# Fro116/RecommenderSystem

Measured on AMD Instinct MI355X. Metric: interactions/sec, higher is better.
Workload: dtype bf16

## Files before the change

### include/rsys_debug.h

```cpp
#ifndef RSYS_DEBUG_H
#define RSYS_DEBUG_H
#include "rsys.h"

#ifdef __cplusplus
extern "C" {
#endif

int32_t rsys_debug_get(rsys_model* m, const char* key, void* out, int64_t bytes);

int32_t rsys_local_group_create(int32_t world, int32_t device, void** group);
int32_t rsys_local_group_destroy(void* group);
int32_t rsys_comm_init_local(void* group, int32_t rank, rsys_comm** out);
int32_t rsys_comm_debug_delay(rsys_comm* c, int32_t microseconds);

int32_t rsys_dev_alloc(void** p, size_t bytes);
int32_t rsys_dev_free(void* p);
int32_t rsys_dev_h2d(void* dst, const void* src, size_t bytes);
int32_t rsys_dev_d2h(void* dst, const void* src, size_t bytes);
int32_t rsys_dev_memset(void* dst, int value, size_t bytes);
int32_t rsys_op_gemm(int32_t dtype, const void* A, const void* B, void* C, int32_t M, int32_t N, int32_t K,
                     int64_t lda, int64_t ldb, int64_t ldc, int32_t a_km, int32_t b_km, int32_t a_f32, int32_t c_f32,
                     int32_t splitk);
int32_t rsys_op_gemm_rows(int32_t dtype, const void* A, const void* B, void* C, int32_t M, int32_t N, int32_t K,
                          int64_t lda, int64_t ldb, int64_t ldc, int32_t b_km, int32_t c_f32, const int32_t* rows_dev);
// ... 8 lines not shown
                              int32_t b_km, int32_t a_f32, int32_t c_f32, int32_t epi, int32_t splitk, int32_t flags, float alpha,
                              int32_t accum, int32_t set, int32_t m_expect, int32_t cus, char* tag, int32_t tag_bytes, int32_t* splits);
int32_t rsys_op_attention(int32_t dtype, int32_t B, int32_t T, int32_t H, int32_t KV, int32_t hd, const void* qkv,
                          const int32_t* uid, const int32_t* tm, void* O, float* lse, const void* dO, void* dqkv,
                          const float* rope_cos, const float* rope_sin);
int32_t rsys_op_attention_ex(int32_t dtype, int32_t B, int32_t T, int32_t H, int32_t KV, int32_t hd, const void* qkv,
                             const int32_t* uid, const int32_t* tm, void* O, float* lse, const void* dO, void* dqkv,
                             const float* rope_cos, const float* rope_sin, const int32_t* rope_pos, int32_t rope_rows,
                             const int32_t* q_active, float* amax_fwd, float* amax_bwd);
int32_t rsys_op_attention_cached(int32_t dtype, int32_t rows, int32_t T, int32_t H, int32_t KV, int32_t hd, const void* qkv, const void* cache,
                                 int32_t n_slots, const int32_t* slot, const int32_t* n_hist, const int32_t* n_cand, void* O);
int32_t rsys_op_attention_cached_tiles(int32_t dtype, int32_t rows, int32_t T, int32_t H, int32_t KV, int32_t hd, const void* qkv, const void* cache,
                                       int32_t n_slots, int32_t Tc, int32_t n_seg, const int32_t* seg, void* O);
int32_t rsys_op_rank_cache_copy_segments(int32_t dtype, int32_t rows, int32_t T, int32_t H, int32_t KV, int32_t hd, const void* qkv, void* cache,
                                         int32_t n_slots, int32_t Tc, int32_t n_seg, const int32_t* seg);
int32_t rsys_rank_cache_get(rsys_model* m, int32_t layer, int32_t slot, void* out, int64_t bytes);
int32_t rsys_op_topk(const float* scores, int64_t ld, int32_t rows, int32_t V, int32_t k,
                     int32_t* ids, float* vals, int32_t* counts);
int32_t rsys_op_target_rank(const float* scores, int64_t ld, int32_t rows, int32_t V, const int32_t* targets, int32_t* rank_out);
int32_t rsys_op_pair_ranks(const float* scores, int64_t ld, int32_t rows, int32_t V, const int32_t* self, const int64_t* tgt_offsets,
                           const int32_t* tgt_ids, int32_t* ranks_out);
int32_t rsys_sim_pair_scores(void* h, int32_t n_src, const int32_t* sources, float* out);
int32_t rsys_rank_gram_get(rsys_model* m, int32_t medium, int32_t n_groups, const int64_t* cand_offsets, const int32_t* cand_ids,
                           float* out, int64_t n_out);
int32_t rsys_op_rerank(int32_t n, int32_t partialk, const float* pen, const float* r, const float* gram, const int32_t* ss_bits,
                       const int32_t* related_bits, int32_t* picks);
int32_t rsys_render_debug_keep(rsys_model* m, int32_t on);
int32_t rsys_render_debug_get(rsys_model* m, const char* key, void* out, int64_t cap, int64_t* bytes);
int32_t rsys_sim_debug_get(void* h, const char* name, void* out, int64_t n);
int32_t rsys_search_debug_get(void* h, const char* name, float* out, int64_t n);
int32_t rsys_op_embedding_scatter(const float* gx0, int64_t ldx, const int32_t* matchedid, const int32_t* m_matchedid, int32_t N,
                                  int32_t V, int32_t D, float* gE, int32_t atomic);
int32_t rsys_op_f8_quantize(const void* src, int64_t ld_src, int32_t rows, int32_t cols, int32_t fmt, int32_t layout, int32_t seg_cols,
                            int32_t seg_rep, void* dst, int64_t ld_dst, float* amax_dev, float* desc_dev, const float* wamax_dev,
                            int32_t n_w, int32_t w_rep, int32_t desc_mode);
int32_t rsys_op_f8_weights(const float* src, int64_t ld, int32_t rows, int32_t cols, int32_t layout, int32_t seg_rows, int32_t seg_rep,
                           float* amax_dev, void* dst, void* dst_t, int64_t ld_t);
int32_t rsys_op_gemm_f8(const void* A8, const void* B8, void* C, int32_t M, int32_t N, int32_t K, int64_t lda, int64_t ldb, int64_t ldc,
                        int32_t a_fmt, int32_t c_f32, const float* desc_dev, int32_t seg_cols, int32_t alt, int32_t kb0, int32_t kb1,
                        int32_t kb2);
int32_t rsys_op_rmsnorm_fwd(int32_t dtype, const float* x, const float* scale, void* y, float* rstd, int64_t rows, int32_t D,
                            const int32_t* rows_dev, const int32_t* in_rows, float* amax);
int32_t rsys_op_rmsnorm_bwd(int32_t dtype, int32_t g_f32, const void* g, const float* x, const float* scale, const float* rstd,
                            const float* resid, const int32_t* resid_slot, const int32_t* io_rows, const int32_t* rows_dev,
                            float* dx, void* dx_t, float* dscale, int64_t rows, int32_t D, float* amax, int32_t deterministic);
int32_t rsys_op_ce(int32_t dtype, void* logits, int64_t ldl, int32_t n, int32_t V, const int32_t* idx, const float* label,
                   const float* weight, const int32_t* position, const float* stats, const int32_t* npos, float task_w, float* loss,
                   int32_t deterministic);
int32_t rsys_op_rating_tail(int32_t dtype, void* z, const void* hact, int32_t n, int32_t D, const float* w2, const float* b2,
                            const int32_t* idx, const float* label, const float* weight, const float* stats, float rating_mean,
                            float task_w, int32_t evaluate, float* loss, float* dw2, float* db2, float* db0, const int32_t* npos,
                            int32_t deterministic);
int32_t rsys_op_sumsq(const float* g, int64_t n, float* out);
int32_t rsys_op_clip_adamw(int32_t dtype, float* p, float* g, float* m, float* v, void* shadow, int64_t n_decay, int64_t n_total,
                           float lr, float b1, float b2, float eps, float wd, int32_t step, float max_norm, float grad_div,
                           int32_t zero_grad, int64_t sh_skip_lo, int64_t sh_skip_hi, int32_t fused, float* sumsq);
int32_t rsys_op_adapter_bank(int32_t dtype, int32_t stages, int32_t train, int32_t rows, int32_t Ttok, int32_t D, int32_t H, int32_t KV, int32_t hd,
                             int32_t L, int32_t layer, float p, uint64_t seed, int64_t stream, const int32_t* row_slot, const void* bankA,
                             const void* bankB, const void* xn, void* La, void* qkv, const void* dqkv, void* dLa, void* dxn, float* partA, float* partB,
                             float* gA, float* gB, const float* rope_cos, const float* rope_sin, const int32_t* rope_pos, int32_t rope_rows);
int32_t rsys_op_adapter_bank_tiles(int32_t dtype, int32_t stages, int32_t rows, int32_t Ttok, int32_t D, int32_t H, int32_t KV, int32_t hd, int32_t L,
                                   int32_t layer, const int32_t* tile_slot, const void* bankA, const void* bankB, const void* xn, void* La, void* qkv,
                                   const float* rope_cos, const float* rope_sin, const int32_t* rope_pos, int32_t rope_rows);
int32_t rsys_op_adapter_bank_segments(int32_t dtype, int32_t stages, int32_t train, int32_t rows, int32_t Ttok, int32_t D, int32_t H, int32_t KV, int32_t hd,
                                      int32_t L, int32_t layer, float p, uint64_t seed, int64_t stream, const int32_t* segs, int32_t n_seg, const void* bankA,
                                      const void* bankB, const void* xn, void* La, void* qkv, const void* dqkv, void* dLa, void* dxn, float* partA,
                                      float* partB, float* gA, float* gB, const float* rope_cos, const float* rope_sin, const int32_t* rope_pos,
                                      int32_t rope_rows);
int32_t rsys_op_adapter_bank_adamw(int32_t dtype, float* A32, float* B32, float* gA, float* gB, float* mA, float* vA, float* mB, float* vB, void* A,
                                   void* B, int64_t nA, int64_t nB, const float* per_slot, float b1, float b2, float eps, float wd, float* norms);
int32_t rsys_op_dropout(int32_t dtype, const void* src, void* dst, int64_t n, float p, uint64_t seed, int64_t stream, int32_t accumulate);
int32_t rsys_op_vp_ce(int32_t dtype, int32_t stages, int32_t deterministic, const int32_t* idx, const float* label, const float* weight,
                      const int32_t* position, const float* stats, const int32_t* npos, float task_w, int32_t KB, int32_t KBmax, float* own,
                      const void* EwAll, const float* metaAll, int32_t W, int32_t D, void* EwC, float* metaC, int32_t* nlive, int32_t* pre,
                      void* logits, int64_t ldl, int32_t Vloc, int32_t col0, float* lmax, const float* gmax, float* sums, int32_t cap,
                      int32_t rank, float* loss, int32_t rows, int32_t rows_finish);
int32_t rsys_op_ss(int32_t dtype, int32_t stages, int32_t deterministic, int32_t len, int32_t n_s, int32_t n_tot, int32_t col0, uint64_t seed,
                   int64_t stream, int32_t* cols, int32_t* bitmap, int32_t* tlist, int32_t* tcount, const float* metaC, const int32_t* nlive,
                   const int32_t* pre, int32_t rank, int32_t cap_rows, int32_t rows, int32_t rows_finish, const void* EwC, const void* Floc,
                   int32_t D, void* logits, int64_t ldl, float* lmax, float* lsum, float* tl, float* gmax, float* loss, float* dt,
                   float* gE_loc, float* dEwC, const int32_t* ridx, int32_t rbase, int64_t rld, int32_t rn, int32_t rtable_rows,
                   const void* gsrc, void* gdst, const float* asrc, float* adst);
int32_t rsys_op_shard_rows(int32_t stages, const int32_t* skey, const int32_t* sidx, int32_t N, int32_t V, int32_t* slot, int32_t* uniq,
                           int32_t* tok2u, int32_t* plan, const int32_t* bound, int32_t nb, int32_t* off, float* table, int64_t ld,
                           int32_t table_rows, const int32_t* ids, int32_t sub, float* packed, int32_t n, int32_t D, const int32_t* count,
                           const int32_t* m_matchedid, const int32_t* userid, const int32_t* m_tmid, int32_t Ntok, const float* Frem,
                           int32_t frem_rows, float* x0, int32_t* uid_t, int32_t* tm_t);

#ifdef __cplusplus
}
#endif
#endif
```

### recommendersystem_amd/_lib.py

```python
import ctypes as C
import os

os.environ.setdefault("HSA_ENABLE_IPC_MODE_LEGACY", "0")

HERE = os.path.dirname(os.path.abspath(__file__))
LIB_PATH = os.path.join(HERE, "librsys_hip.so")


class RsysError(RuntimeError):
    pass


class rsys_config(C.Structure):
    _fields_ = [
        ("num_layers", C.c_int32), ("num_heads", C.c_int32), ("num_kv_heads", C.c_int32),
        ("embed_dim", C.c_int32), ("intermediate_dim", C.c_int32), ("max_sequence_length", C.c_int32),
        ("vocab_0", C.c_int32), ("vocab_1", C.c_int32),
        ("vocab_status", C.c_int32), ("vocab_gender", C.c_int32), ("vocab_source", C.c_int32),
        ("metadata_dim", C.c_int32),
        ("min_ts", C.c_double), ("max_ts", C.c_double),
        ("rating_mean", C.c_float), ("rating_std", C.c_float), ("mask_rate", C.c_float),
        ("mask_topk", C.c_int32), ("finetune", C.c_int32), ("finetune_metric", C.c_int32),
        ("dtype", C.c_int32), ("max_rows", C.c_int32), ("lora_dropout", C.c_float),
        ("table_shard_rank", C.c_int32), ("table_shard_world", C.c_int32), ("sampled_negatives", C.c_int32),
# ... 149 lines not shown
    ("rsys_comm_destroy", C.c_int32, [_P]),
    ("rsys_comm_debug_delay", C.c_int32, [_P, C.c_int32]),
    ("rsys_set_grad_sync", C.c_int32, [_P, _P]),
    ("rsys_model_set_split_table_reduce", C.c_int32, [_P, C.c_int32]),
    ("rsys_model_set_shard_comm", C.c_int32, [_P, _P]),
    ("rsys_table_rows", C.c_int32, [_P, C.POINTER(C.c_int64), C.POINTER(C.c_int64)]),
    ("rsys_local_group_create", C.c_int32, [C.c_int32, C.c_int32, C.POINTER(_P)]),
    ("rsys_local_group_destroy", C.c_int32, [_P]),
    ("rsys_comm_init_local", C.c_int32, [_P, C.c_int32, C.POINTER(_P)]),
    ("rsys_allreduce_grads", C.c_int32, [_P, _P]),
    ("rsys_grad_sync_early", C.c_int32, [_P, C.POINTER(C.c_int64)]),
    ("rsys_grad_sync_schedule", C.c_int32, [_P, C.POINTER(C.c_int64), C.c_int32, C.POINTER(C.c_int32)]),
    ("rsys_comm_info", C.c_int32, [_P, C.POINTER(C.c_int32)]),
    ("rsys_allreduce_f64", C.c_int32, [_P, C.POINTER(C.c_double), C.c_int32]),
    ("rsys_self_test", C.c_int32, [_P]),
    ("rsys_param_checksum", C.c_int32, [_P, C.POINTER(C.c_double * 4)]),
    ("rsys_grad_buffer", C.c_int32, [_P, C.POINTER(_P), C.POINTER(C.c_int64)]),
    ("rsys_param_buffer", C.c_int32, [_P, C.POINTER(_P), C.POINTER(C.c_int64)]),
    ("rsys_refresh_shadow", C.c_int32, [_P]),
    ("rsys_dev_alloc", C.c_int32, [C.POINTER(_P), C.c_size_t]),
    ("rsys_dev_free", C.c_int32, [_P]),
    ("rsys_dev_h2d", C.c_int32, [_P, _P, C.c_size_t]),
    ("rsys_dev_d2h", C.c_int32, [_P, _P, C.c_size_t]),
    ("rsys_dev_memset", C.c_int32, [_P, C.c_int, C.c_size_t]),
    ("rsys_op_gemm", C.c_int32, [C.c_int32, _P, _P, _P, C.c_int32, C.c_int32, C.c_int32, C.c_int64, C.c_int64, C.c_int64,
                                 C.c_int32, C.c_int32, C.c_int32, C.c_int32, C.c_int32]),
    ("rsys_op_f8_quantize", C.c_int32, [_P, C.c_int64, C.c_int32, C.c_int32, C.c_int32, C.c_int32, C.c_int32, C.c_int32, _P, C.c_int64, _P, _P, _P,
                                          C.c_int32, C.c_int32, C.c_int32]),
    ("rsys_op_f8_weights", C.c_int32, [_P, C.c_int64, C.c_int32, C.c_int32, C.c_int32, C.c_int32, C.c_int32, _P, _P, _P, C.c_int64]),
    ("rsys_op_gemm_f8", C.c_int32, [_P, _P, _P, C.c_int32, C.c_int32, C.c_int32, C.c_int64, C.c_int64, C.c_int64, C.c_int32, C.c_int32, _P,
                                      C.c_int32, C.c_int32, C.c_int32, C.c_int32, C.c_int32]),
    ("rsys_op_gemm_rows", C.c_int32, [C.c_int32, _P, _P, _P, C.c_int32, C.c_int32, C.c_int32, C.c_int64, C.c_int64, C.c_int64,
                                      C.c_int32, C.c_int32, _P]),
    ("rsys_op_gemm_klimit", C.c_int32, [C.c_int32, _P, _P, _P, C.c_int32, C.c_int32, C.c_int32, C.c_int64, C.c_int64, C.c_int64, C.c_int32, _P]),
    ("rsys_op_gemm_epi", C.c_int32, [C.c_int32, _P, _P, _P, C.c_int32, C.c_int32, C.c_int32, C.c_int64, C.c_int64, C.c_int64, C.c_int32, C.c_int32,
                                     C.c_int32, C.c_float, C.c_int32, _P, _P, C.c_int64, _P, C.c_int64, _P, _P, _P, _P, _P,
                                     C.c_int32, C.c_int32, C.c_int32, C.c_int32, _P, C.c_char_p, C.c_int32, C.POINTER(C.c_int32)]),
    ("rsys_debug_gemm_route", C.c_int32, [C.c_int32] * 4 + [C.c_int64] * 3 + [C.c_int32] * 7 + [C.c_float] + [C.c_int32] * 4
                                          + [C.c_char_p, C.c_int32, C.POINTER(C.c_int32)]),
    ("rsys_op_attention", C.c_int32, [C.c_int32] + [C.c_int32] * 5 + [_P] * 9),
    ("rsys_op_attention_ex", C.c_int32, [C.c_int32] + [C.c_int32] * 5 + [_P] * 10 + [C.c_int32, _P, _P, _P]),
    ("rsys_op_topk", C.c_int32, [_P, C.c_int64, C.c_int32, C.c_int32, C.c_int32, _P, _P, _P]),
    ("rsys_op_target_rank", C.c_int32, [_P, C.c_int64, C.c_int32, C.c_int32, _P, _P]),
    ("rsys_op_pair_ranks", C.c_int32, [_P, C.c_int64, C.c_int32, C.c_int32, _P, _P, _P, _P]),
    ("rsys_rank_gram_get", C.c_int32, [_P, C.c_int32, C.c_int32, _P, _P, _P, C.c_int64]),
    ("rsys_op_rerank", C.c_int32, [C.c_int32, C.c_int32, _P, _P, _P, _P, _P, _P]),
    ("rsys_op_embedding_scatter", C.c_int32, [_P, C.c_int64, _P, _P, C.c_int32, C.c_int32, C.c_int32, _P, C.c_int32]),
    ("rsys_op_rmsnorm_fwd", C.c_int32, [C.c_int32, _P, _P, _P, _P, C.c_int64, C.c_int32, _P, _P, _P]),
    ("rsys_op_rmsnorm_bwd", C.c_int32, [C.c_int32, C.c_int32] + [_P] * 11 + [C.c_int64, C.c_int32, _P, C.c_int32]),
    ("rsys_op_ce", C.c_int32, [C.c_int32, _P, C.c_int64, C.c_int32, C.c_int32] + [_P] * 6 + [C.c_float, _P, C.c_int32]),
    ("rsys_op_rating_tail", C.c_int32, [C.c_int32, _P, _P, C.c_int32, C.c_int32] + [_P] * 6 + [C.c_float, C.c_float, C.c_int32]
                                        + [_P] * 5 + [C.c_int32]),
    ("rsys_op_sumsq", C.c_int32, [_P, C.c_int64, _P]),
    ("rsys_op_clip_adamw", C.c_int32, [C.c_int32] + [_P] * 5 + [C.c_int64, C.c_int64] + [C.c_float] * 5
                                       + [C.c_int32, C.c_float, C.c_float, C.c_int32, C.c_int64, C.c_int64, C.c_int32, _P]),
    ("rsys_op_adapter_bank", C.c_int32, [C.c_int32] * 11 + [C.c_float, C.c_uint64, C.c_int64] + [_P] * 16 + [C.c_int32]),
    ("rsys_op_adapter_bank_tiles", C.c_int32, [C.c_int32] * 10 + [_P] * 9 + [C.c_int32]),
    ("rsys_op_adapter_bank_segments", C.c_int32, [C.c_int32] * 11 + [C.c_float, C.c_uint64, C.c_int64, _P, C.c_int32] + [_P] * 15 + [C.c_int32]),
    ("rsys_op_adapter_bank_adamw", C.c_int32, [C.c_int32] + [_P] * 10 + [C.c_int64, C.c_int64, _P] + [C.c_float] * 4 + [_P]),
    ("rsys_op_dropout", C.c_int32, [C.c_int32, _P, _P, C.c_int64, C.c_float, C.c_uint64, C.c_int64, C.c_int32]),
    ("rsys_op_vp_ce", C.c_int32, [C.c_int32] * 3 + [_P] * 6 + [C.c_float, C.c_int32, C.c_int32, _P, _P, _P, C.c_int32, C.c_int32]
                                  + [_P] * 5 + [C.c_int64, C.c_int32, C.c_int32, _P, _P, _P, C.c_int32, C.c_int32, _P, C.c_int32, C.c_int32]),
    ("rsys_op_ss", C.c_int32, [C.c_int32] * 7 + [C.c_uint64, C.c_int64] + [_P] * 7 + [C.c_int32] * 4 + [_P, _P, C.c_int32, _P, C.c_int64]
                               + [_P] * 9 + [C.c_int32, C.c_int64, C.c_int32, C.c_int32] + [_P] * 4),
    ("rsys_op_shard_rows", C.c_int32, [C.c_int32, _P, _P, C.c_int32, C.c_int32] + [_P] * 5 + [C.c_int32, _P, _P, C.c_int64, C.c_int32, _P,
                                       C.c_int32, _P, C.c_int32, C.c_int32] + [_P] * 4 + [C.c_int32, _P, C.c_int32, _P, _P, _P]),
    ("rsys_step_mark", C.c_int32, [_P]),
    ("rsys_step_marks_get", C.c_int32, [_P, _P, C.c_int32, C.POINTER(C.c_int32)]),
    ("rsys_op_timing", C.c_int32, [_P, C.c_int32]),
    ("rsys_timing_get", C.c_int32, [_P, C.c_char_p, C.c_size_t]),
    ("rsys_op_timing_filter", C.c_int32, [_P, C.c_char_p]),
    ("rsys_switches_reload", C.c_int32, []),
    ("rsys_switches_describe", C.c_int32, [C.c_char_p, C.c_int32]),
]
EXPORTED = [s[0] for s in _SIGS]

_lib = None


def lib():
    global _lib
    if _lib is None:
        if not os.path.exists(LIB_PATH):
            raise RsysError(f"{LIB_PATH} is missing: build it with `make -C recommendersystem_amd/csrc` "
                            "(there is no CPU fallback for the HIP path)")
        L = C.CDLL(LIB_PATH, mode=C.RTLD_GLOBAL)
        for name, res, args in _SIGS:
            fn = getattr(L, name)
            fn.restype = res
            fn.argtypes = args
        _lib = L
    return _lib


def last_error():
    buf = C.create_string_buffer(2048)
    lib().rsys_last_error(buf, 2048)
    return buf.value.decode(errors="replace")


def check(rc):
    if rc != 0:
        raise RsysError(f"rsys error {rc}: {last_error()}")


def device_count():
# ... 16 lines not shown
```

### recommendersystem_amd/csrc/capi.hip

```cpp
#include <algorithm>
#include <dlfcn.h>
#include <math.h>
#include <stdlib.h>
#include <string.h>

#include <sstream>

#include "comm.hpp"
#include "encoder_handle.hpp"
#include "model_internal.hpp"

namespace rsys {
static thread_local std::string g_err;
void set_error(const std::string& msg) { g_err = msg; }
}

using namespace rsys;

struct rsys_model { Model* m; };
struct rsys_optimizer { Optimizer o; };

#define CHECK_HANDLE(h) do { if ((h) == nullptr) { set_error("null handle"); return RSYS_ERR_ARG; } } while (0)

extern "C" {

const char* rsys_version(void) { return "recommendersystem_amd 0.1 (gfx950)"; }

size_t rsys_last_error(char* buf, size_t n) {
  if (buf && n) { strncpy(buf, g_err.c_str(), n - 1); buf[n - 1] = 0; }
  return g_err.size();
}

int32_t rsys_device_count(int32_t* n) {
  int c = 0;
  hipError_t e = hipGetDeviceCount(&c);
  if (e != hipSuccess) c = 0;
  if (n) *n = c;
  return RSYS_OK;
}
int32_t rsys_device_synchronize(void) { HIP_CHECK(hipDeviceSynchronize()); return RSYS_OK; }

int32_t rsys_model_create(const rsys_config* cfg, int32_t device, rsys_model** out) {
  switches_parse();
  Model* m = nullptr;
  int rc = model_create(cfg, device, &m);
  if (rc) return rc;
  *out = new rsys_model{m};
  return RSYS_OK;
}
int32_t rsys_model_destroy(rsys_model* h) { if (!h) return RSYS_OK; model_destroy(h->m); delete h; return RSYS_OK; }
int32_t rsys_model_init_random(rsys_model* h, uint64_t seed) { CHECK_HANDLE(h); return model_init_random(h->m, seed); }
int32_t rsys_model_load_metadata(rsys_model* h, const float* t, int64_t V, int64_t M) { CHECK_HANDLE(h); ARG_CHECK(t, "null table"); return model_load_metadata(h->m, t, V, M); }
int32_t rsys_model_random_metadata(rsys_model* h, uint64_t seed) { CHECK_HANDLE(h); return model_random_metadata(h->m, seed); }
int32_t rsys_model_set_rope(rsys_model* h, const float* c, const float* s, int64_t n) { CHECK_HANDLE(h); ARG_CHECK(c && s, "null table"); return model_set_rope(h->m, c, s, n); }

int32_t rsys_param_count(rsys_model* h, int32_t* n) { CHECK_HANDLE(h); *n = (int32_t)h->m->tensors.size(); return RSYS_OK; }
int32_t rsys_param_info(rsys_model* h, int32_t i, char* name, size_t cap, int64_t shape[2], int32_t* ndim, int32_t* trainable) {
  CHECK_HANDLE(h);
  ARG_CHECK(i >= 0 && i < (int)h->m->tensors.size(), "parameter index");
  const TensorInfo& t = h->m->tensors[i];
  if (name && cap) { strncpy(name, t.name.c_str(), cap - 1); name[cap - 1] = 0; }
  if (shape) { if (t.ndim == 1) { shape[0] = t.cols; shape[1] = 0; } else { shape[0] = t.rows; shape[1] = t.cols; } }
  if (ndim) *ndim = t.ndim;
  if (trainable) *trainable = t.trainable ? 1 : 0;
  return RSYS_OK;
}
int32_t rsys_param_get(rsys_model* h, const char* name, float* out, int64_t n) { CHECK_HANDLE(h); ARG_CHECK(name && out, "null"); return model_param_io(h->m, name, out, nullptr, n, 0); }
int32_t rsys_param_set(rsys_model* h, const char* name, const float* in, int64_t n) { CHECK_HANDLE(h); ARG_CHECK(name && in, "null"); return model_param_io(h->m, name, nullptr, in, n, 0); }
int32_t rsys_grad_get(rsys_model* h, const char* name, float* out, int64_t n) { CHECK_HANDLE(h); ARG_CHECK(name && out, "null"); return model_param_io(h->m, name, out, nullptr, n, 1); }
int32_t rsys_zero_grad(rsys_model* h) {
  CHECK_HANDLE(h);
  HIP_CHECK(hipSetDevice(h->m->device));
  HIP_CHECK(hipMemsetAsync(h->m->G, 0, h->m->n_total * 4, h->m->stream));
  h->m->table_grads_pending = false;
  h->m->gE_clean[0] = h->m->gE_clean[1] = true;
  return RSYS_OK;
}

int32_t rsys_batch_upload(rsys_model* h, const rsys_batch* b) { CHECK_HANDLE(h); return model_batch_upload(h->m, b); }
int32_t rsys_batch_rows(rsys_model* h, int32_t* rows_out) { CHECK_HANDLE(h); ARG_CHECK(rows_out, "null"); *rows_out = h->m->cur_rows; return RSYS_OK; }
int32_t rsys_batch_upload_trimmed(rsys_model* h, const rsys_batch* b, int32_t row_len) { CHECK_HANDLE(h); return model_batch_upload_trimmed(h->m, b, row_len); }
int32_t rsys_batch_row_length(rsys_model* h, int32_t* row_len_out) {
  CHECK_HANDLE(h); ARG_CHECK(row_len_out, "null");
  *row_len_out = h->m->cur_rows > 0 ? h->m->S : 0;
  return RSYS_OK;
}
int32_t rsys_serving_pack_set(rsys_model* h, int32_t on) { CHECK_HANDLE(h); h->m->serving_pack = on != 0; return RSYS_OK; }
int32_t rsys_serving_pack_get(rsys_model* h, int32_t* on_out) { CHECK_HANDLE(h); ARG_CHECK(on_out, "null"); *on_out = h->m->serving_pack ? 1 : 0; return RSYS_OK; }
int32_t rsys_serving_pack_ranking_set(rsys_model* h, int32_t on) { CHECK_HANDLE(h); h->m->serving_pack_ranking = on != 0; return RSYS_OK; }
int32_t rsys_serving_pack_ranking_get(rsys_model* h, int32_t* on_out) { CHECK_HANDLE(h); ARG_CHECK(on_out, "null"); *on_out = h->m->serving_pack_ranking ? 1 : 0; return RSYS_OK; }
int32_t rsys_serving_trim_set(rsys_model* h, int32_t on) { CHECK_HANDLE(h); h->m->serving_trim = on != 0; return RSYS_OK; }
int32_t rsys_serving_trim_get(rsys_model* h, int32_t* on_out) { CHECK_HANDLE(h); ARG_CHECK(on_out, "null"); *on_out = h->m->serving_trim ? 1 : 0; return RSYS_OK; }
int32_t rsys_batch_prefetch(rsys_model* h, const rsys_batch* b) { CHECK_HANDLE(h); return model_batch_prefetch(h->m, b); }
int32_t rsys_batch_swap(rsys_model* h) { CHECK_HANDLE(h); return model_batch_swap(h->m); }

int32_t rsys_forward_backward(rsys_model* h, int32_t evaluate, const float task_w[4], float grad_scale, uint64_t seed, uint64_t step) {
  CHECK_HANDLE(h);
  return model_forward_backward(h->m, evaluate, task_w, grad_scale, seed, step);
}

int32_t rsys_losses_get(rsys_model* h, float losses_out[12], float wsum_out[4]) {
  CHECK_HANDLE(h);
  Model* m = h->m;
  HIP_CHECK(hipSetDevice(m->device));
  float acc[16], st[8];
  HIP_CHECK(hipMemcpyAsync(acc, m->loss_acc, 16 * 4, hipMemcpyDeviceToHost, m->stream));
  HIP_CHECK(hipMemcpyAsync(st, m->stats, 8 * 4, hipMemcpyDeviceToHost, m->stream));
  HIP_CHECK(hipStreamSynchronize(m->stream));
  for (int ti = 0; ti < 4; ++ti) {
    float ws = fmaxf(st[2 * ti], 1e-8f);
    for (int k = 0; k < 3; ++k) losses_out[3 * ti + k] = acc[3 * ti + k] / ws;
    if (wsum_out) wsum_out[ti] = st[2 * ti + 1];
  }
  return RSYS_OK;
}

int32_t rsys_losses_push(rsys_model* h) {
  CHECK_HANDLE(h);
  Model* m = h->m;
  HIP_CHECK(hipSetDevice(m->device));
  if (m->loss_ring == nullptr) HIP_CHECK(hipMalloc((void**)&m->loss_ring, (size_t)Model::loss_ring_cap * 24 * 4));
  if (m->loss_ring_n >= Model::loss_ring_cap) { set_error("rsys_losses_push: ring full (rsys_losses_drain first)"); return RSYS_ERR_STATE; }
  float* slot = m->loss_ring + (size_t)m->loss_ring_n * 24;
  HIP_CHECK(hipMemcpyAsync(slot, m->loss_acc, 16 * 4, hipMemcpyDeviceToDevice, m->stream));
  HIP_CHECK(hipMemcpyAsync(slot + 16, m->stats, 8 * 4, hipMemcpyDeviceToDevice, m->stream));
  m->loss_ring_n += 1;
  return RSYS_OK;
}
// ... 561 lines not shown
  std::vector<std::pair<int64_t, int64_t>> done = m->reduced, rem;
  m->reduced.clear();
  if (m->sharded) done.emplace_back(m->o_E, m->o_E + (int64_t)m->TR * m->D);
  if (split) {
    done.emplace_back(m->o_E, m->o_E + (int64_t)m->TR * m->D);
    m->early_reduced += (int64_t)m->TR * m->D;
  }
  std::sort(done.begin(), done.end());
  int64_t at = 0;
  for (auto& r : done) { if (r.first > at) rem.emplace_back(at, r.first); at = std::max(at, r.second); }
  if (at < m->n_opt) rem.emplace_back(at, m->n_opt);
  auto reduce_rest = [&](int64_t lo, int64_t hi) -> int {
    for (auto& r : rem) {
      const int64_t a = std::max(r.first, lo), b = std::min(r.second, hi);
      if (a < b) { int rc = reduce_range(m, c, a, b); if (rc) return rc; }
    }
    return RSYS_OK;
  };
  if (model_finalize_splittable(m)) {
    int64_t wo = 0, wn = 0;
    int rc = model_finalize_stage(m, 1, &wo, &wn);
    if (rc) return rc;
    HIP_CHECK(hipEventRecord(c->ev_ready, m->stream));
    HIP_CHECK(hipStreamWaitEvent(c->stream, c->ev_ready, 0));
    m->bucket_phase = 1;
    if (split) {
      int64_t tail_rows = 0;
      rc = model_split_table_tail(m, c, c->stream, &tail_rows);
      if (rc) return rc;
      m->bucket_log.push_back({0, (int64_t)c->world * tail_rows * (m->D + 1), 4});
    }
    rc = reduce_rest(0, std::min(wo, m->n_opt));
    if (rc) return rc;
    rc = reduce_rest(std::min(wo + wn, m->n_opt), m->n_opt);
    if (rc) return rc;
    rc = model_finalize_stage(m, 2, nullptr, nullptr);
    if (rc) return rc;
    HIP_CHECK(hipEventRecord(c->ev_ready, m->stream));
    HIP_CHECK(hipStreamWaitEvent(c->stream, c->ev_ready, 0));
    m->bucket_phase = 2;
    rc = reduce_rest(wo, std::min(wo + wn, m->n_opt));
    if (rc) return rc;
  } else {
    m->bucket_phase = 1;
    int rc = model_finalize_grads(m);
    if (rc) return rc;
    HIP_CHECK(hipEventRecord(c->ev_ready, m->stream));
    HIP_CHECK(hipStreamWaitEvent(c->stream, c->ev_ready, 0));
    rc = reduce_rest(0, m->n_opt);
    if (rc) return rc;
  }
  HIP_CHECK(hipEventRecord(c->ev_done, c->stream));
  HIP_CHECK(hipStreamWaitEvent(m->stream, c->ev_done, 0));
  return RSYS_OK;
}
int32_t rsys_grad_sync_early(rsys_model* h, int64_t* n) { CHECK_HANDLE(h); ARG_CHECK(n, "null"); *n = h->m->early_reduced; return RSYS_OK; }
int32_t rsys_grad_sync_schedule(rsys_model* h, int64_t* out, int32_t cap, int32_t* n_out) {
  CHECK_HANDLE(h); ARG_CHECK(out && n_out && cap >= 0, "null");
  const auto& log = h->m->bucket_log;
  const int n = (int)std::min<size_t>(log.size(), (size_t)cap);
  for (int i = 0; i < n; ++i) { out[3 * i] = log[i].lo; out[3 * i + 1] = log[i].hi; out[3 * i + 2] = log[i].phase; }
  *n_out = (int32_t)log.size();
  return RSYS_OK;
}
int32_t rsys_comm_info(rsys_comm* c, int32_t out[4]) {
  CHECK_HANDLE(c); ARG_CHECK(out, "null");
  out[0] = c->rank; out[1] = c->world;
  out[2] = c->lg ? 2 : (c->comm ? 1 : 0);
  out[3] = c->comm ? comm_rccl_version() : 0;
  return RSYS_OK;
}
int32_t rsys_allreduce_f64(rsys_comm* c, double* x, int32_t n) {
  CHECK_HANDLE(c);
  ARG_CHECK(n >= 1 && n <= 64 && x, "n in [1,64]");
  if (!comm_active(c)) return RSYS_OK;
  HIP_CHECK(hipSetDevice(c->device));
  HIP_CHECK(hipMemcpyAsync(c->scratch, x, n * 8, hipMemcpyHostToDevice, c->stream));
  RC(comm_all_reduce_f64(c, c->scratch, (size_t)n, c->stream));
  HIP_CHECK(hipMemcpyAsync(x, c->scratch, n * 8, hipMemcpyDeviceToHost, c->stream));
  HIP_CHECK(hipStreamSynchronize(c->stream));
  return RSYS_OK;
}
int32_t rsys_self_test(rsys_comm* c) {
  CHECK_HANDLE(c);
  double one = 1.0;
  int rc = rsys_allreduce_f64(c, &one, 1);
  if (rc) return rc;
  if (one != (double)c->world) { set_error("all-reduce self test: sum of ones != world size"); return RSYS_ERR_COMM; }
  return RSYS_OK;
}

int32_t rsys_grad_buffer(rsys_model* h, void** p, int64_t* n) {
  CHECK_HANDLE(h);
  int rc = model_finalize_grads(h->m);
  if (rc) return rc;
  *p = h->m->G; *n = h->m->n_opt;
  return RSYS_OK;
}
int32_t rsys_param_buffer(rsys_model* h, void** p, int64_t* n) { CHECK_HANDLE(h); *p = h->m->P; *n = h->m->n_total; return RSYS_OK; }
int32_t rsys_refresh_shadow(rsys_model* h) { CHECK_HANDLE(h); return model_refresh_shadow(h->m); }

int32_t rsys_dev_alloc(void** p, size_t bytes) { HIP_CHECK(hipMalloc(p, bytes ? bytes : 16)); HIP_CHECK(hipMemset(*p, 0, bytes ? bytes : 16)); return RSYS_OK; }
int32_t rsys_dev_free(void* p) { HIP_CHECK(hipFree(p)); return RSYS_OK; }
int32_t rsys_dev_h2d(void* d, const void* s, size_t n) { HIP_CHECK(hipMemcpy(d, s, n, hipMemcpyHostToDevice)); return RSYS_OK; }
int32_t rsys_dev_d2h(void* d, const void* s, size_t n) { HIP_CHECK(hipDeviceSynchronize()); HIP_CHECK(hipMemcpy(d, s, n, hipMemcpyDeviceToHost)); return RSYS_OK; }
int32_t rsys_dev_memset(void* d, int v, size_t n) { HIP_CHECK(hipMemset(d, v, n)); return RSYS_OK; }

int32_t rsys_op_gemm(int32_t dtype, const void* A, const void* B, void* C, int32_t M, int32_t N, int32_t K, int64_t lda,
                     int64_t ldb, int64_t ldc, int32_t a_km, int32_t b_km, int32_t a_f32, int32_t c_f32, int32_t splitk) {
  switches_parse();
  GemmParams p{};
  p.A = A; p.B = B; p.C = C; p.M = M; p.N = N; p.K = K; p.lda = lda; p.ldb = ldb; p.ldc = ldc;
  p.c_f32 = c_f32; p.splitk = splitk < 1 ? 1 : splitk; p.alpha = 1.f;
  p.epi = p.splitk > 1 ? EPI_ATOMIC : EPI_STORE;
  if (sw().debug_epi >= 0) p.epi = sw().debug_epi;
  int rc = dtype == RSYS_DTYPE_BF16 ? launch_gemm<bf16>(p, a_f32 != 0, false, a_km != 0, b_km != 0, nullptr)
                                    : launch_gemm<float>(p, false, false, a_km != 0, b_km != 0, nullptr);
  if (rc) return rc;
  HIP_CHECK(hipDeviceSynchronize());
  return RSYS_OK;
}

int32_t rsys_op_gemm_rows(int32_t dtype, const void* A, const void* B, void* C, int32_t M, int32_t N, int32_t K, int64_t lda,
                          int64_t ldb, int64_t ldc, int32_t b_km, int32_t c_f32, const int32_t* rows_dev) {
  switches_parse();
  ARG_CHECK(rows_dev != nullptr, "rsys_op_gemm_rows: rows_dev is null");
  GemmParams p{};
  p.A = A; p.B = B; p.C = C; p.M = M; p.N = N; p.K = K; p.lda = lda; p.ldb = ldb; p.ldc = ldc;
  p.c_f32 = c_f32 != 0; p.splitk = 1; p.alpha = 1.f; p.epi = EPI_STORE; p.m_dev = rows_dev;
  if (c_f32 == 3) { p.epi = EPI_ATOMIC; p.splitk = 8; }
  int rc = dtype == RSYS_DTYPE_BF16 ? launch_gemm<bf16>(p, false, false, false, b_km != 0, nullptr)
                                    : launch_gemm<float>(p, false, false, false, b_km != 0, nullptr);
  if (rc) return rc;
  HIP_CHECK(hipDeviceSynchronize());
  return RSYS_OK;
}

int32_t rsys_op_gemm_klimit(int32_t dtype, const void* A, const void* B, void* C, int32_t M, int32_t N, int32_t K, int64_t lda,
                            int64_t ldb, int64_t ldc, int32_t accumulate, const int32_t* k_dev) {
  switches_parse();
  ARG_CHECK(k_dev != nullptr, "rsys_op_gemm_klimit: k_dev is null");
  GemmParams p{};
  p.A = A; p.B = B; p.C = C; p.M = M; p.N = N; p.K = K; p.lda = lda; p.ldb = ldb; p.ldc = ldc;
  p.c_f32 = 1; p.splitk = 1; p.alpha = 1.f; p.epi = accumulate ? EPI_ACCUM : EPI_STORE; p.k_dev = k_dev;
  int rc = dtype == RSYS_DTYPE_BF16 ? launch_gemm<bf16>(p, false, false, true, true, nullptr)
                                    : launch_gemm<float>(p, false, false, true, true, nullptr);
  if (rc) return rc;
  HIP_CHECK(hipDeviceSynchronize());
// ... 335 lines not shown
                     : launch_rmsnorm_bwd_f32<float>((const float*)g, x, scale, rstd, resid, dx, (float*)dx_t, dscale, rows, D, nullptr, rows_dev, amax);
  else rc = bf ? launch_rmsnorm_bwd<bf16>((const bf16*)g, x, scale, rstd, resid, dx, (bf16*)dx_t, dscale, rows, D, nullptr, rows_dev, resid_slot, io_rows, amax)
               : launch_rmsnorm_bwd<float>((const float*)g, x, scale, rstd, resid, dx, (float*)dx_t, dscale, rows, D, nullptr, rows_dev, resid_slot, io_rows, amax);
  if (rc) return rc;
  HIP_CHECK(hipDeviceSynchronize());
  return det.check("rsys_op_rmsnorm_bwd");
}

int32_t rsys_op_ce(int32_t dtype, void* logits, int64_t ldl, int32_t n, int32_t V, const int32_t* idx, const float* label,
                   const float* weight, const int32_t* position, const float* stats, const int32_t* npos, float task_w, float* loss,
                   int32_t deterministic) {
  switches_parse();
  ARG_CHECK(logits && idx && label && weight && position && stats && loss && n >= 0 && V >= 1, "rsys_op_ce: arguments");
  HookDet det(deterministic != 0 && n > 0);
  RC(det.alloc(n, ceil32(n)));
  int rc = dtype == RSYS_DTYPE_BF16 ? launch_ce_fwd_bwd<bf16>((bf16*)logits, ldl, n, V, idx, label, weight, position, stats, npos, task_w, loss, nullptr)
                                    : launch_ce_fwd_bwd<float>((float*)logits, ldl, n, V, idx, label, weight, position, stats, npos, task_w, loss, nullptr);
  if (rc) return rc;
  HIP_CHECK(hipDeviceSynchronize());
  return det.check("rsys_op_ce");
}

int32_t rsys_op_rating_tail(int32_t dtype, void* z, const void* hact, int32_t n, int32_t D, const float* w2, const float* b2,
                            const int32_t* idx, const float* label, const float* weight, const float* stats, float rating_mean,
                            float task_w, int32_t evaluate, float* loss, float* dw2, float* db2, float* db0, const int32_t* npos,
                            int32_t deterministic) {
  switches_parse();
  ARG_CHECK(z && hact && w2 && b2 && idx && label && weight && stats && loss && dw2 && db2 && db0 && n >= 0, "rsys_op_rating_tail: arguments");
  HookDet det(deterministic != 0 && n > 0);
  const long long grid = std::min<long long>((n + 3) / 4, 512);
  RC(det.alloc(grid * (2LL * D + 4), ceil32(grid) * D));
  int rc = dtype == RSYS_DTYPE_BF16
               ? launch_rating_tail<bf16>((bf16*)z, (const bf16*)hact, n, D, w2, b2, idx, label, weight, stats, rating_mean, task_w, evaluate, loss,
                                          dw2, db2, db0, nullptr, npos)
               : launch_rating_tail<float>((float*)z, (const float*)hact, n, D, w2, b2, idx, label, weight, stats, rating_mean, task_w, evaluate, loss,
                                           dw2, db2, db0, nullptr, npos);
  if (rc) return rc;
  HIP_CHECK(hipDeviceSynchronize());
  return det.check("rsys_op_rating_tail");
}

int32_t rsys_op_sumsq(const float* g, int64_t n, float* out) {
  ARG_CHECK(g && out, "rsys_op_sumsq: arguments");
  float* part = nullptr;
  HIP_CHECK(hipMalloc((void**)&part, (size_t)sumsq_parts() * 4));
  int rc = launch_sumsq(g, n, out, part, nullptr, true);
  hipError_t e = hipDeviceSynchronize();
  hipFree(part);
  if (rc) return rc;
  HIP_CHECK(e);
  return RSYS_OK;
}

int32_t rsys_op_clip_adamw(int32_t dtype, float* p, float* g, float* m, float* v, void* shadow, int64_t n_decay, int64_t n_total,
                           float lr, float b1, float b2, float eps, float wd, int32_t step, float max_norm, float grad_div,
                           int32_t zero_grad, int64_t sh_skip_lo, int64_t sh_skip_hi, int32_t fused, float* sumsq) {
  switches_parse();
  ARG_CHECK(p && g && m && v && sumsq && n_total >= 4 && step >= 1, "rsys_op_clip_adamw: arguments");
  float* part = nullptr;
  HIP_CHECK(hipMalloc((void**)&part, (size_t)sumsq_parts() * 4));
  const bool bf = dtype == RSYS_DTYPE_BF16;
  int rc = launch_sumsq(g, n_total, sumsq, part, nullptr, true);
  if (fused) {
    const float* ss = max_norm > 0.f ? sumsq : nullptr;
    if (!rc) rc = bf ? launch_adamw<bf16>(p, g, m, v, (bf16*)shadow, n_decay, n_total, lr, b1, b2, eps, wd, step, ss, grad_div, max_norm, zero_grad, nullptr,
                                          sh_skip_lo, sh_skip_hi)
                     : launch_adamw<float>(p, g, m, v, nullptr, n_decay, n_total, lr, b1, b2, eps, wd, step, ss, grad_div, max_norm, zero_grad, nullptr);
  } else {
    if (!rc) rc = launch_scale(g, n_total, sumsq, grad_div, max_norm, nullptr);
    if (!rc) rc = bf ? launch_adamw<bf16>(p, g, m, v, (bf16*)shadow, n_decay, n_total, lr, b1, b2, eps, wd, step, nullptr, 1.f, 0.f, zero_grad, nullptr,
                                          sh_skip_lo, sh_skip_hi)
                     : launch_adamw<float>(p, g, m, v, nullptr, n_decay, n_total, lr, b1, b2, eps, wd, step, nullptr, 1.f, 0.f, zero_grad, nullptr);
  }
  hipError_t e = hipDeviceSynchronize();
  hipFree(part);
  if (rc) return rc;
  HIP_CHECK(e);
  return RSYS_OK;
}

int32_t rsys_op_adapter_bank(int32_t dtype, int32_t stages, int32_t train, int32_t rows, int32_t Ttok, int32_t D, int32_t H, int32_t KV, int32_t hd,
                             int32_t L, int32_t layer, float p, uint64_t seed, int64_t stream, const int32_t* row_slot, const void* bankA,
                             const void* bankB, const void* xn, void* La, void* qkv, const void* dqkv, void* dLa, void* dxn, float* partA, float* partB,
                             float* gA, float* gB, const float* rope_cos, const float* rope_sin, const int32_t* rope_pos, int32_t rope_rows) {
  switches_parse();
  return adapter_bank_op(dtype, stages, train, rows, Ttok, D, H, KV, hd, L, layer, p, seed, stream, row_slot, bankA, bankB, xn, La, qkv, dqkv, dLa, dxn,
                         partA, partB, gA, gB, rope_cos, rope_sin, rope_pos, rope_rows);
}

int32_t rsys_op_adapter_bank_tiles(int32_t dtype, int32_t stages, int32_t rows, int32_t Ttok, int32_t D, int32_t H, int32_t KV, int32_t hd, int32_t L,
                                   int32_t layer, const int32_t* tile_slot, const void* bankA, const void* bankB, const void* xn, void* La, void* qkv,
                                   const float* rope_cos, const float* rope_sin, const int32_t* rope_pos, int32_t rope_rows) {
  switches_parse();
  return adapter_bank_op(dtype, stages, 0, rows, Ttok, D, H, KV, hd, L, layer, 0.f, 0, 0, tile_slot, bankA, bankB, xn, La, qkv, nullptr, nullptr, nullptr,
                         nullptr, nullptr, nullptr, nullptr, rope_cos, rope_sin, rope_pos, rope_rows, 1);
}

int32_t rsys_op_adapter_bank_segments(int32_t dtype, int32_t stages, int32_t train, int32_t rows, int32_t Ttok, int32_t D, int32_t H, int32_t KV, int32_t hd,
                                      int32_t L, int32_t layer, float p, uint64_t seed, int64_t stream, const int32_t* segs, int32_t n_seg, const void* bankA,
                                      const void* bankB, const void* xn, void* La, void* qkv, const void* dqkv, void* dLa, void* dxn, float* partA,
                                      float* partB, float* gA, float* gB, const float* rope_cos, const float* rope_sin, const int32_t* rope_pos,
                                      int32_t rope_rows) {
  switches_parse();
  return adapter_bank_op(dtype, stages, train, rows, Ttok, D, H, KV, hd, L, layer, p, seed, stream, segs, bankA, bankB, xn, La, qkv, dqkv, dLa, dxn, partA,
                         partB, gA, gB, rope_cos, rope_sin, rope_pos, rope_rows, 2, n_seg);
}
// ... 275 lines not shown
```

### recommendersystem_amd/csrc/elementwise.hip

```cpp
#include "kernels.hpp"

namespace rsys {

thread_local DetScratch g_det;

__global__ void reduce_parts_kernel(const float* __restrict__ part, int nparts, long long stride, int n, float* dst) {
  const int c = blockIdx.x * blockDim.x + threadIdx.x;
  if (c >= n) return;
  float acc = 0.f;
  for (int b = 0; b < nparts; ++b) acc += part[(long long)b * stride + c];
  dst[c] += acc;
}
__global__ void reduce_parts_stage_kernel(const float* __restrict__ part, int nparts, long long stride, int n, float* out) {
  const int c = blockIdx.x * blockDim.x + threadIdx.x, chunk = blockIdx.y;
  if (c >= n) return;
  const int b0 = chunk * 32, b1 = min(nparts, b0 + 32);
  float acc = 0.f;
  for (int b = b0; b < b1; ++b) acc += part[(long long)b * stride + c];
  out[(long long)chunk * n + c] = acc;
}
int launch_reduce_parts(const float* part, int nparts, long long stride, int n, float* dst, hipStream_t s) {
  if (nparts <= 0 || n <= 0) return RSYS_OK;
  if (nparts > 64 && g_det.tmp != nullptr) {
    const int chunks = (nparts + 31) / 32;
// ... 796 lines not shown
__global__ __launch_bounds__(1024) void cast_colsum_kernel(const float* __restrict__ src, bf16* __restrict__ dst, long long rows, int D,
                                                           float* colsum, int rows_per_block, float* part) {
  __shared__ float red[2048];
  const int cg = D >> 2;
  const int c = (threadIdx.x % cg) * 4, lane_r = threadIdx.x / cg, nr = 1024 / cg;
  const long long r0 = (long long)blockIdx.x * rows_per_block, r1 = min(rows, r0 + rows_per_block);
  float4 acc = make_float4(0, 0, 0, 0);
  long long r = r0 + lane_r;
  for (; r + 3 * nr < r1; r += 4 * nr) {
    float4 v[4];
#pragma unroll
    for (int u = 0; u < 4; ++u) v[u] = *(const float4*)(src + (r + u * nr) * D + c);
#pragma unroll
    for (int u = 0; u < 4; ++u) {
      bf16x4 o; o[0] = (bf16)v[u].x; o[1] = (bf16)v[u].y; o[2] = (bf16)v[u].z; o[3] = (bf16)v[u].w;
      *(bf16x4*)(dst + (r + u * nr) * D + c) = o;
      acc.x += v[u].x; acc.y += v[u].y; acc.z += v[u].z; acc.w += v[u].w;
    }
  }
  for (; r < r1; r += nr) {
    const float4 v = *(const float4*)(src + r * D + c);
    bf16x4 o; o[0] = (bf16)v.x; o[1] = (bf16)v.y; o[2] = (bf16)v.z; o[3] = (bf16)v.w;
    *(bf16x4*)(dst + r * D + c) = o;
    acc.x += v.x; acc.y += v.y; acc.z += v.z; acc.w += v.w;
  }
  if (lane_r < 2) *(float4*)&red[lane_r * D + c] = acc;
  __syncthreads();
  for (int base = 2; base < nr; base += 2) {
    if (lane_r >= base && lane_r < base + 2) {
      float4 o = *(float4*)&red[(lane_r - base) * D + c];
      o.x += acc.x; o.y += acc.y; o.z += acc.z; o.w += acc.w;
      *(float4*)&red[(lane_r - base) * D + c] = o;
    }
    __syncthreads();
  }
  for (int cc = threadIdx.x; cc < D; cc += 1024) {
    const float v = red[cc] + (nr > 1 ? red[D + cc] : 0.f);
    if (part != nullptr) part[(long long)blockIdx.x * D + cc] = v;
    else if (v != 0.f) atomicAdd(&colsum[cc], v);
  }
}
int launch_cast_colsum(const float* src, bf16* dst, long long rows, int D, float* colsum, hipStream_t s) {
  ARG_CHECK(D % 4 == 0 && D <= 1024 && 1024 % (D >> 2) == 0, "cast_colsum: D/4 must divide 1024, D <= 1024");
  const int rpb = (int)std::max<long long>(32, (rows + 511) / 512);
  const int grid = div_up(rows, rpb);
  float* part = det_part((long long)grid * D);
  hipLaunchKernelGGL(cast_colsum_kernel, dim3(grid), dim3(1024), 0, s, src, dst, rows, D, colsum, rpb, part);
  HIP_CHECK(hipGetLastError());
  if (part != nullptr) return launch_reduce_parts(part, grid, D, D, colsum, s);
  return RSYS_OK;
}

__global__ __launch_bounds__(256) void cast_transpose_colsum_kernel(const float* __restrict__ src, bf16* __restrict__ dstT, long long rows, int D,
                                                                    long long ldt, float* colsum, int rows_per_block, float* part) {
  __shared__ unsigned short tile[64][72];
  __shared__ float red[16][64];
  const int t = threadIdx.x;
  const int lr = t >> 4, c4 = (t & 15) * 4;
  const int oc = t >> 2, or8 = (t & 3) * 16;
  const long long r0 = (long long)blockIdx.x * rows_per_block;
  const long long rend = min((rows + 63) & ~63LL, r0 + rows_per_block);
  for (int ct = 0; ct < D / 64; ++ct) {
    float4 acc = make_float4(0, 0, 0, 0);
    for (long long rb = r0; rb < rend; rb += 64) {
      float4 v[4];
#pragma unroll
      for (int i = 0; i < 4; ++i) {
        const long long r = rb + 4 * lr + i;
        v[i] = r < rows ? *(const float4*)(src + r * D + ct * 64 + c4) : make_float4(0, 0, 0, 0);
        acc.x += v[i].x; acc.y += v[i].y; acc.z += v[i].z; acc.w += v[i].w;
      }
      {
        bf16x4 o;
        o[0] = (bf16)v[0].x; o[1] = (bf16)v[1].x; o[2] = (bf16)v[2].x; o[3] = (bf16)v[3].x; *(bf16x4*)&tile[c4 + 0][4 * lr] = o;
        o[0] = (bf16)v[0].y; o[1] = (bf16)v[1].y; o[2] = (bf16)v[2].y; o[3] = (bf16)v[3].y; *(bf16x4*)&tile[c4 + 1][4 * lr] = o;
        o[0] = (bf16)v[0].z; o[1] = (bf16)v[1].z; o[2] = (bf16)v[2].z; o[3] = (bf16)v[3].z; *(bf16x4*)&tile[c4 + 2][4 * lr] = o;
        o[0] = (bf16)v[0].w; o[1] = (bf16)v[1].w; o[2] = (bf16)v[2].w; o[3] = (bf16)v[3].w; *(bf16x4*)&tile[c4 + 3][4 * lr] = o;
      }
      __syncthreads();
      {
        const uint4 q0 = *(const uint4*)&tile[oc][or8], q1 = *(const uint4*)&tile[oc][or8 + 8];
        uint4* d = (uint4*)(dstT + (long long)(ct * 64 + oc) * ldt + rb + or8);
        d[0] = q0; d[1] = q1;
      }
      __syncthreads();
    }
    *(float4*)&red[lr][c4] = acc;
    __syncthreads();
    if (t < 64) {
      float v = 0.f;
#pragma unroll
      for (int k = 0; k < 16; ++k) v += red[k][t];
      if (part != nullptr) part[(long long)blockIdx.x * D + ct * 64 + t] = v;
      else if (v != 0.f) atomicAdd(&colsum[ct * 64 + t], v);
    }
    __syncthreads();
  }
}
int launch_cast_transpose_colsum(const float* src, bf16* dstT, long long rows, int D, long long ldt, float* colsum, hipStream_t s) {
  ARG_CHECK(D % 64 == 0 && ldt % 8 == 0 && ldt >= ((rows + 63) & ~63LL), "cast_transpose_colsum: D % 64, ldt % 8, ldt >= rows rounded up to 64");
  const long long chunks = (rows + 63) / 64;
  const int cpb = (int)std::max<long long>(1, (chunks + 2047) / 2048);
  const int grid = (int)((chunks + cpb - 1) / cpb);
  float* part = det_part((long long)grid * D);
  hipLaunchKernelGGL(cast_transpose_colsum_kernel, dim3(grid), dim3(256), 0, s, src, dstT, rows, D, ldt, colsum, cpb * 64, part);
  HIP_CHECK(hipGetLastError());
  if (part != nullptr) return launch_reduce_parts(part, grid, D, D, colsum, s);
  return RSYS_OK;
}

__global__ void embedding_scatter_kernel(const float* __restrict__ gx0, BatchDev b, int V, int D, float* gE) {
  const int n = (blockIdx.x * blockDim.x + threadIdx.x) >> 6, l = threadIdx.x & 63;
  if (n >= b.N) return;
  int id = b.m_matchedid[n];
  id = id == -1 ? V : id;
  const float* src = gx0 + (long long)(2 * n) * D;
  float* dst = gE + (long long)id * D;
  for (int c = l; c < D; c += 64) atomicAdd(&dst[c], src[c]);
}
int launch_embedding_scatter_add(const float* gx0, const BatchDev& b, int V, int D, float* gE, hipStream_t s) {
  hipLaunchKernelGGL(embedding_scatter_kernel, dim3(div_up(b.N, 4)), dim3(256), 0, s, gx0, b, V, D, gE);
  HIP_CHECK(hipGetLastError());
  return RSYS_OK;
}

__global__ __launch_bounds__(256) void action_small_bwd_kernel(const float* __restrict__ gf, BatchDev b, SmallParams sp,
                                                               float* g_cos, float* g_sin, float* g_status, float* g_gender,
                                                               float* g_source) {
  __shared__ float acc[4 + 16 * 4 + 16 * 4 + 16 * 16];
  const int NG = (sp.n_gender + 1) * 4, NS = (sp.n_source + 1) * 4, NST = (sp.n_status + 1) * 16;
  float* a_g = acc + 4; float* a_s = a_g + 64; float* a_st = a_s + 64;
  for (int c = threadIdx.x; c < 4 + 64 + 64 + 256; c += 256) acc[c] = 0.f;
  __syncthreads();
  for (int i = blockIdx.x * blockDim.x + threadIdx.x; i < b.N; i += gridDim.x * blockDim.x) {
    const float* g = gf + (long long)i * 32;
    float p0, p1; double ts;
    periodic_args(b.time[i], sp.min_ts, p0, p1, ts);
    atomicAdd(&acc[0], -sinf(p0 + sp.per_cos[0]) * g[1]);
    atomicAdd(&acc[1], -sinf(p1 + sp.per_cos[1]) * g[2]);
    atomicAdd(&acc[2], cosf(p0 + sp.per_sin[0]) * g[3]);
    atomicAdd(&acc[3], cosf(p1 + sp.per_sin[1]) * g[4]);
    int gi = b.gender[i]; gi = gi == -1 ? sp.n_gender : gi;
    int si = b.source[i]; si = si == -1 ? sp.n_source : si;
    int st = b.m_status[i]; st = st == -1 ? sp.n_status : st;
#pragma unroll
    for (int k = 0; k < 4; ++k) atomicAdd(&a_g[gi * 4 + k], g[5 + k]);
#pragma unroll
    for (int k = 0; k < 4; ++k) atomicAdd(&a_s[si * 4 + k], g[9 + k]);
#pragma unroll
    for (int k = 0; k < 16; ++k) atomicAdd(&a_st[st * 16 + k], g[15 + k]);
  }
  __syncthreads();
  const int t = threadIdx.x;
  if (t < 2) atomicAdd(&g_cos[t], acc[t]);
  else if (t < 4) atomicAdd(&g_sin[t - 2], acc[t]);
  for (int c = t; c < NG; c += 256) atomicAdd(&g_gender[c], a_g[c]);
  for (int c = t; c < NS; c += 256) atomicAdd(&g_source[c], a_s[c]);
  for (int c = t; c < NST; c += 256) atomicAdd(&g_status[c], a_st[c]);
// ... 51 lines not shown
```

### recommendersystem_amd/csrc/kernels.hpp

```cpp
#pragma once
#include "common.hpp"

namespace rsys {

struct BatchDev {
  int N, rows, S;
  const int *userid, *tmid, *gender, *source, *matchedid, *status;
  const double* time;
  const float *rating, *progress;
  const float* label[6]; const float* weight[6]; const int* position[6];
  const unsigned char *watch_mask, *rating_mask;
  const int* rope_pos;
  int *m_tmid, *m_matchedid, *m_status;
  float *m_rating, *m_progress;
  float* m_label[4]; float* m_weight[4]; int* m_position[4];
};

struct DetScratch {
  float* part = nullptr; long long cap = 0; float* tmp = nullptr; long long tmp_cap = 0;
  int part_used = 0, part_short = 0;
};
extern thread_local DetScratch g_det;
int launch_reduce_parts(const float* part, int nparts, long long stride, int n, float* dst, hipStream_t s);

// ... 10 lines not shown

int launch_mask_tokens_rows(BatchDev b, const int* row_task, hipStream_t s);
int launch_mask_tokens_tiles(BatchDev b, const int* tile_task, hipStream_t s);

template <typename T>
int launch_action_features(const BatchDev& b, const SmallParams& sp, T* feat , hipStream_t s);

int launch_gather_items(const BatchDev& b, const float* F32, int V, int D, float* x0, int* uid_t, int* tm_t, hipStream_t s);

template <typename T>
int launch_rmsnorm_fwd(const float* x, const float* scale, T* y, float* rstd, long long rows, int D, hipStream_t s, const int* rows_dev = nullptr,
                       const int* in_rows = nullptr ,
                       float* f8_amax = nullptr );

template <typename T>
int launch_rmsnorm_bwd(const T* g, const float* x, const float* scale, const float* rstd, const float* resid_grad,
                       float* dx_out, T* dx_out_t, float* dscale, long long rows, int D, hipStream_t s, const int* rows_dev = nullptr,
                       const int* resid_slot = nullptr ,
                       const int* io_rows = nullptr ,
                       float* f8_amax = nullptr );
template <typename T>
int launch_rmsnorm_bwd_f32(const float* g, const float* x, const float* scale, const float* rstd, const float* resid_grad,
                           float* dx_out, T* dx_out_t, float* dscale, long long rows, int D, hipStream_t s, const int* rows_dev = nullptr,
                           float* f8_amax = nullptr);

template <typename T>
int launch_dropout(const T* src, T* dst, long long n, float p, unsigned long long seed, unsigned int stream, int accumulate, hipStream_t s);

int launch_select_positions(const float* w, int N, int topk, int* idx, float* stats ,
                            int* npos_out , hipStream_t s);
int launch_select_positions_chunked(int ntask, const float* const* w, int N, int topk, int* const* idx, float* const* stats, int* const* npos_out,
                                    void* scratch, hipStream_t s);
int launch_select_positions_batch(int ntask, const float* const* w, int N, int topk, int* const* idx, float* const* stats,
                                  int* const* npos_out, hipStream_t s);

template <typename T>
int launch_gather_rows(const T* src, long long ld, const int* idx, int parity, T* dst, int n, int D, hipStream_t s);

int launch_scatter_rows_add(const float* src, const int* idx, int parity, float* dst, long long ld, int n, int D, hipStream_t s,
                            const int* npos = nullptr );

template <typename T>
int launch_ce_fwd_bwd(T* logits, long long ldl, int n, int V, const int* idx, const float* label, const float* weight,
                      const int* position, const float* stats, const int* npos, float task_w, float* loss_out, hipStream_t s);

template <typename T>
int launch_rating_tail(T* z, const T* hact, int n, int D, const float* w2, const float* b2, const int* idx,
                       const float* label, const float* weight, const float* stats, float rating_mean, float task_w,
                       int evaluate, float* loss_out , float* dw2, float* db2, float* db0, hipStream_t s,
                       const int* npos = nullptr );

int launch_colsum_add(const float* src, long long ld, long long rows, int cols, float* dst, hipStream_t s);
int launch_cast_colsum(const float* src, bf16* dst, long long rows, int D, float* colsum, hipStream_t s);
int launch_cast_transpose_colsum(const float* src, bf16* dstT, long long rows, int D, long long ldt, float* colsum, hipStream_t s);

int launch_embedding_scatter_add(const float* gx0, const BatchDev& b, int V, int D, float* gE, hipStream_t s);

int token_index_capacity(int N);
int launch_token_index_build(const int* matchedid, int N, int V, unsigned long long* keys, int* skey, int* sidx, hipStream_t s);
size_t seg_scatter_slab_floats(int N, int D);
int launch_embedding_scatter_segmented(const float* gx0, long long ldx, const int* m_matchedid, const int* skey, const int* sidx,
                                       int N, int V, int D, float* gE, float* slab, hipStream_t s);

int launch_token_union(const int* const* idx, const int* const* npos, int ntask, int NT, unsigned int* bits, int* pre, int* nsel, hipStream_t s);
int launch_selected_first(const unsigned int* bits, const int* pre, int* slot, int* sel, const int* uid, const int* tm, const int* rope_pos, int B, int T,
                          int* perm, int* uid_p, int* tm_p, int* pos_p, int* slot_p, int* sel_p, int* q_active, hipStream_t s);
template <typename T> int launch_gather_rows_sel(const T* src, long long ld, const int* sel, const int* n_dev, int cap, T* dst, int D, hipStream_t s);
template <typename T> int launch_scatter_rows_fill(const T* src, const int* slot_p, const int* q_active, int B, int Tseq, T* dst, long long ld, int D, hipStream_t s);
template <typename T> int launch_scatter_rows_sel(const T* src, const int* sel, const int* n_dev, int cap, T* dst, long long ld, int D, hipStream_t s);
template <typename T> int launch_scatter_rows_map(const T* src, const int* map, int n, T* dst, long long ld, int D, hipStream_t s);
template <typename T> int launch_gather_rows_slot(const T* compact, const int* slot, const int* idx, int parity, T* dst, int n, int D, hipStream_t s);
int launch_scatter_rows_add_slot(const float* src, const int* slot, const int* idx, int parity, const int* npos, float* compact, int n, int D, hipStream_t s);

int launch_plan_unique(const int* skey, const int* sidx, int N, int V, int* slot, int* uniq, int* tok2u, int* plan , hipStream_t s);
int launch_plan_offsets(const int* uniq, const int* plan, const int* bound_dev, int nb, int* off, hipStream_t s);
int launch_gather_rows_by_id(const float* src, long long ld, const int* ids, int sub, float* dst, int n, int D, hipStream_t s);
int launch_add_rows_by_id(const float* src, const int* ids, int sub, float* dst, long long ld, int n, int D, hipStream_t s);
int launch_add_rows_by_id_counted(const float* src, const int* ids, const int* count_dev, float* dst, long long ld, int cap, int D, hipStream_t s);
int launch_gather_items_remote(const BatchDev& b, const float* Frem, const int* tok2u, const int* plan, int D, float* x0,
                               int* uid_t, int* tm_t, hipStream_t s);
int launch_vp_meta(const int* idx, const float* label, const float* weight, const int* position, const float* stats,
                   const int* npos, float task_w, int KB, int KBmax, float* own , hipStream_t s);
int launch_add_scalar(float* dst, const float* src, hipStream_t s);
template <typename T>
int launch_vp_compact(const T* EwAll, const float* metaAll, int W, int KB, int D, T* EwC, float* metaC, int* nlive, int* pre , hipStream_t s);
template <typename T>
int launch_vp_stats(const T* logits, long long ldl, int Vloc, int col0, const float* metaC, const int* nlive, float* lmax,
                    float* sums , int cap, int grid_rows, hipStream_t s);
int launch_vp_rebase(const float* lmax, const float* gmax, float* sums, int n, hipStream_t s);
template <typename T>
int launch_vp_finish(T* logits, long long ldl, int Vloc, int col0, const float* metaC, const float* gmax, const float* sums, int cap,
                     const int* nlive, const int* pre, int rank, float* loss_out, int grid_rows, hipStream_t s);

int launch_ss_sample(int len, int n_s, unsigned long long seed, unsigned int stream, int* cols, hipStream_t s);
template <typename T> int launch_gather_rows_plain(const T* src, long long ld, const int* idx, int base, T* dst, int n, int D, hipStream_t s);
int launch_add_rows_plain(const float* src, const int* idx, int base, float* dst, long long ld, int n, int D, hipStream_t s);
template <typename T>
int launch_ss_target_logit(const T* EwC, const T* Floc, int D, int len, int col0, const float* metaC, const int* nlive, float* tl, int grid_rows, hipStream_t s);
template <typename T>
int launch_ss_stats(const T* logits, long long ldl, int n_s, int n_tot, int len, int col0, const int* cols, const float* metaC, const int* nlive,
                    float* lmax, float* lsum, int grid_rows, hipStream_t s);
int launch_ss_targets(const float* metaC, const int* nlive, int cap_rows, int len, int col0, unsigned int* bitmap, int* out, int* count, hipStream_t s);
int launch_ss_drop_hits(int* cols, int n_s, const unsigned int* bitmap, hipStream_t s);
int launch_ss_max_with_target(const float* lmax, const float* tl, float* out, int n, hipStream_t s);
int launch_ss_rebase(const float* lmax, const float* gmax, float* lsum, int n, hipStream_t s);
template <typename T>
int launch_ss_finish(T* logits, long long ldl, int n_s, int n_tot, int len, int col0, const int* cols, const float* metaC, const float* gmax,
                     const float* sneg, const float* tl, const int* nlive, const int* pre, int rank, float* loss_out,
                     float* dt, int grid_rows, hipStream_t s);
template <typename T>
int launch_ss_target_grad(const T* EwC, const T* Floc, int D, int len, int col0, const float* metaC, const float* dt, const int* nlive,
                          float* gE_loc, float* dEwC, int grid_rows, hipStream_t s);

int launch_action_small_bwd(const float* gf , const BatchDev& b, const SmallParams& sp,
                            float* g_per_cos, float* g_per_sin, float* g_status, float* g_gender, float* g_source,
                            hipStream_t s);

struct AttnParams {
  int B, T, H, KV, hd;
  int is_bf16;
  const void *q, *k, *v;
  long long ld;
  void* o; long long ldo;
  float* lse;
  const int *uid, *tm;
  unsigned int *qmap, *kmap, *qmap_full, *kmap_full;
  unsigned int *qmap16, *kmap16;
  const int* q_active;
  void* maps_zero_base; size_t maps_zero_bytes;
  const void* dO; float* delta;
  void *dq, *dk, *dv; long long ldg;
  const float *rope_cos, *rope_sin; const int* rope_pos;
  float* f8_amax;
  int *order_q, *order_k;
  unsigned long long *qbits, *kbits;
};
inline int attn_map_words(int T) { return (T + 63) / 64 > 32 ? 2 : 1; }
int launch_attn_tilemap(const AttnParams& p, hipStream_t s);
struct CandAttnParams {
  int rows, T, H, KV, hd;
  const void* qkv; long long ld;
  const void* cache; int n_slots;
  int Tc;
  const int *slot, *n_hist, *n_cand;
  void* o; long long ldo;
  const int *tile_seg, *seg; int n_seg;
};
template <typename T> int launch_attn_cand(const CandAttnParams& p, hipStream_t s);
template <typename T> int launch_rank_cache_copy(const T* qkv, long long ld, int kv_off, int kvw, int T_len, int T_slot, int rows, const int* slot, const int* n_hist,
                                                 int n_slots, T* cache, hipStream_t s);
template <typename T> int launch_rank_cache_copy_segments(const T* qkv, long long ld, int kv_off, int kvw, int T_len, int T_slot, int rows, const int* seg, int n_seg,
                                                          int n_slots, T* cache, hipStream_t s);
template <typename T> int launch_attn_fwd(const AttnParams& p, hipStream_t s);
template <typename T> int launch_attn_bwd(const AttnParams& p, hipStream_t s);

int launch_sumsq(const float* g, long long n, float* out , float* part, hipStream_t s, bool overwrite = false);
int sumsq_parts();
int launch_checksum(const float* p, const long long* ranges, int n_ranges, double* part, double* out, hipStream_t s);
int checksum_scratch_doubles();
template <typename T>
int launch_adamw(float* p, float* g, float* m, float* v, T* shadow, long long n_decay, long long n_total,
                 float lr, float b1, float b2, float eps, float wd, int step, const float* sumsq, float grad_div,
                 float max_norm, int zero_grad, hipStream_t s, long long sh_skip_lo = 0, long long sh_skip_hi = 0 );
template <typename T> int launch_cast(const float* src, T* dst, long long n, hipStream_t s);
int launch_add_bias_rows(const float* a, const float* bias, float* dst, long long rows, int D, hipStream_t s);
template <typename T> int launch_widen(const T* src, float* dst, long long n, hipStream_t s);
template <typename T> int launch_rowdot(const T* h, const float* w, const float* b, float* out, int n, int D, hipStream_t s);
struct TransposeJob { const void* src; void* dst; int rows, cols; long long ld_src, ld_dst; };
struct TransposeBatch { TransposeJob job[64]; int n; };
int launch_transpose_bf16(const TransposeBatch& b, hipStream_t s);
int launch_scale(float* g, long long n, const float* sumsq, float grad_div, float max_norm, hipStream_t s);
int launch_fill_normal(float* dst, long long n, float std, unsigned long long seed, unsigned int stream, hipStream_t s, long long first = 0);
template <typename T>
int launch_fill_normal_t(T* dst, long long rows, int cols, long long ld, float std, unsigned long long seed, hipStream_t s, long long row0 = 0);


enum { F8_E4M3 = 0, F8_E5M2 = 1 };
enum { F8_LAYOUT_PLAIN = 0, F8_LAYOUT_SEGS = 1, F8_LAYOUT_SWIGLU = 2 };
struct F8Cast {
  const void* src; long long ld_src; int src_f32;
  int rows, cols;
  const int* rows_dev;
  int fmt, layout, seg_cols, seg_rep;
  float* amax;
  unsigned char* dst; long long ld_dst;
  float* desc; const float* wamax; int n_w; int w_rep; int desc_mode;
  unsigned char* dst_t; long long ld_dst_t;
  float* desc_dw; const float* xamax; int dw_units;
};
int launch_f8_amax(const F8Cast& c, hipStream_t s);
int launch_round_bf16_accum(float* stage, float* dst, long long n, hipStream_t s);
int launch_f8_cast(const F8Cast& c, hipStream_t s);
struct F8WeightJob {
  const float* src; long long ld; int rows, cols;
  int layout, seg_rows, seg_rep;
  float* amax;
  unsigned char* dst;
  unsigned char* dst_t; long long ld_t;
};
int launch_f8_weights(const F8WeightJob* jobs_dev, const int* tile_job_dev, const int* tile_first_dev, int ntiles, hipStream_t s);
int launch_scatter_nan(float* sc, const long long* pos, long long n, hipStream_t s);

}
```

### recommendersystem_amd/csrc/model.hip

```cpp
#include "model_internal.hpp"

namespace rsys {

static void add_tensor(Model* m, const std::string& name, int64_t rows, int64_t cols, int ndim, int64_t off, int64_t ld,
                       int map, bool trainable = true, bool frozen = false) {
  TensorInfo t{name, rows, cols, ndim, off, ld, map, trainable, frozen};
  m->by_name[name] = (int)m->tensors.size();
  m->tensors.push_back(t);
}

static void build_layout(Model* m) {
  const int D = m->D, Ip = m->Ip, I = m->I, L = m->L, hd = m->hd, H = m->H, KV = m->KV;
  const bool ft = m->cfg.finetune != 0;
  int64_t off = 0;
  auto take = [&](int64_t n) { int64_t o = off; off += pad8(n); return o; };
  m->lo.resize(L);
  if (ft) {
    for (int l = 0; l < L; ++l) { m->lo[l].la = take((int64_t)16 * D); m->lo[l].lb = take((int64_t)m->Nqkv * 16); }
  }
  const int64_t n_lora = off;
  m->o_status = take((m->cfg.vocab_status + 1) * 16);
  m->o_gender = take((m->cfg.vocab_gender + 1) * 4);
  m->o_source = take((m->cfg.vocab_source + 1) * 4);
  m->o_lin_w = take((int64_t)D * 32);
// ... 179 lines not shown
  for (int l = 0; l < m->L; ++l) {
    Model::LayerAct& a = m->la[l];
    if (l == 0) a.x = m->x0; else DALLOC(a.x, NT * D * 4);
    DALLOC(a.xn, NT * D * e); DALLOC(a.qkv, NT * m->Nqkv * e);
    a.xnd = a.xn; a.La = nullptr;
    if (cfg->finetune) { DALLOC(a.La, NT * 16 * e); if (cfg->lora_dropout > 0.f) DALLOC(a.xnd, NT * D * e); }
    DALLOC(a.O, NT * D * e); DALLOC(a.lse, (int64_t)m->rows_max * m->H * m->Ta * 4);
    DALLOC(a.rstd1, NT * 4); DALLOC(a.h, NT * D * 4); DALLOC(a.hn, NT * D * e); DALLOC(a.rstd2, NT * 4);
    DALLOC(a.ab, NT * 2 * m->Ip * e); DALLOC(a.g, NT * m->Ip * e);
  }
  DALLOC(m->xL, NT * D * 4); DALLOC(m->rstdf, NT * 4); DALLOC(m->out, NT * D * e);
  for (int k = 0; k < 4; ++k) DALLOC(m->idx[k], KB * 4);
  DALLOC(m->stats, 8 * 4); DALLOC(m->npos, 4 * 4); DALLOC(m->Ew, KB * D * e);
  m->ldl = pad8(std::max(m->V0, m->V1));
  if (m->sharded) {
    const int W = m->sh_world;
    int len_max = 0;
    for (int med = 0; med < 2; ++med) { int len, col0, row; shard_medium_range(m, med, &len, &col0, &row); len_max = std::max(len_max, len); }
    m->ldl_loc = pad8(std::max(len_max, 8));
    const int64_t cap = (int64_t)W * KB;
    const int64_t ss_ns = std::min<int64_t>(cfg->sampled_negatives, std::max(len_max, 1)), ss_tmax = std::min<int64_t>(cap, len_max);
    if (cfg->sampled_negatives > 0) m->ldl_loc = pad8(std::max<int64_t>(m->ldl_loc, ss_ns + ss_tmax));
    DALLOC(m->logits, cap * m->ldl_loc * e); DALLOC(m->dEwC, cap * D * 4); m->dE = m->dEwC;
    DALLOC(m->EwAll, cap * D * e); DALLOC(m->EwC, cap * D * e);
    DALLOC(m->metaOwn, (KB * 4 + 4) * 4); DALLOC(m->metaAll, (int64_t)W * (KB * 4 + 4) * 4); DALLOC(m->metaC, cap * 4 * 4 + 4096);
    DALLOC(m->metaAllT[0], (int64_t)W * (KB * 4 + 4) * 4); DALLOC(m->metaAllT[1], (int64_t)W * (KB * 4 + 4) * 4);
    HIP_CHECK(hipHostMalloc((void**)&m->h_counts, 2 * 64 * sizeof(int), hipHostMallocDefault));
    HIP_CHECK(hipEventCreateWithFlags(&m->ev_counts, hipEventDisableTiming));
    DALLOC(m->vp_max, cap * 4); DALLOC(m->vp_lmax, cap * 4); DALLOC(m->vp_sums, 2 * cap * 4); DALLOC(m->vp_nlive, 64); DALLOC(m->vp_pre, 64 * 4);
    DALLOC(m->u_slot, N * 4); DALLOC(m->u_ids, (N + 1) * 4); DALLOC(m->u_tok, N * 4); DALLOC(m->u_plan, 64);
    DALLOC(m->u_bound, (W + 1) * 4); DALLOC(m->u_off, ((W + 1) + W + (int64_t)W * W) * 4 + 64);
    DALLOC(m->Frem, (N + 1) * D * 4); DALLOC(m->sumsq_E, 64);
    if (cfg->sampled_negatives > 0) {
      const int64_t ns = ss_ns + ss_tmax;
      DALLOC(m->ss_cols, ns * 4 + 64); DALLOC(m->ss_F, ns * D * e); DALLOC(m->ss_dF, ns * D * 4);
      DALLOC(m->ss_tl, cap * 4); DALLOC(m->ss_dt, cap * 4);
      DALLOC(m->ss_bitmap, (len_max / 32 + 2) * 4); DALLOC(m->ss_tcount, 64);
    }
    std::vector<int> bound(W + 1);
    for (int r = 0; r <= W; ++r) bound[r] = (int)((int64_t)r * (m->V + 1) / W);
    HIP_CHECK(hipMemcpy(m->u_bound, bound.data(), (W + 1) * 4, hipMemcpyHostToDevice));
    m->need_off.assign(W + 1, 0); m->serve_off.assign(W + 1, 0); m->need_offD.assign(W + 1, 0); m->serve_offD.assign(W + 1, 0);
  } else {
    DALLOC(m->logits, KB * m->ldl * e); DALLOC(m->dE, KB * D * 4);
  }
  DALLOC(m->z, KB * D * e); DALLOC(m->hact, KB * D * e); DALLOC(m->loss_acc, 16 * 4);
  DALLOC(m->gy, NT * D * 4); DALLOC(m->gxa, NT * D * 4); DALLOC(m->gxb, NT * D * 4); DALLOC(m->dh, NT * D * 4);
  if (m->bf16_mode) { DALLOC(m->gxa_t, NT * D * 2); DALLOC(m->gxb_t, NT * D * 2); DALLOC(m->dh_t, NT * D * 2); }
  else { m->gxa_t = m->gxa; m->gxb_t = m->gxb; m->dh_t = m->dh; }
  DALLOC(m->dab, NT * 2 * m->Ip * e); DALLOC(m->dhn, NT * D * e);
  DALLOC(m->dO, NT * D * e); DALLOC(m->dqkv, NT * m->Nqkv * e);
  DALLOC(m->delta, (int64_t)m->rows_max * m->H * m->Ta * 4); DALLOC(m->gf, N * 32 * 4);
  DALLOC(m->sumsq, 64); DALLOC(m->sumsq_part, (size_t)sumsq_parts() * 4);
  DALLOC(m->sel_scratch, 12 * 32 * 4);
  m->dLa = nullptr; m->dxl = nullptr;
  if (cfg->finetune) { DALLOC(m->dLa, NT * 16 * e); DALLOC(m->dxl, NT * D * e); }
  {
    const int grp = sw().dw_group;
    const long long t13 = (long long)((2 * m->Ip + 255) / 256) * ((m->D + 255) / 256);
    m->defer_dw = grp != 0 && m->bf16_mode && !cfg->finetune && t13 < 32 && m->D % 8 == 0 && m->Ip % 8 == 0 && m->Nqkv % 8 == 0 && m->L <= 30;
    const int sp = sw().sparse_top;
    m->sparse_top = sp != 0 && NT <= (1 << 19) && !m->fp8;
    if (m->defer_dw) {
      m->dwb.resize(m->L);
      for (int l = 0; l < m->L; ++l) {
        m->dwb[l] = Model::DwOperands{nullptr, nullptr, nullptr, nullptr};
        DALLOC(m->dwb[l].dqkv, NT * m->Nqkv * 2);
        if (l == m->L - 1 && m->sparse_top) continue;
        DALLOC(m->dwb[l].gxt, NT * D * 2); DALLOC(m->dwb[l].dab, NT * 2 * m->Ip * 2); DALLOC(m->dwb[l].dht, NT * D * 2);
      }
    }
    if (m->sparse_top) {
      const int64_t cap = (std::min<int64_t>(NT, 4 * KB) + 255) / 256 * 256;
      m->ctop_cap = (int)cap;
      DALLOC(m->c_sel, cap * 4); DALLOC(m->c_slot, NT * 4); DALLOC(m->c_n, 64);
      DALLOC(m->c_bits, (NT / 32 + 2) * 4); DALLOC(m->c_pre, (NT / 32 + 2) * 4);
      DALLOC(m->c_x, cap * D * 4); DALLOC(m->c_h, cap * D * 4); DALLOC(m->c_xL, cap * D * 4); DALLOC(m->c_rstd2, cap * 4); DALLOC(m->c_rstdf, cap * 4);
      DALLOC(m->c_O, cap * D * e); DALLOC(m->c_hn, cap * D * e); DALLOC(m->c_ab, cap * 2 * m->Ip * e); DALLOC(m->c_g, cap * m->Ip * e); DALLOC(m->c_out, cap * D * e);
      { float* blk = nullptr; DALLOC(blk, 256 + cap * D * 4); m->loss_acc = blk; m->c_gy = blk + 64; m->loss_acc_with_c_gy = true; }
      DALLOC(m->c_gx, cap * D * 4); DALLOC(m->c_dh, cap * D * 4);
      DALLOC(m->c_dab, cap * 2 * m->Ip * e); DALLOC(m->c_dhn, cap * D * e); DALLOC(m->c_dO, cap * D * e);
      if (m->bf16_mode) { DALLOC(m->c_gx_t, cap * D * 2); DALLOC(m->c_dh_t, cap * D * 2); } else { m->c_gx_t = m->c_gx; m->c_dh_t = m->c_dh; }
      DALLOC(m->c_perm, NT * 4); DALLOC(m->uid_p, NT * 4); DALLOC(m->tm_p, NT * 4); DALLOC(m->pos_p, NT * 4); DALLOC(m->c_slot_p, NT * 4);
      DALLOC(m->c_sel_p, cap * 4); DALLOC(m->c_qact, (int64_t)m->rows_max * 4 + 64);
      const int64_t mb = ((int64_t)m->rows_max * ((m->Ta + 63) / 64) * 4 * attn_map_words(m->Ta) + 255) / 256 * 256;
      unsigned char* base = nullptr;
      DALLOC(base, mb * 12);
      m->kmap_p = (unsigned int*)base; m->kmap_full_p = (unsigned int*)(base + mb); m->qmap_full_p = (unsigned int*)(base + 2 * mb); m->kmap16_p = (unsigned int*)(base + 3 * mb);
      m->qmap_p = (unsigned int*)(base + 7 * mb); m->qmap16_p = (unsigned int*)(base + 8 * mb);
      const int64_t nt = (m->Ta + 63) / 64;
      DALLOC(m->attn_order_q_p, (int64_t)m->rows_max * m->H * nt * 4); DALLOC(m->attn_order_k_p, (int64_t)m->rows_max * m->KV * nt * 4);
      DALLOC(m->attn_qbits_p, (int64_t)m->rows_max * nt * nt * 64 * 8); DALLOC(m->attn_kbits_p, (int64_t)m->rows_max * nt * nt * 64 * 8);
    }
  }
  if (m->fp8) {
    const int L = m->L, Ip = m->Ip;
    const int64_t base = m->lo[0].wqkv, end = m->lo[L - 1].w2 + (int64_t)D * Ip;
    m->w8_base = base;
    DALLOC(m->W8, end - base); DALLOC(m->W8T, end - base);
    DALLOC(m->f8_wamax, L * 8 * 4); DALLOC(m->f8_aamax, (int64_t)L * F8_AMAX_SHARDS * F8_AMAX_SHARD * 4); DALLOC(m->f8_desc, L * 8 * 32 * 4);
    DALLOC(m->a8, NT * std::max<int64_t>(2 * Ip, m->Nqkv));
    std::vector<F8WeightJob> jobs; std::vector<int> tile_job, tile_first;
    bool aligned = true;
    auto add = [&](int l, int64_t off, int rows, int cols, int layout, int seg_rows, int slot) {
      F8WeightJob j{};
      j.src = m->P + off; j.ld = cols; j.rows = rows; j.cols = cols; j.layout = layout; j.seg_rows = seg_rows; j.seg_rep = m->H / m->KV;
// ... 183 lines not shown
  ARG_CHECK(V == m->V && Mdim == m->M, "metadata table shape must be (V, metadata_dim)");
  const int64_t nrows = std::max<int64_t>(0, std::min<int64_t>(m->row_lo + m->TR, m->V) - m->row_lo);
  return meta_write_rows(m, table + (int64_t)m->row_lo * Mdim, nrows);
}

int model_random_metadata(Model* m, uint64_t seed) {
  HIP_CHECK(hipSetDevice(m->device));
  HIP_CHECK(hipMemsetAsync(m->Meta, 0, (size_t)m->TR * m->Mp * m->esz, m->stream));
  const float std_ = 1.0f / sqrtf((float)m->M);
  const long long nrows = std::max<long long>(0, std::min<long long>(m->row_lo + m->TR, m->V) - m->row_lo);
  if (m->bf16_mode) RC(launch_fill_normal_t<bf16>((bf16*)m->Meta, nrows, m->M, m->Mp, std_, seed, m->stream, m->row_lo));
  else RC(launch_fill_normal_t<float>((float*)m->Meta, nrows, m->M, m->Mp, std_, seed, m->stream, m->row_lo));
  HIP_CHECK(hipStreamSynchronize(m->stream));
  return build_meta_t(m);
}

int model_set_rope(Model* m, const float* c, const float* s, int64_t n_pos) {
  ARG_CHECK(n_pos == m->Ta, "rope tables must have 2*max_sequence_length positions");
  HIP_CHECK(hipSetDevice(m->device));
  size_t bytes = (size_t)n_pos * (m->hd / 2) * 4;
  HIP_CHECK(hipMemcpy(m->rope_cos, c, bytes, hipMemcpyHostToDevice));
  HIP_CHECK(hipMemcpy(m->rope_sin, s, bytes, hipMemcpyHostToDevice));
  {
    const size_t n = bytes / 4;
    std::vector<float> cs(n * 2);
    for (size_t i = 0; i < n; ++i) { cs[2 * i] = c[i]; cs[2 * i + 1] = s[i]; }
    HIP_CHECK(hipMemcpy(m->rope_cs, cs.data(), cs.size() * 4, hipMemcpyHostToDevice));
  }
  return RSYS_OK;
}

int model_param_io(Model* m, const char* name, float* out, const float* in, int64_t n, int which) {
  auto it = m->by_name.find(name);
  if (it == m->by_name.end()) { set_error(std::string("unknown parameter: ") + name); return RSYS_ERR_ARG; }
  const TensorInfo& t = m->tensors[it->second];
  ARG_CHECK(n == t.rows * t.cols, "element count does not match the parameter's shape");
  HIP_CHECK(hipSetDevice(m->device));
  HIP_CHECK(hipStreamSynchronize(m->stream));
  if (t.frozen_table) {
    ARG_CHECK(which == 0, "the metadata table is frozen (model.py:113-114)");
    if (in) {
      return meta_write_rows(m, in, std::max<int64_t>(0, std::min<int64_t>(m->row_lo + m->TR, m->V) - m->row_lo));
    }
    std::vector<unsigned char> host((size_t)t.rows * m->Mp * m->esz);
    HIP_CHECK(hipMemcpy(host.data(), m->Meta, host.size(), hipMemcpyDeviceToHost));
    for (int64_t r = 0; r < t.rows; ++r)
      for (int64_t c = 0; c < t.cols; ++c) {
        if (m->bf16_mode) { uint32_t u = (uint32_t)((unsigned short*)host.data())[r * m->Mp + c] << 16; memcpy(&out[r * t.cols + c], &u, 4); }
        else out[r * t.cols + c] = ((float*)host.data())[r * m->Mp + c];
      }
    return RSYS_OK;
  }
  if (which == 1) RC(model_finalize_grads(m));
  float* base = (which == 0 ? m->P : m->G) + t.off;
  const int64_t int_rows = (t.map == MAP_DIRECT) ? t.rows : 2 * m->Ip;
  std::vector<float> host((size_t)int_rows * t.ld);
  HIP_CHECK(hipStreamSynchronize(m->stream));
  HIP_CHECK(hipMemcpy(host.data(), base, host.size() * 4, hipMemcpyDeviceToHost));
  if (out) {
    for (int64_t r = 0; r < t.rows; ++r) memcpy(out + r * t.cols, host.data() + internal_row(t, r) * t.ld, t.cols * 4);
    return RSYS_OK;
  }
  for (int64_t r = 0; r < t.rows; ++r) memcpy(host.data() + internal_row(t, r) * t.ld, in + r * t.cols, t.cols * 4);
  HIP_CHECK(hipMemcpy(base, host.data(), host.size() * 4, hipMemcpyHostToDevice));
  if (which == 0) { m->wt_dirty = true; m->table_dirty = true; m->w8_dirty = true; }
  if (which == 0 && m->bf16_mode)
    RC(launch_cast<bf16>(base, (bf16*)m->Sh + t.off, (int64_t)host.size(), m->stream));
  HIP_CHECK(hipStreamSynchronize(m->stream));
  return RSYS_OK;
}

static int build_exchange_plan(Model* m, int N) {
  const int W = m->sh_world;
  hipStream_t s = m->stream;
  ARG_CHECK(W == 1 || m->shard_comm != nullptr, "row-sharded table: call rsys_model_set_shard_comm before the first batch");
  RC(launch_plan_unique(m->tok_skey, m->tok_sidx, N, m->V, m->u_slot, m->u_ids, m->u_tok, m->u_plan, s));
  int* d_off = m->u_off; int* d_cnt = m->u_off + (W + 1); int* d_all = d_cnt + W;
  RC(launch_plan_offsets(m->u_ids, m->u_plan, m->u_bound, W + 1, d_off, s));
  int plan[2]; std::vector<int> off(W + 1), cnt(W), all((size_t)W * W);
  HIP_CHECK(hipMemcpyAsync(plan, m->u_plan, 8, hipMemcpyDeviceToHost, s));
  HIP_CHECK(hipMemcpyAsync(off.data(), d_off, (W + 1) * 4, hipMemcpyDeviceToHost, s));
  HIP_CHECK(hipStreamSynchronize(s));
  m->U = plan[0]; m->uV = plan[1];
  ARG_CHECK(off[W] == m->U && m->U >= 1 && m->U <= N + 1, "exchange plan: inconsistent unique-id list");
  for (int q = 0; q <= W; ++q) { m->need_off[q] = off[q]; m->need_offD[q] = (long long)off[q] * m->D; }
  for (int q = 0; q < W; ++q) cnt[q] = off[q + 1] - off[q];
  HIP_CHECK(hipMemcpyAsync(d_cnt, cnt.data(), W * 4, hipMemcpyHostToDevice, s));
  RC(comm_all_gather(m->shard_comm, d_cnt, d_all, (size_t)W * 4, s));
  HIP_CHECK(hipMemcpyAsync(all.data(), d_all, (size_t)W * W * 4, hipMemcpyDeviceToHost, s));
  HIP_CHECK(hipStreamSynchronize(s));
  long long acc = 0;
  for (int q = 0; q < W; ++q) { m->serve_off[q] = acc; m->serve_offD[q] = acc * m->D; acc += all[(size_t)q * W + m->sh_rank]; }
  m->serve_off[W] = acc; m->serve_offD[W] = acc * m->D; m->R = acc;
  if (acc > m->req_cap) {
    if (m->req_ids) HIP_CHECK(hipFree(m->req_ids));
    if (m->rows_xchg) HIP_CHECK(hipFree(m->rows_xchg));
    m->req_cap = acc + acc / 4 + 1024;
    HIP_CHECK(hipMalloc((void**)&m->req_ids, (size_t)m->req_cap * 4));
    HIP_CHECK(hipMalloc((void**)&m->rows_xchg, (size_t)m->req_cap * m->D * 4));
  }
  RC(comm_exchange(m->shard_comm, m->u_ids, m->need_off.data(), m->req_ids, m->serve_off.data(), 4, s));
  HIP_CHECK(hipStreamSynchronize(s));
  return RSYS_OK;
}

struct BlobLayout {
// ... 231 lines not shown
  m->has_masks = m->pending.has_masks; m->d_wm = m->pending.d_wm; m->d_rm = m->pending.d_rm;
  m->has_rope_pos = m->pending.has_rope_pos; m->d_rope_pos = m->pending.d_rope_pos;
  m->cur_rows = m->pending.rows;
  set_row_len(m, m->Sa);
  m->u_bound_host = m->pending.distinct_ids;
  m->tok_index_valid = false;
  m->split_plan_valid = false;
  m->pending.valid = false;
  return RSYS_OK;
}

int model_ensure_det_scratch(Model* m) {
  HIP_CHECK(hipSetDevice(m->device));
  if (m->det_part == nullptr) {
    const long long KB = (long long)m->K * m->rows_max;
    m->det_part_floats = std::max<long long>(std::max<long long>(2048LL * m->D, 512LL * (2 * m->D + 4)), std::max<long long>(KB * m->sh_world, 4096)) + 1024;
    HIP_CHECK(hipMalloc((void**)&m->det_part, (size_t)m->det_part_floats * 4));
    m->det_tmp_floats = m->det_part_floats / 32 + 4096;
    HIP_CHECK(hipMalloc((void**)&m->det_tmp, (size_t)m->det_tmp_floats * 4));
  }
  return RSYS_OK;
}

int model_set_deterministic(Model* m, int on) {
  if (on) RC(model_ensure_det_scratch(m));
  m->deterministic = on != 0;
  return RSYS_OK;
}

template <typename T>
static int forward_backward_t(Model* m, int evaluate, const float task_w[4], float grad_scale, uint64_t seed, uint64_t step,
                              const int* d_row_task = nullptr ) {
  const int rows = m->cur_rows, N = rows * m->S;
  BatchDev b = m->bd; b.N = N; b.rows = rows; b.S = m->S;
  if (m->has_masks) { b.watch_mask = m->d_wm; b.rating_mask = m->d_rm; }
  m->cur_seed = seed; m->cur_step = step;
  if (d_row_task && m->bank_packed) RC(launch_mask_tokens_tiles(b, d_row_task, m->stream));
  else if (d_row_task) RC(launch_mask_tokens_rows(b, d_row_task, m->stream));
  else RC(launch_mask_tokens(b, m->cfg.finetune, m->cfg.finetune_metric, m->cfg.mask_rate, seed, step, m->stream));
  m->drop_active = m->cfg.finetune && !evaluate && m->cfg.lora_dropout > 0.f;
  m->drop_seed = seed ^ 0xD409ull; m->drop_step = step;
  m->top_is_sparse = m->sparse_top && !evaluate && !m->bank_packed;
  m->f8_tcopies = !evaluate;
  m->host_stream_syncs = 0; m->host_event_waits = 0;
  float tw[4];
  for (int i = 0; i < 4; ++i) tw[i] = task_w ? task_w[i] * grad_scale : 0.f;
  RC(select_positions_all(m));
  if (m->sharded) RC(sharded_counts_early<T>(m, !evaluate, tw));
  RC(forward_trunk<T>(m));
  RC(heads<T>(m, evaluate, tw));
  if (!evaluate) {
    m->split_head_reduced = false;
    m->split_head_event = nullptr;
    if (m->table_head_hook) RC(m->table_head_hook());
    RC(backward_trunk<T>(m));
  }
  return RSYS_OK;
}

int model_forward_backward(Model* m, int evaluate, const float task_w[4], float grad_scale, uint64_t seed, uint64_t step) {
  ARG_CHECK(m->cur_rows > 0, "no batch uploaded");
  RC(check_not_trimmed(m));
  ARG_CHECK(evaluate || task_w != nullptr, "task weights are required for training");
  HIP_CHECK(hipSetDevice(m->device));
  DetScope det(m);
  m->last_evaluate = evaluate != 0;
  return m->bf16_mode ? forward_backward_t<bf16>(m, evaluate, task_w, grad_scale, seed, step)
                      : forward_backward_t<float>(m, evaluate, task_w, grad_scale, seed, step);
}

int model_forward_backward_rows(Model* m, int evaluate, const int* d_row_task, float grad_scale, uint64_t seed, uint64_t step) {
  const float tw[4] = {1.f, 1.f, 1.f, 1.f};
  RC(check_not_trimmed(m));
  m->last_evaluate = evaluate != 0;
  return m->bf16_mode ? forward_backward_t<bf16>(m, evaluate, tw, grad_scale, seed, step, d_row_task)
                      : forward_backward_t<float>(m, evaluate, tw, grad_scale, seed, step, d_row_task);
}

template <typename T>
static int infer_rows_t(Model* m, int task, const int* d_sel, int64_t ntok, float* dst, const float** rows_f32);

template <typename T>
static int infer_t(Model* m, int task, const int32_t* sel, int64_t n_sel, float* out, int64_t n) {
  const int rows = m->cur_rows, N = rows * m->S, NT = 2 * N, D = m->D;
  hipStream_t s = m->stream;
  std::vector<int32_t> moved;
  if (sel != nullptr) {
    ARG_CHECK(n_sel <= NT, "selection: more tokens than the batch holds");
    if (batch_trimmed(m)) {
      moved.resize((size_t)n_sel);
      for (int64_t i = 0; i < n_sel; ++i) {
        ARG_CHECK(sel[i] >= 0 && sel[i] < rows * m->Ta, "selection: token index out of range");
        const int r = sel[i] / m->Ta, t = sel[i] % m->Ta;
        ARG_CHECK(t < m->T, "selection: a token at or behind 2 row_len of a trimmed row");
        moved[(size_t)i] = r * m->T + t;
      }
      sel = moved.data();
    }
    for (int64_t i = 0; i < n_sel; ++i) ARG_CHECK(sel[i] >= 0 && sel[i] < NT, "selection: token index out of range");
  }
  const int64_t ntok = sel != nullptr ? n_sel : NT;
  ARG_CHECK(n == (task == 0 ? ntok * D : ntok), task == 0 ? "retrieval output has tokens*D floats" : "ranking output has one float per token");
  int* d_sel = nullptr;
  if (sel != nullptr) {
    d_sel = (int*)m->gf;
    HIP_CHECK(hipMemcpyAsync(d_sel, sel, (size_t)n_sel * 4, hipMemcpyHostToDevice, s));
  }
// ... 136 lines not shown
```

### recommendersystem_amd/csrc/model.hpp

```cpp
#pragma once
#include <functional>
#include <map>
#include <string>
#include <vector>

#include "../../include/rsys.h"
#include "../../include/rsys_debug.h"
#include "comm.hpp"
#include "gemm.hpp"
#include "kernels.hpp"
#include "workspace.hpp"

namespace rsys {

enum RowMap { MAP_DIRECT = 0, MAP_W1 = 1, MAP_W3 = 2 };

struct TensorInfo {
  std::string name;
  int64_t rows, cols;
  int ndim;
  int64_t off;
  int64_t ld;
  int map;
  bool trainable;
// ... 112 lines not shown
  std::vector<void*> allocs;
  BatchDev bd;
  void* batch_blob = nullptr;
  unsigned char* raw_blob = nullptr; unsigned char* h_stage = nullptr; size_t raw_bytes = 0;
  unsigned char* slot_blob[2] = {nullptr, nullptr}; unsigned char* slot_stage[2] = {nullptr, nullptr};
  int cur_slot = 0;
  hipStream_t copy_stream = nullptr;
  hipEvent_t ev_copy_done = nullptr;
  hipEvent_t ev_blob_free[2] = {nullptr, nullptr};
  bool blob_free_valid[2] = {false, false};
  struct PendingBatch { bool valid = false; BatchDev bd; int rows = 0; bool has_masks = false, has_rope_pos = false; int distinct_ids = 0;
                        unsigned char *d_wm = nullptr, *d_rm = nullptr; int* d_rope_pos = nullptr; } pending;
  bool tok_index_valid = false;
  bool deterministic = false;
  float* det_slab = nullptr; long long det_slab_floats = 0;
  float* det_part = nullptr; long long det_part_floats = 0;
  float* det_tmp = nullptr; long long det_tmp_floats = 0;
  bool has_masks = false, has_rope_pos = false;
  int cur_rows = 0;
  unsigned long long* tok_keys = nullptr; int *tok_skey = nullptr, *tok_sidx = nullptr; float* scatter_slab = nullptr;
  unsigned char *d_wm = nullptr, *d_rm = nullptr;
  int* d_rope_pos = nullptr;
  size_t maps_zero_bytes = 0;
  void* feat; float* x0; int *uid_t, *tm_t; unsigned int *qmap, *kmap, *qmap_full, *kmap_full, *qmap16, *kmap16;
  struct LayerAct { float* x; void* xn; void* xnd; void* La; void* qkv; void* O; float* lse; float* rstd1; float* h; void* hn; float* rstd2; void* ab; void* g; };
  std::vector<LayerAct> la;
  float* xL; float* rstdf; void* out;
  float* loss_ring = nullptr; int loss_ring_n = 0; static constexpr int loss_ring_cap = 1024;
  int* idx[4]; int* npos; float* stats; void* Ew; void* logits; int64_t ldl; float* dE; void* z; void* hact; float* loss_acc;
  float *gy, *gxa, *gxb, *dh; void *gxa_t, *gxb_t, *dh_t;
  void *dab, *dhn, *dO, *dqkv; float* delta; float* gf;
  void *dLa, *dxl;
  float* sumsq; float* sumsq_part;
  bool defer_dw = false;
  struct DwOperands { void *gxt, *dab, *dht, *dqkv; };
  std::vector<DwOperands> dwb;
  std::map<long long, GemmGroupPlan*> dw_plans;
  bool sparse_top = false;
  bool top_is_sparse = false;
  int ctop_cap = 0;
  int *c_sel = nullptr, *c_slot = nullptr, *c_n = nullptr;
  unsigned int* c_bits = nullptr; int* c_pre = nullptr;
  float *c_x = nullptr, *c_h = nullptr, *c_xL = nullptr, *c_rstd2 = nullptr, *c_rstdf = nullptr;
  void *c_O = nullptr, *c_hn = nullptr, *c_ab = nullptr, *c_g = nullptr, *c_out = nullptr;
  float *c_gy = nullptr, *c_gx = nullptr, *c_dh = nullptr;
  bool loss_acc_with_c_gy = false;
  void *c_gx_t = nullptr, *c_dab = nullptr, *c_dhn = nullptr, *c_dh_t = nullptr, *c_dO = nullptr;
  int *c_perm = nullptr, *uid_p = nullptr, *tm_p = nullptr, *pos_p = nullptr, *c_slot_p = nullptr, *c_sel_p = nullptr, *c_qact = nullptr;
  unsigned int *qmap_p = nullptr, *kmap_p = nullptr, *qmap_full_p = nullptr, *kmap_full_p = nullptr, *qmap16_p = nullptr, *kmap16_p = nullptr;
  unsigned long long *attn_qbits = nullptr, *attn_kbits = nullptr, *attn_qbits_p = nullptr, *attn_kbits_p = nullptr;
  int *attn_order_q = nullptr, *attn_order_k = nullptr, *attn_order_q_p = nullptr, *attn_order_k_p = nullptr;
  bool table_grads_pending = false;
  bool gE_clean[2] = {false, false};
  bool drop_active = false; unsigned long long drop_seed = 0, drop_step = 0;
  bool last_evaluate = false;
  PhaseTimer timer;
  std::vector<hipEvent_t> step_marks;
  DevScratch rws;
  RetrievalTables* rtab = nullptr;
  RankTables* rank = nullptr;
  DevScratch ews;
  AdapterBank* bank = nullptr;
  const int* bank_rows = nullptr;
  const int* bank_tiles = nullptr;
  bool bank_train = false;
  bool bank_packed = false;
  float* bank_sink = nullptr;
  RenderState* render = nullptr;
  void* rcache = nullptr; int rc_slots = 0; std::vector<int> rc_nhist;
  int* rc_rows = nullptr;
  int rc_mode = 0;
  int* rc_seg = nullptr;
  int rc_nseg = 0;
};

struct Optimizer {
  Model* m;
  int device = 0;
  float lr, b1, b2, eps, wd;
  int step = 0;
  float *mom = nullptr, *var = nullptr;
  bool zero1 = false;
  int z_rank = 0, z_world = 1;
  long long z_chunk = 0, z_tail = 0;
  float* z_tailbuf = nullptr;
};
int optimizer_set_zero1(Optimizer* o, int rank, int world);
int optimizer_step_zero1(Optimizer* o, struct rsys_comm* c, float lr_factor, float clip, float grad_div);

int model_create(const rsys_config* cfg, int device, Model** out);
int model_destroy(Model* m);
int model_init_random(Model* m, uint64_t seed);
int model_load_metadata(Model* m, const float* table, int64_t V, int64_t Mdim);
int model_random_metadata(Model* m, uint64_t seed);
int model_set_rope(Model* m, const float* c, const float* s, int64_t n_pos);
int model_param_io(Model* m, const char* name, float* out, const float* in, int64_t n, int which );
int model_refresh_shadow(Model* m);
int model_batch_upload(Model* m, const rsys_batch* b);
int model_batch_upload_trimmed(Model* m, const rsys_batch* b, int row_len);
int check_not_trimmed(const Model* m);
int model_forward_backward(Model* m, int evaluate, const float task_w[4], float grad_scale, uint64_t seed, uint64_t step);
int model_infer(Model* m, int task, const int32_t* token_index, int64_t n_tokens, float* out, int64_t n);
int adapter_io(Model* m, int slot, const char* name, float* out, const float* in, int64_t n);
int adapter_clear(Model* m, int slot);
int adapter_slots(Model* m, int32_t* mask_out);
int adapter_bind_rows(Model* m, const int32_t* row_adapter);
int adapter_bind_tiles(Model* m, const int32_t* tile_adapter);
void adapter_unbind_rows(Model* m);
void adapter_bank_free(Model* m);
template <typename T> int adapter_bank_stage_a(Model* m, int l, const T* xn);
template <typename T> int adapter_bank_stage_b(Model* m, int l, T* qkv, const int* rope_pos);
inline void set_row_len(Model* m, int row_len) { m->S = row_len; m->T = 2 * row_len; }
inline bool batch_trimmed(const Model* m) { return m->S != m->Sa; }
inline bool trunk_frozen(const Model* m) { return m->cfg.finetune != 0 || m->bank_train; }
inline float* small_grad(Model* m, int64_t off) { return m->bank_train ? m->bank_sink : m->G + off; }
int adapter_train_enable(Model* m, float dropout);
int adapter_forward_backward(Model* m, int evaluate, const int32_t* row_slot, const int32_t* row_task, float grad_scale, uint64_t seed, uint64_t step);
int adapter_forward_backward_packed(Model* m, int evaluate, const int32_t* seg, int n_seg, float grad_scale, uint64_t seed, uint64_t step);
int adapter_grad_get(Model* m, int slot, const char* name, float* out, int64_t n);
int adapter_zero_grad(Model* m);
int adapter_adamw_step(Model* m, float lr0, float b1, float b2, float eps, float wd, const float* per_slot, int n_slots, float* norms_out);
int adapter_adamw_state_io(Model* m, int slot, const char* name, float* m_out, float* v_out, const float* m_in, const float* v_in, int64_t n, int32_t* step_out, int32_t step_in);
template <typename T> int adapter_bank_backward(Model* m, int l, const T* xn, const T* dqkv, T* dxn);
int adapter_bank_op(int dtype, int stages, int train, int rows, int Ttok, int D, int H, int KV, int hd, int L, int layer, float p, uint64_t seed,
                    int64_t stream, const int32_t* row_slot, const void* bankA, const void* bankB, const void* xn, void* La, void* qkv, const void* dqkv,
                    void* dLa, void* dxn, float* partA, float* partB, float* gA, float* gB, const float* rope_cos, const float* rope_sin,
                    const int32_t* rope_pos, int rope_rows, int tiles = 0 ,
                    int n_seg = 0 );
int adapter_bank_adamw_op(int dtype, float* A32, float* B32, float* gA, float* gB, float* mA, float* vA, float* mB, float* vB, void* A, void* B,
                          int64_t nA, int64_t nB, const float* per_slot, float b1, float b2, float eps, float wd, float* norms);
int model_forward_backward_rows(Model* m, int evaluate, const int* d_row_task, float grad_scale, uint64_t seed, uint64_t step);
int model_infer_adapters(Model* m, int task, const int32_t* row_adapter, const int32_t* token_index, int64_t n_tokens, float* out, int64_t n);
int model_infer_tiles(Model* m, int task, const int32_t* tile_adapter, const int32_t* token_index, int64_t n_tokens, float* out, int64_t n);
struct BatchDevRows { double* time; int *userid, *tmid, *gender, *source, *matchedid, *status; float *rating, *progress; int* rope_pos; };
int model_batch_device_begin(Model* m, int rows, BatchDevRows* out, int row_len = 0 );
int model_infer_device(Model* m, int task, const int32_t* row_adapter, const int* d_sel, int n_sel, float* d_out, const int32_t* tile_adapter = nullptr);
int model_rank_cache_reserve(Model* m, int n_slots);
int model_rank_cache_store(Model* m, const int32_t* row_adapter, const int32_t* n_hist, const int32_t* slot);
int model_rank_cache_candidates(Model* m, const int32_t* row_adapter, const int32_t* slot, const int32_t* n_cand, float* out);
int model_rank_cache_store_packed(Model* m, const int32_t* seg_adapter, int n_seg, const int32_t* seg);
int model_rank_cache_candidates_packed(Model* m, const int32_t* seg_adapter, int n_seg, const int32_t* seg, float* out);
int model_rank_cache_get(Model* m, int layer, int slot, void* out, int64_t bytes);
void rank_cache_free(Model* m);
int rank_cache_store_rows(Model* m, const int32_t* row_adapter, const int32_t* n_hist, const int32_t* slot, int* tab);
int rank_cache_candidates_rows(Model* m, const int32_t* row_adapter, const int32_t* slot, const int32_t* n_cand, int* tab, int* d_pos,
                               const int* d_sel, int64_t ntok, float* d_out);
int rank_cache_store_packed_rows(Model* m, const int32_t* seg_adapter, int n_seg, const int32_t* seg, int* d_pos);
template <typename T> int rank_cache_store_layer(Model* m, int l, const T* qkv);
template <typename T> int rank_cache_attention(Model* m, int l, const T* qkv, T* O);
template <typename T> int infer_rows_device(Model* m, int task, const int* d_sel, int64_t ntok, float* dst, const float** rows_f32);
template <typename T> int infer_trunk(Model* m);
int model_item_table(Model* m, float* out, int64_t n);
int model_item_table_device(Model* m, int medium, const float** rows, int64_t* Vm, int* D);
int model_materialise_trunk_output(Model* m);
int model_finalize_grads(Model* m);
bool model_finalize_splittable(const Model* m);
int model_batch_prefetch(Model* m, const rsys_batch* b);
int model_batch_swap(Model* m);
int model_split_table_enable(Model* m, int on);
int model_split_table_arm(Model* m, struct rsys_comm* c);
int model_split_table_tail(Model* m, struct rsys_comm* c, hipStream_t cs, int64_t* rows_out);
int model_finalize_stage(Model* m, int stage , int64_t* wp_off, int64_t* wp_n);
int model_clip(Model* m, float max_norm, float* norm_out);
int model_set_deterministic(Model* m, int on);
int model_ensure_det_scratch(Model* m);
int model_retrieve_topk(Model* m, int medium, const float* queries, int64_t nq, const int32_t* group, int32_t ng, const float* prior,
                        const int64_t* excl_off, const int32_t* excl_ids, int32_t k, int32_t* ids_out, float* scores_out, int32_t* counts_out);
using RetrieveInit = std::function<int(float* sc, hipStream_t s)>;
struct RetrieveDev;
struct RetrieveWin { const int64_t* start; const int32_t* len; int32_t* total_out; };
int model_retrieve_run(Model* m, int medium, const float* queries, int64_t nq, const int32_t* group, int32_t ng, const RetrieveInit& init,
                       int32_t k, int32_t* ids_out, float* scores_out, int32_t* counts_out, RetrieveDev* dev = nullptr,
                       const RetrieveWin* win = nullptr);
constexpr int RETRIEVE_CHUNK = 256, RETRIEVE_LSE_SPLIT = 64;
template <typename T>
int retrieve_chunk_scores(Model* m, const T* qt, int nc, int q0, const T* Fm, int Vm, float* z, long long ldz, float2* part, float* lse);
int model_retrieve_relations_set(Model* m, int medium, int kind, int64_t n_rows, int64_t n_cols, const int64_t* colptr, const int32_t* rowval,
                                 const float* nzval);
int model_retrieve_similarity_set(Model* m, int medium, int64_t dim, const float* emb, const float* crossproject);
int model_retrieve_released_set(Model* m, int medium, const uint8_t* mask);
int model_retrieve_request(Model* m, int medium, const float* queries, int64_t nq, const int32_t* group, int32_t ng, const int64_t* hist_off,
                           const int32_t* hist_medium, const int32_t* hist_ids, const int32_t* hist_status, const int64_t* sel_off,
                           const int32_t* sel_medium, const int32_t* sel_ids, int32_t k, int32_t* ids_out, float* scores_out,
                           int32_t* counts_out);
void retrieve_tables_free(Model* m);
struct RetrieveDev { const float* d_queries = nullptr; int32_t* d_ids = nullptr; float* d_vals = nullptr; };
int model_retrieve_request_dev(Model* m, int medium, RetrieveDev* dev, int64_t nq, const int32_t* group, int32_t ng, const int64_t* hist_off,
                               const int32_t* hist_medium, const int32_t* hist_ids, const int32_t* hist_status, const int64_t* sel_off,
                               const int32_t* sel_medium, const int32_t* sel_ids, int32_t k, int32_t* counts_out);
int model_retrieve_window(Model* m, int medium, const float* queries, int64_t nq, const int32_t* group, int32_t ng, const int64_t* hist_off,
                          const int32_t* hist_medium, const int32_t* hist_ids, const int32_t* hist_status, const int64_t* sel_off,
                          const int32_t* sel_medium, const int32_t* sel_ids, const RetrieveWin* win, RetrieveDev* dev, int32_t* ids_out,
                          float* scores_out, int32_t* counts_out);
const float* retrieve_similarity_table(Model* m, int medium, int64_t* dim);
int model_rank_related_set(Model* m, int medium, int64_t n, const int64_t* colptr, const int32_t* rowval, const float* nzval);
int model_rank_request(Model* m, int medium, int32_t ng, const int64_t* cand_off, const int32_t* cand_ids, const int32_t* partialk,
                       const float* penalties, const float* queries, int64_t nu, const int32_t* group, const float* r_masked, int64_t n_rm,
                       const int64_t* hist_off, const int32_t* hist_medium, const int32_t* hist_ids, const int32_t* hist_status,
                       const float* retrieval_coef, const float* rating_coefs, float rating_mean, const float* r_in, int32_t* ids_out,
                       float* r_out);
int model_rank_gram(Model* m, int medium, int32_t ng, const int64_t* cand_off, const int32_t* cand_ids, float* out, int64_t n_out);
struct RankDev { const int32_t* d_cand; const float* d_queries; const float* d_rm; const int32_t *page_lo, *page_hi; const int64_t* page_off;
                 int32_t* page_out; float* keep_r; int32_t* keep_picks; };
int model_rank_request_dev(Model* m, int medium, int32_t ng, const int64_t* cand_off, const RankDev* dev, const int32_t* partialk,
                           const float* penalties, int64_t nu, const int32_t* group, int64_t n_rm, const int64_t* hist_off,
                           const int32_t* hist_medium, const int32_t* hist_ids, const int32_t* hist_status, const float* retrieval_coef,
                           const float* rating_coefs, float rating_mean);
int model_rank_items_dev(Model* m, int medium, int32_t ng, const int64_t* cand_off, const RankDev* dev, const int32_t* partialk,
// ... 37 lines not shown
```

### recommendersystem_amd/csrc/model_backward.hip

```cpp
#include "model_internal.hpp"

namespace rsys {

static int ensure_transposes(Model* m) {
  if (!m->bf16_mode || !m->wt_dirty) return RSYS_OK;
  const int D = m->D, Ip = m->Ip;
  TransposeBatch b; b.n = 0;
  auto add = [&](int64_t off, int rows, int cols, long long ld) -> int {
    TransposeJob& j = b.job[b.n++];
    j.src = (const bf16*)m->Sh + off; j.dst = (bf16*)m->ShT + off; j.rows = rows; j.cols = cols; j.ld_src = ld; j.ld_dst = rows;
    if (b.n == 64) { int rc = launch_transpose_bf16(b, m->stream); b.n = 0; return rc; }
    return RSYS_OK;
  };
  for (int l = 0; l < m->L; ++l) {
    RC(add(m->lo[l].wqkv, m->Nqkv, D, D));
    RC(add(m->lo[l].wo, D, D, D));
    RC(add(m->lo[l].w13, 2 * Ip, D, D));
    RC(add(m->lo[l].w2, D, Ip, Ip));
  }
  RC(launch_transpose_bf16(b, m->stream));
  m->wt_dirty = false;
  return RSYS_OK;
}

// ... 248 lines not shown
        p.C = m->G + m->lo[l].lb + (int64_t)nv0 * 16 + 8; p.ldc = 16; p.c_f32 = 1;
        p.M = nkv; p.N = 8; p.K = NT; p.epi = EPI_ATOMIC; p.alpha = 2.f;
        RC(gemm<T>(m, "gemm_lora_db", p, false, true, true));
      }
      {
        GemmParams p{};
        p.A = m->dLa; p.lda = 16; p.B = xnd; p.ldb = D; p.C = m->G + m->lo[l].la; p.ldc = D; p.c_f32 = 1;
        p.M = 16; p.N = D; p.K = NT; p.epi = EPI_ATOMIC;
        RC(gemm<T>(m, "gemm_lora_da", p, false, true, true));
      }
      {
        GemmParams p{};
        p.A = m->dLa; p.lda = 16; p.B = W<T>(m, m->lo[l].la); p.ldb = D; p.ldc = D;
        p.M = NT; p.N = D; p.K = 16; p.epi = EPI_STORE;
        if (m->drop_active) {
          p.C = m->dxl;
          RC(gemm<T>(m, "gemm_lora_dx", p, false, false, true));
          RC(launch_dropout<T>(AT<T>(m->dxl), AT<T>(m->dhn), (long long)NT * D, m->cfg.lora_dropout, m->drop_seed,
                               (unsigned int)(m->drop_step * 64 + l), 1, s));
        } else {
          p.C = m->dhn; p.accum = 1;
          RC(gemm<T>(m, "gemm_lora_dx", p, false, false, true));
        }
      }
    }
    tic(m, "hbm_rmsnorm_bwd", nb_bytes);
    if (top)
      RC(launch_rmsnorm_bwd<T>(AT<T>(m->dhn), a.x, m->P + m->lo[l].sa, a.rstd1, m->c_dh, gx_other, cp ? gxt_other : nullptr, small_grad(m, m->lo[l].sa), NT, D, s,
                               nullptr, m->c_slot_p, m->c_perm));
    else {
      RC(launch_rmsnorm_bwd<T>(AT<T>(m->dhn), a.x, m->P + m->lo[l].sa, a.rstd1, m->dh, gx_other, cp ? gxt_other : nullptr, small_grad(m, m->lo[l].sa), NT, D, s, nullptr, nullptr, nullptr,
                               (m->fp8 && l > 0) ? f8_slot(m, l - 1, F8S_DY2) : nullptr));
    }
    toc(m);
    std::swap(gx, gx_other);
    std::swap(gxt, gxt_other);
    if (f8dw && !defer && !ft) RC(f8_dw_round_accum(m, l, l));
    if (defer && !m->grad_bucket_hook && l == 0) RC(grouped_weight_grads<T>(m, 0, m->L - 1));
    if (m->grad_bucket_hook && !ft) {
      const int64_t lo = m->lo[l].wqkv, hi = m->lo[bucket_top].w2 + pad8((int64_t)D * Ip);
      const bool boundary = defer ? (l == m->L / 2 && (hi - lo) * 4 >= (25ll << 20)) : (hi - lo) * 4 >= (25ll << 20);
      if (l == 0 || boundary) {
        if (defer) RC(grouped_weight_grads<T>(m, l, bucket_top));
        RC(m->grad_bucket_hook(lo, hi));
        bucket_top = l - 1;
        m->gemm_flags |= GEMM_ONE_WG_PER_TILE;
      }
    }
  }
  toc(m);
  if (trunk_frozen(m)) return RSYS_OK;
  tic(m, "phase_embed_bwd");
  BatchDev b = m->bd; b.N = N; b.rows = rows; b.S = m->S;
  tic(m, "hbm_scatter", 12.0 * D * N);
  {
    const bool atomic_ab = sw().scatter_atomic != 0;
    if (m->sharded) {
      HIP_CHECK(hipMemsetAsync(m->Frem, 0, (size_t)m->U * D * 4, s));
      RC(launch_embedding_scatter_segmented(gx, 2LL * D, b.m_matchedid, m->u_slot, m->tok_sidx, N, m->uV, D, m->Frem, m->scatter_slab, s));
      RC(comm_exchange(m->shard_comm, m->Frem, m->need_offD.data(), m->rows_xchg, m->serve_offD.data(), 4, s));
      for (int q = 0; q < m->sh_world; ++q) {
        const long long o = m->serve_off[q], n = m->serve_off[q + 1] - o;
        RC(launch_add_rows_by_id(m->rows_xchg + o * D, m->req_ids + o, m->row_lo, m->G + m->o_E, D, (int)n, D, s));
      }
    } else if (atomic_ab) RC(launch_embedding_scatter_add(gx, b, m->V, D, m->G + m->o_E, s));
    else {
      if (!m->tok_index_valid) {
        RC(launch_token_index_build(b.matchedid, N, m->V, m->tok_keys, m->tok_skey, m->tok_sidx, s));
        m->tok_index_valid = true;
      }
      if (m->split_head_reduced) {
        if (!m->split_plan_valid) {
          RC(launch_plan_unique(m->tok_skey, m->tok_sidx, N, m->V, m->u_slot, m->u_ids, m->u_tok, m->u_plan, s));
          int plan[2];
          HIP_CHECK(hipMemcpyAsync(plan, m->u_plan, 8, hipMemcpyDeviceToHost, s));
          HIP_CHECK(hipStreamSynchronize(s));
          ARG_CHECK(plan[0] >= 1 && plan[0] <= N + 1 && plan[0] <= m->tok_cap && plan[1] >= 0 && plan[1] < plan[0], "split table reduce: inconsistent list of distinct ids");
          m->U = plan[0]; m->uV = plan[1];
          m->split_plan_valid = true;
        }
        HIP_CHECK(hipMemsetAsync(m->tok_T, 0, (size_t)m->U * D * 4, s));
        RC(launch_embedding_scatter_segmented(gx, 2LL * D, b.m_matchedid, m->u_slot, m->tok_sidx, N, m->uV, D, m->tok_T, m->scatter_slab, s));
        if (m->split_head_event) HIP_CHECK(hipStreamWaitEvent(s, m->split_head_event, 0));
        RC(launch_add_rows_by_id(m->tok_T, m->u_ids, 0, m->G + m->o_E, D, m->U, D, s));
      } else
      RC(launch_embedding_scatter_segmented(gx, 2LL * D, b.m_matchedid, m->tok_skey, m->tok_sidx, N, m->V, D, m->G + m->o_E, m->scatter_slab, s));
    }
  }
  toc(m);
  m->table_grads_pending = true;
  m->gE_clean[0] = m->gE_clean[1] = false;
  {
    GemmParams p{};
    p.A = gxt + D; p.lda = 2 * D; p.B = m->feat; p.ldb = 32; p.C = m->G + m->o_lin_w; p.ldc = 32; p.c_f32 = 1;
    p.M = D; p.N = 32; p.K = N; p.epi = EPI_ATOMIC;
    RC(gemm<T>(m, "gemm_action_dw", p, false, true, true));
  }
  RC(launch_colsum_add(gx + D, 2 * D, N, D, m->G + m->o_lin_b, s));
  {
    GemmParams p{};
    p.A = gxt + D; p.lda = 2 * D; p.B = W<T>(m, m->o_lin_w); p.ldb = 32; p.C = m->gf; p.ldc = 32; p.c_f32 = 1;
    p.M = N; p.N = 32; p.K = D; p.epi = EPI_STORE;
    RC(gemm<T>(m, "gemm_action_dx", p, false, false, true));
  }
  SmallParams sp = small_params(m);
  RC(launch_action_small_bwd(m->gf, b, sp, m->G + m->o_pcos, m->G + m->o_psin, m->G + m->o_status, m->G + m->o_gender,
                             m->G + m->o_source, s));
  toc(m);
  return RSYS_OK;
}

template <typename T>
static int finalize_grads_t(Model* m, int stage) {
  tic(m, stage == 2 ? "phase_table_bwd_gemm" : "phase_table_bwd");
  const bool direct = m->bf16_mode && m->D % 64 == 0;
  if (stage != 2 && direct) {
    RC(launch_cast_transpose_colsum(m->G + m->o_E, (bf16*)m->dFT, m->TR, m->D, m->Vp, m->G + m->o_bp, m->stream));
  } else if (stage != 2) {
    m->table_dirty = true;
    const bool fused = m->bf16_mode && m->D <= 1024 && 1024 % (m->D >> 2) == 0;
    if (fused) {
      RC(launch_cast_colsum(m->G + m->o_E, (bf16*)m->FT, m->TR, m->D, m->G + m->o_bp, m->stream));
    } else {
      if (m->bf16_mode) RC(launch_cast<bf16>(m->G + m->o_E, (bf16*)m->FT, (long long)m->TR * m->D, m->stream));
      RC(launch_colsum_add(m->G + m->o_E, m->D, m->TR, m->D, m->G + m->o_bp, m->stream));
    }
    if (m->bf16_mode) {
      TransposeBatch b; b.n = 1;
      b.job[0].src = (const bf16*)m->FT; b.job[0].dst = (bf16*)m->dFT; b.job[0].rows = m->TR; b.job[0].cols = m->D;
      b.job[0].ld_src = m->D; b.job[0].ld_dst = m->Vp;
      RC(launch_transpose_bf16(b, m->stream));
    }
  }
  if (stage != 1) {
    GemmParams p{};
    p.C = m->G + m->o_Wp; p.ldc = m->Mp; p.c_f32 = 1; p.M = m->D; p.N = m->Mp; p.epi = EPI_ATOMIC;
    if (m->bf16_mode) {
      p.A = m->dFT; p.lda = m->Vp; p.B = m->MetaT; p.ldb = m->Vp; p.K = (int)m->Vp;
      RC(gemm<T>(m, "gemm_table_dw", p, false, false, false));
    } else {
      p.A = m->G + m->o_E; p.lda = m->D; p.B = m->Meta; p.ldb = m->Mp; p.K = m->TR;
      RC(gemm<T>(m, "gemm_table_dw", p, false, true, true));
    }
  }
  toc(m);
  return RSYS_OK;
}

int model_finalize_grads(Model* m) {
  if (!m->table_grads_pending || m->cfg.finetune) return RSYS_OK;
  DetScope det(m);
  m->table_grads_pending = false;
  return m->bf16_mode ? finalize_grads_t<bf16>(m, 0) : finalize_grads_t<float>(m, 0);
}

bool model_finalize_splittable(const Model* m) { return m->table_grads_pending && !m->cfg.finetune && m->bf16_mode; }

int model_split_table_enable(Model* m, int on) {
  if (!on) { m->split_table = false; m->table_head_hook = nullptr; return RSYS_OK; }
  ARG_CHECK(!m->sharded, "split table reduce: the item table is row-sharded (its rows are reduced by their owners already)");
  ARG_CHECK(m->bf16_mode && !m->cfg.finetune, "split table reduce: bf16 training of the full model only (the fp32 mode's metadata-projection gradient reads G[E] itself)");
  HIP_CHECK(hipSetDevice(m->device));
  if (!m->tbl_R) {
    const int64_t N = (int64_t)m->rows_max * m->Sa;
    m->tok_cap = N + 1;
    DALLOC(m->tbl_R, (int64_t)m->TR * m->D * 4);
    DALLOC(m->tok_T, m->tok_cap * m->D * 4);
    if (!m->u_slot) { DALLOC(m->u_slot, N * 4); DALLOC(m->u_ids, (N + 1) * 4); DALLOC(m->u_tok, N * 4); DALLOC(m->u_plan, 64); }
  }
  m->split_table = true;
  return RSYS_OK;
}

int model_split_table_rows(Model* m, int64_t* rows) {
  int64_t n = m->tok_cap;
  if (m->umax_pending) {
    HIP_CHECK(hipEventSynchronize(m->ev_umax));
    m->umax_pending = false;
    const int64_t got = (int64_t)m->h_umax[1];
    ARG_CHECK(got >= m->U && got <= m->tok_cap, "split table reduce: the ranks' maximum of distinct ids is smaller than this rank's own list");
    n = (got + 63) / 64 * 64;
    if (n > m->tok_cap) n = m->tok_cap;
  }
  *rows = n;
  return RSYS_OK;
}
int model_split_table_arm(Model* m, rsys_comm* c) {
  if (m->h_umax == nullptr) {
    HIP_CHECK(hipHostMalloc((void**)&m->h_umax, 64, hipHostMallocDefault));
    HIP_CHECK(hipMalloc((void**)&m->d_umax, 64));
    HIP_CHECK(hipEventCreateWithFlags(&m->ev_umax, hipEventDisableTiming));
  }
  const int64_t bound = (m->u_bound_host >= 1 && m->u_bound_host <= m->tok_cap) ? m->u_bound_host : m->tok_cap;
  if (m->umax_pending) HIP_CHECK(hipEventSynchronize(m->ev_umax));
  m->h_umax[0] = (float)bound;
  HIP_CHECK(hipMemcpyAsync(m->d_umax, m->h_umax, 4, hipMemcpyHostToDevice, c->stream));
  RC(comm_all_reduce_f32(c, m->d_umax, 1, COMM_MAX, c->stream));
  HIP_CHECK(hipMemcpyAsync(m->h_umax + 1, m->d_umax, 4, hipMemcpyDeviceToHost, c->stream));
  HIP_CHECK(hipEventRecord(m->ev_umax, c->stream));
  m->umax_pending = true;
  return RSYS_OK;
}

int model_split_table_tail(Model* m, rsys_comm* c, hipStream_t cs, int64_t* rows_out) {
  const int W = comm_active(c) ? c->world : 1, D = m->D;
  int64_t cap = 0;
  RC(model_split_table_rows(m, &cap));
  if (rows_out) *rows_out = cap;
  if (m->tok_all_world < W || m->tok_all_rows < cap) {
    for (void* p : {(void*)m->tok_Tall, (void*)m->tok_Uall, (void*)m->tok_Pall}) if (p) HIP_CHECK(hipFree(p));
    m->tok_Tall = nullptr; m->tok_Uall = nullptr; m->tok_Pall = nullptr;
    const int64_t rows = std::min<int64_t>(m->tok_cap, cap + cap / 8);
    HIP_CHECK(hipMalloc((void**)&m->tok_Tall, (size_t)W * rows * D * 4));
    HIP_CHECK(hipMalloc((void**)&m->tok_Uall, (size_t)W * rows * 4));
    HIP_CHECK(hipMalloc((void**)&m->tok_Pall, (size_t)W * 64));
    m->tok_all_world = W; m->tok_all_rows = rows;
  }
  RC(comm_all_gather(c, m->tok_T, m->tok_Tall, (size_t)cap * D * 4, cs));
  RC(comm_all_gather(c, m->u_ids, m->tok_Uall, (size_t)cap * 4, cs));
  RC(comm_all_gather(c, m->u_plan, m->tok_Pall, 64, cs));
  HIP_CHECK(hipMemcpyAsync(m->G + m->o_E, m->tbl_R, (size_t)m->TR * D * 4, hipMemcpyDeviceToDevice, cs));
  for (int q = 0; q < W; ++q)
    RC(launch_add_rows_by_id_counted(m->tok_Tall + (size_t)q * cap * D, m->tok_Uall + (size_t)q * cap, m->tok_Pall + (size_t)q * 16,
                                     m->G + m->o_E, D, (int)cap, D, cs));
  return RSYS_OK;
}
int model_finalize_stage(Model* m, int stage, int64_t* wp_off, int64_t* wp_n) {
  if (wp_off) *wp_off = m->o_Wp;
  if (wp_n) *wp_n = (int64_t)m->D * m->Mp;
  if (stage == 2) m->table_grads_pending = false;
  DetScope det(m);
  return finalize_grads_t<bf16>(m, stage);
}

template int backward_trunk<float>(Model*);
template int backward_trunk<bf16>(Model*);

}
```

### recommendersystem_amd/csrc/model_forward.hip

```cpp
#include "model_internal.hpp"

namespace rsys {

template <typename T>
int table_forward(Model* m) {
  GemmParams p{};
  p.A = m->Meta; p.lda = m->Mp; p.B = W<T>(m, m->o_Wp); p.ldb = m->Mp; p.C = m->F32; p.ldc = m->D; p.c_f32 = 1;
  p.M = m->TR; p.N = m->D; p.K = m->Mp; p.epi = EPI_TABLE; p.E = m->P + m->o_E; p.bias = m->P + m->o_bp;
  p.C2 = m->FT; p.ldc2 = m->D;
  int rows_main = m->TR;
  if constexpr (is_bf16<T>::value) {
    const int cus = cu_count();
    const int tiles_n = (m->D + 255) / 256, tiles = ((m->TR + 255) / 256) * tiles_n;
    const int rounds = tiles / cus, rem = tiles % cus;
    if (sw().table_tail != 0 && !m->deterministic && rounds >= 3 && rem > 0 && rem * 4 <= cus && (rounds * cus) % tiles_n == 0 && m->D % 256 == 0 &&
        m->Mp % 64 == 0 && m->Mp >= 1024)
      rows_main = (rounds * cus / tiles_n) * 256;
  }
  p.M = rows_main;
  RC(gemm<T>(m, "gemm_table_fwd", p, false, false, false));
  if (rows_main < m->TR) {
    const int64_t r0 = rows_main, nr = m->TR - rows_main;
    float* Ft = (float*)m->F32 + r0 * m->D;
    tic(m, "table_tail_rows");
// ... 387 lines not shown
  return RSYS_OK;
}

template <typename T>
int heads(Model* m, int evaluate, const float tw[4]) {
  const int D = m->D, rows = m->cur_rows, N = rows * m->S, NT = 2 * N, KB = m->K * rows;
  hipStream_t s = m->stream;
  const bool train = !evaluate;
  tic(m, "phase_heads");
  const bool ctop = m->top_is_sparse;
  if (train && ctop && m->loss_acc_with_c_gy) HIP_CHECK(hipMemsetAsync(m->loss_acc, 0, 256 + (size_t)m->ctop_cap * D * 4, s));
  else {
    HIP_CHECK(hipMemsetAsync(m->loss_acc, 0, 16 * 4, s));
    if (train && !ctop) HIP_CHECK(hipMemsetAsync(m->gy, 0, (size_t)NT * D * 4, s));
    if (train && ctop) HIP_CHECK(hipMemsetAsync(m->c_gy, 0, (size_t)m->ctop_cap * D * 4, s));
  }
  auto add_rows = [&](const float* src, int ti, int parity) -> int { return head_add_rows(m, src, ti, parity, KB); };
  for (int ti = 0; ti < 4; ++ti) {
    const int medium = ti >> 1, metric = ti & 1;
    float* st = m->stats + 2 * ti;
    int* np = m->npos + ti;
    if (ctop) RC(launch_gather_rows_slot<T>(AT<T>(m->c_out), m->c_slot, m->idx[ti], metric, AT<T>(m->Ew), KB, D, s));
    else RC(launch_gather_rows<T>(AT<T>(m->out), D, m->idx[ti], metric, AT<T>(m->Ew), KB, D, s));
    const bool bwd = train && tw[ti] != 0.f;
    if (metric == 0 && m->sharded) {
      RC(watch_head_sharded<T>(m, ti, medium, train, bwd, tw[ti]));
    } else if (metric == 0) {
      const int vs = medium == 0 ? 0 : m->V0, Vm = medium == 0 ? m->V0 : m->V1;
      T* Fm = AT<T>(m->FT) + (int64_t)vs * D;
      {
        GemmParams p{};
        p.A = m->Ew; p.lda = D; p.B = Fm; p.ldb = D; p.C = m->logits; p.ldc = m->ldl;
        p.M = KB; p.N = Vm; p.K = D; p.epi = EPI_STORE; p.m_dev = np;
        RC(gemm<T>(m, "gemm_logits", p, false, false, false));
      }
      tic(m, "ce");
      RC(launch_ce_fwd_bwd<T>(AT<T>(m->logits), m->ldl, KB, Vm, m->idx[ti], m->bd.m_label[ti], m->bd.m_weight[ti],
                              m->bd.m_position[ti], st, np, train ? tw[ti] : 0.f, m->loss_acc + 3 * ti, s));
      toc(m);
      if (bwd) {
        {
          GemmParams p{};
          HIP_CHECK(hipMemsetAsync(m->dE, 0, (size_t)KB * D * 4, s));
          p.A = m->logits; p.lda = m->ldl; p.B = Fm; p.ldb = D; p.C = m->dE; p.ldc = D; p.c_f32 = 1;
          p.M = KB; p.N = D; p.K = Vm; p.epi = EPI_ATOMIC; p.m_dev = np;
          RC(gemm<T>(m, "gemm_head_dx", p, false, false, true));
        }
        RC(add_rows(m->dE, ti, 0));
        if (!trunk_frozen(m)) {
          GemmParams p{};
          p.A = m->logits; p.lda = m->ldl; p.B = m->Ew; p.ldb = D; p.C = m->G + m->o_E + (int64_t)vs * D; p.ldc = D; p.c_f32 = 1;
          p.M = Vm; p.N = D; p.K = KB; p.epi = m->gE_clean[medium] ? EPI_STORE : EPI_ACCUM; p.k_dev = np;
          m->gE_clean[medium] = false;
          RC(gemm<T>(m, "gemm_head_dw", p, false, true, true));
        }
        if (!trunk_frozen(m)) m->table_grads_pending = true;
      }
    } else {
      {
        GemmParams p{};
        p.A = m->Ew; p.lda = D; p.B = W<T>(m, m->o_r0w); p.ldb = D; p.C = m->z; p.ldc = D;
        p.M = KB; p.N = D; p.K = D; p.epi = EPI_GELU; p.bias = m->P + m->o_r0b; p.C2 = m->hact; p.ldc2 = D;
        p.m_dev = np;
        RC(gemm<T>(m, "gemm_rating_fwd", p, false, false, false));
      }
      RC(launch_rating_tail<T>(AT<T>(m->z), AT<T>(m->hact), KB, D, m->P + m->o_r2w, m->P + m->o_r2b, m->idx[ti],
                               m->bd.m_label[ti], m->bd.m_weight[ti], st, m->cfg.rating_mean, bwd ? tw[ti] : 0.f,
                               bwd ? 0 : 1, m->loss_acc + 3 * ti, small_grad(m, m->o_r2w), small_grad(m, m->o_r2b), small_grad(m, m->o_r0b), s, np));
      if (bwd) {
        if (!trunk_frozen(m)) {
          GemmParams p{};
          p.A = m->z; p.lda = D; p.B = m->Ew; p.ldb = D; p.C = m->G + m->o_r0w; p.ldc = D; p.c_f32 = 1;
          p.M = D; p.N = D; p.K = KB; p.epi = EPI_ATOMIC; p.k_dev = np;
          RC(gemm<T>(m, "gemm_rating_dw", p, false, true, true));
        }
        {
          GemmParams p{};
          p.A = m->z; p.lda = D; p.B = W<T>(m, m->o_r0w); p.ldb = D; p.C = m->dE; p.ldc = D; p.c_f32 = 1;
          p.M = KB; p.N = D; p.K = D; p.epi = EPI_STORE; p.m_dev = np;
          RC(gemm<T>(m, "gemm_rating_dx", p, false, false, true));
        }
        RC(add_rows(m->dE, ti, 1));
      }
    }
  }
  toc(m);
  return RSYS_OK;
}

int select_positions_all(Model* m) {
  const int N = m->cur_rows * m->S, KB = m->K * m->cur_rows;
  const float* ws[4]; int* is[4]; float* sts[4]; int* nps[4];
  for (int ti = 0; ti < 4; ++ti) { ws[ti] = m->bd.m_weight[ti]; is[ti] = m->idx[ti]; sts[ti] = m->stats + 2 * ti; nps[ti] = m->npos + ti; }
  hipStream_t s = m->stream;
  const bool chunked_on = sw().select_chunked != 0;
  if (chunked_on && N >= 4096) RC(launch_select_positions_chunked(4, ws, N, KB, is, sts, nps, m->sel_scratch, s));
  else RC(launch_select_positions_batch(4, ws, N, KB, is, sts, nps, s));
  if (m->top_is_sparse) RC(launch_token_union(is, nps, 4, 2 * N, m->c_bits, m->c_pre, m->c_n, s));
  return RSYS_OK;
}

template int table_forward<float>(Model*);
template int table_forward<bf16>(Model*);
template int forward_trunk<float>(Model*);
template int forward_trunk<bf16>(Model*);
template int heads<float>(Model*, int, const float*);
// ... 6 lines not shown
```

### recommendersystem_amd/csrc/model_optim.hip

```cpp
#include "model_internal.hpp"

namespace rsys {

static int grad_sumsq(Model* m) {
  if (!m->sharded || !comm_active(m->shard_comm)) return launch_sumsq(m->G, m->n_opt, m->sumsq, m->sumsq_part, m->stream, true);
  const int64_t e0 = m->o_E, e1 = m->o_E + (int64_t)m->TR * m->D;
  RC(launch_sumsq(m->G, e0, m->sumsq, m->sumsq_part, m->stream, true));
  RC(launch_sumsq(m->G + e1, m->n_opt - e1, m->sumsq, m->sumsq_part, m->stream));
  RC(launch_sumsq(m->G + e0, e1 - e0, m->sumsq_E, m->sumsq_part, m->stream, true));
  RC(comm_all_reduce_f32(m->shard_comm, m->sumsq_E, 1, COMM_SUM, m->stream));
  return launch_add_scalar(m->sumsq, m->sumsq_E, m->stream);
}

int model_clip(Model* m, float max_norm, float* norm_out) {
  HIP_CHECK(hipSetDevice(m->device));
  DetScope det(m);
  RC(model_finalize_grads(m));
  RC(grad_sumsq(m));
  RC(launch_scale(m->G, m->n_opt, m->sumsq, 1.0f, max_norm, m->stream));
  if (norm_out) {
    float ss;
    HIP_CHECK(hipMemcpyAsync(&ss, m->sumsq, 4, hipMemcpyDeviceToHost, m->stream));
    HIP_CHECK(hipStreamSynchronize(m->stream));
    *norm_out = sqrtf(ss);
  }
  return RSYS_OK;
}

int optimizer_step(Optimizer* o, float lr_factor, float clip, float grad_div) {
  Model* m = o->m;
  HIP_CHECK(hipSetDevice(m->device));
  DetScope det(m);
  RC(model_finalize_grads(m));
  if (grad_div <= 0.f) grad_div = 1.f;
  const float* ss = nullptr;
  if (clip > 0.f) {
    tic(m, "sumsq", 4.0 * m->n_opt);
    RC(grad_sumsq(m));
    toc(m);
    ss = m->sumsq;
  }
  o->step += 1;
  const long long e_lo = m->cfg.finetune ? 0 : m->o_E, e_hi = m->cfg.finetune ? 0 : m->o_E + pad8((int64_t)m->TR * m->D);
  tic(m, "adamw", 32.0 * m->n_opt + (m->bf16_mode ? 2.0 * (m->n_opt - (e_hi - e_lo)) : 0.0));
  int rc;
  if (!m->cfg.finetune) { m->wt_dirty = true; m->table_dirty = true; m->w8_dirty = true; }
  if (m->bf16_mode)
    rc = launch_adamw<bf16>(m->P, m->G, o->mom, o->var, (bf16*)m->Sh, m->n_opt_decay, m->n_opt, o->lr * lr_factor, o->b1, o->b2,
                            o->eps, o->wd, o->step, ss, grad_div, clip, 1, m->stream, e_lo, e_hi);
  else
    rc = launch_adamw<float>(m->P, m->G, o->mom, o->var, nullptr, m->n_opt_decay, m->n_opt, o->lr * lr_factor, o->b1, o->b2,
                             o->eps, o->wd, o->step, ss, grad_div, clip, 1, m->stream);
  toc(m);
  if (rc == RSYS_OK && !m->cfg.finetune) m->gE_clean[0] = m->gE_clean[1] = true;
  return rc;
}

int optimizer_set_zero1(Optimizer* o, int rank, int world) {
  Model* m = o->m;
  ARG_CHECK(world >= 1 && rank >= 0 && rank < world, "zero1: rank / world");
  ARG_CHECK(!m->sharded && !m->cfg.finetune, "zero1: replicated pretraining model only (the row-sharded table already partitions its optimizer state)");
  ARG_CHECK(o->step == 0, "zero1: set before the first step");
  HIP_CHECK(hipSetDevice(m->device));
  const long long chunk = (m->n_opt / world) & ~63LL, tail = m->n_opt - chunk * world;
  ARG_CHECK(chunk > 0, "zero1: fewer than 64 parameters per rank");
  if (o->mom) HIP_CHECK(hipFree(o->mom));
  if (o->var) HIP_CHECK(hipFree(o->var));
  o->mom = o->var = nullptr;
  const size_t n = (size_t)(chunk + tail);
  HIP_CHECK(hipMalloc((void**)&o->mom, n * 4)); HIP_CHECK(hipMalloc((void**)&o->var, n * 4));
  HIP_CHECK(hipMemset(o->mom, 0, n * 4)); HIP_CHECK(hipMemset(o->var, 0, n * 4));
  if (o->z_tailbuf) { HIP_CHECK(hipFree(o->z_tailbuf)); o->z_tailbuf = nullptr; }
  if (tail > 0) HIP_CHECK(hipMalloc((void**)&o->z_tailbuf, (size_t)tail * 4));
  o->zero1 = true; o->z_rank = rank; o->z_world = world; o->z_chunk = chunk; o->z_tail = tail;
  return RSYS_OK;
}

int optimizer_step_zero1(Optimizer* o, rsys_comm* c, float lr_factor, float clip, float grad_div) {
  Model* m = o->m;
  ARG_CHECK(o->zero1, "zero1: rsys_adamw_set_zero1 first");
  ARG_CHECK(c != nullptr && c->world == o->z_world && c->rank == o->z_rank, "zero1: communicator of another rank / world");
  HIP_CHECK(hipSetDevice(m->device));
  DetScope det(m);
  RC(model_finalize_grads(m));
  hipStream_t s = m->stream;
  const long long chunk = o->z_chunk, tail = o->z_tail, lo = o->z_rank * chunk, tail_lo = chunk * o->z_world;
  const bool last = o->z_rank == o->z_world - 1;
  if (grad_div <= 0.f) grad_div = 1.f;
  RC(comm_reduce_scatter_f32(c, m->G, (size_t)chunk, s));
  if (tail > 0) RC(comm_all_reduce_f32(c, m->G + tail_lo, (size_t)tail, COMM_SUM, s));
  const float* ss = nullptr;
  if (clip > 0.f) {
    RC(launch_sumsq(m->G + lo, chunk, m->sumsq, m->sumsq_part, s, true));
    if (last && tail > 0) RC(launch_sumsq(m->G + tail_lo, tail, m->sumsq, m->sumsq_part, s));
    RC(comm_all_reduce_f32(c, m->sumsq, 1, COMM_SUM, s));
    ss = m->sumsq;
  }
  o->step += 1;
  const long long e_lo = m->o_E, e_hi = m->o_E + pad8((int64_t)m->TR * m->D);
  auto part = [&](long long at, long long n, float* mom, float* var) -> int {
    const long long nd = std::min(std::max(m->n_opt_decay - at, 0LL), n);
    if (m->bf16_mode)
      return launch_adamw<bf16>(m->P + at, m->G + at, mom, var, (bf16*)m->Sh + at, nd, n, o->lr * lr_factor, o->b1, o->b2, o->eps, o->wd, o->step, ss,
                                grad_div, clip, 1, s, e_lo - at, e_hi - at);
    return launch_adamw<float>(m->P + at, m->G + at, mom, var, nullptr, nd, n, o->lr * lr_factor, o->b1, o->b2, o->eps, o->wd, o->step, ss, grad_div, clip, 1, s, 0, 0);
  };
  RC(part(lo, chunk, o->mom, o->var));
// ... 22 lines not shown
```

### recommendersystem_amd/csrc/optim.hip

```cpp
#include "kernels.hpp"
#include "switches.hpp"

namespace rsys {

__global__ __launch_bounds__(256) void sumsq_kernel(const float* __restrict__ g, long long n, float* __restrict__ part) {
  __shared__ float red[16];
  float a0 = 0.f, a1 = 0.f, a2 = 0.f, a3 = 0.f;
  const long long n4 = n >> 2, stride = (long long)gridDim.x * blockDim.x;
  long long i = (long long)blockIdx.x * blockDim.x + threadIdx.x;
  const float4* g4 = (const float4*)g;
  for (; i + 3 * stride < n4; i += 4 * stride) {
    const float4 v0 = g4[i], v1 = g4[i + stride], v2 = g4[i + 2 * stride], v3 = g4[i + 3 * stride];
    a0 += v0.x * v0.x + v0.y * v0.y + v0.z * v0.z + v0.w * v0.w;
    a1 += v1.x * v1.x + v1.y * v1.y + v1.z * v1.z + v1.w * v1.w;
    a2 += v2.x * v2.x + v2.y * v2.y + v2.z * v2.z + v2.w * v2.w;
    a3 += v3.x * v3.x + v3.y * v3.y + v3.z * v3.z + v3.w * v3.w;
  }
  for (; i < n4; i += stride) {
    const float4 v = g4[i];
    a0 += v.x * v.x + v.y * v.y + v.z * v.z + v.w * v.w;
  }
  if (blockIdx.x == 0)
    for (long long k = (n4 << 2) + threadIdx.x; k < n; k += blockDim.x) a1 += g[k] * g[k];
  const float acc = block_sum((a0 + a1) + (a2 + a3), red);
  if (threadIdx.x == 0) part[blockIdx.x] = acc;
}
__global__ __launch_bounds__(256) void sumsq_final_kernel(const float* __restrict__ part, int nparts, float* out, int overwrite) {
  __shared__ float red[16];
  float a = 0.f;
  for (int i = threadIdx.x; i < nparts; i += 256) a += part[i];
  a = block_sum(a, red);
  if (threadIdx.x == 0) *out = overwrite ? a : *out + a;
}

int sumsq_parts() { return 2048; }
int launch_sumsq(const float* g, long long n, float* out, float* part, hipStream_t s, bool overwrite) {
  ARG_CHECK(part != nullptr, "sumsq: no partial-sum buffer");
  if (n <= 0) { if (overwrite) HIP_CHECK(hipMemsetAsync(out, 0, 4, s)); return RSYS_OK; }
  ARG_CHECK(((uintptr_t)g % 16) == 0, "sumsq: the range must start on a 16-byte boundary");
  const int grid = (int)std::min<long long>(((n >> 2) + 1023) / 1024 + 1, 2048);
  hipLaunchKernelGGL(sumsq_kernel, dim3(grid), dim3(256), 0, s, g, n, part);
  HIP_CHECK(hipGetLastError());
  hipLaunchKernelGGL(sumsq_final_kernel, dim3(1), dim3(256), 0, s, part, grid, out, overwrite ? 1 : 0);
  HIP_CHECK(hipGetLastError());
  return RSYS_OK;
}

static constexpr int CHECKSUM_GRID = 1024;
__global__ __launch_bounds__(256) void checksum_part_kernel(const float* __restrict__ p, long long n, double* part, int add) {
  __shared__ double s0[256], s1[256];
  __shared__ unsigned long long s2[256];
  double a = 0.0, b = 0.0;
  unsigned long long c = 0;
  for (long long i = (long long)blockIdx.x * blockDim.x + threadIdx.x; i < n; i += (long long)gridDim.x * blockDim.x) {
    const float v = p[i];
    a += (double)v; b += (double)v * (double)v; c += (unsigned long long)__float_as_uint(v) * (unsigned long long)((i & 1023) + 1);
  }
  s0[threadIdx.x] = a; s1[threadIdx.x] = b; s2[threadIdx.x] = c;
  __syncthreads();
  for (int w = 128; w > 0; w >>= 1) {
    if ((int)threadIdx.x < w) { s0[threadIdx.x] += s0[threadIdx.x + w]; s1[threadIdx.x] += s1[threadIdx.x + w]; s2[threadIdx.x] += s2[threadIdx.x + w]; }
    __syncthreads();
  }
  if (threadIdx.x == 0) {
    double* q = part + 3 * blockIdx.x;
    unsigned long long prev = add ? (unsigned long long)__double_as_longlong(q[2]) : 0ull;
    q[0] = (add ? q[0] : 0.0) + s0[0]; q[1] = (add ? q[1] : 0.0) + s1[0];
    q[2] = __longlong_as_double((long long)(prev + s2[0]));
  }
}
__global__ __launch_bounds__(64) void checksum_final_kernel(const double* part, int nparts, double* out) {
  if (threadIdx.x != 0 || blockIdx.x != 0) return;
  double a = 0.0, b = 0.0; unsigned long long c = 0;
  for (int i = 0; i < nparts; ++i) { a += part[3 * i]; b += part[3 * i + 1]; c += (unsigned long long)__double_as_longlong(part[3 * i + 2]); }
  out[0] = a; out[1] = b; out[2] = (double)(unsigned int)(c & 0xffffffffull); out[3] = (double)(unsigned int)(c >> 32);
}
int launch_checksum(const float* p, const long long* ranges, int n_ranges, double* part, double* out, hipStream_t s) {
  for (int r = 0; r < n_ranges; ++r) {
    const long long lo = ranges[2 * r], hi = ranges[2 * r + 1];
    ARG_CHECK(hi >= lo, "checksum: empty or reversed range");
    hipLaunchKernelGGL(checksum_part_kernel, dim3(CHECKSUM_GRID), dim3(256), 0, s, p + lo, hi - lo, part, r > 0 ? 1 : 0);
    HIP_CHECK(hipGetLastError());
  }
  hipLaunchKernelGGL(checksum_final_kernel, dim3(1), dim3(64), 0, s, part, CHECKSUM_GRID, out);
  HIP_CHECK(hipGetLastError());
  return RSYS_OK;
}
int checksum_scratch_doubles() { return 3 * CHECKSUM_GRID + 4; }

__device__ __forceinline__ float grad_coef(const float* sumsq, float grad_div, float max_norm) {
  float inv = 1.f / grad_div;
  if (sumsq == nullptr || max_norm <= 0.f) return inv;
  float norm = sqrtf(*sumsq) * inv;
  float c = max_norm / (norm + 1e-6f);
  return inv * (c < 1.f ? c : 1.f);
}

template <typename T, bool NT = false>
__global__ __launch_bounds__(256) void adamw_kernel(float* p, float* g, float* m, float* v, T* shadow, long long n_decay,
                                                    long long n_total, float lr, float b1, float b2, float eps, float wd,
                                                    float bc1, float bc2_sqrt, const float* sumsq, float grad_div,
                                                    float max_norm, int zero_grad, long long sh_skip_lo, long long sh_skip_hi) {
  const float coef = grad_coef(sumsq, grad_div, max_norm);
  const long long n4 = n_total >> 2;
  for (long long i = (long long)blockIdx.x * blockDim.x + threadIdx.x; i < n4; i += (long long)gridDim.x * blockDim.x) {
    float4 pv, gv, mv, vv;
    if constexpr (NT) {
      typedef __attribute__((ext_vector_type(4))) float nt_f32x4;
      auto ld = [](const float* q) { const nt_f32x4 t = __builtin_nontemporal_load((const nt_f32x4*)q); return make_float4(t[0], t[1], t[2], t[3]); };
      pv = ld(p + 4 * i); gv = ld(g + 4 * i); mv = ld(m + 4 * i); vv = ld(v + 4 * i);
    } else { pv = ((float4*)p)[i]; gv = ((float4*)g)[i]; mv = ((float4*)m)[i]; vv = ((float4*)v)[i]; }
    const float decay = (i * 4 < n_decay) ? (1.f - lr * wd) : 1.f;
    float* pp = (float*)&pv; float* gg = (float*)&gv; float* mm = (float*)&mv; float* vvp = (float*)&vv;
#pragma unroll
    for (int k = 0; k < 4; ++k) {
      float gk = gg[k] * coef;
      float pk = pp[k] * decay;
      mm[k] = b1 * mm[k] + (1.f - b1) * gk;
      vvp[k] = b2 * vvp[k] + (1.f - b2) * gk * gk;
      float denom = sqrtf(vvp[k]) / bc2_sqrt + eps;
      pp[k] = pk - (lr / bc1) * (mm[k] / denom);
    }
    if constexpr (NT) {
      typedef __attribute__((ext_vector_type(4))) float nt_f32x4;
      auto st = [](float* q, const float4& x) { const nt_f32x4 t = {x.x, x.y, x.z, x.w}; __builtin_nontemporal_store(t, (nt_f32x4*)q); };
      st(p + 4 * i, pv); st(m + 4 * i, mv); st(v + 4 * i, vv);
      if (zero_grad) st(g + 4 * i, make_float4(0, 0, 0, 0));
    } else {
      ((float4*)p)[i] = pv; ((float4*)m)[i] = mv; ((float4*)v)[i] = vv;
      if (zero_grad) ((float4*)g)[i] = make_float4(0, 0, 0, 0);
    }
    if constexpr (is_bf16<T>::value) {
      if (shadow && !(i * 4 >= sh_skip_lo && i * 4 < sh_skip_hi)) {
        bf16x4 sv; sv[0] = (bf16)pp[0]; sv[1] = (bf16)pp[1]; sv[2] = (bf16)pp[2]; sv[3] = (bf16)pp[3];
        ((bf16x4*)shadow)[i] = sv;
      }
    }
  }
}

template <typename T>
int launch_adamw(float* p, float* g, float* m, float* v, T* shadow, long long n_decay, long long n_total, float lr,
                 float b1, float b2, float eps, float wd, int step, const float* sumsq, float grad_div, float max_norm,
                 int zero_grad, hipStream_t s, long long sh_skip_lo, long long sh_skip_hi) {
  ARG_CHECK(n_decay % 4 == 0 && n_total % 4 == 0 && sh_skip_lo % 4 == 0 && sh_skip_hi % 4 == 0, "adamw: flat sizes must be multiples of 4");
  const float bc1 = 1.f - powf(b1, (float)step);
  const float bc2s = sqrtf(1.f - powf(b2, (float)step));
  const int mode = sw().debug_adamw;
  int grid = (int)std::min<long long>(((n_total >> 2) + 255) / 256, (mode & 2) ? 8192 : 4096);
  if (!(mode & 1))
    hipLaunchKernelGGL((adamw_kernel<T, true>), dim3(grid), dim3(256), 0, s, p, g, m, v, shadow, n_decay, n_total, lr, b1, b2, eps,
                       wd, bc1, bc2s, sumsq, grad_div, max_norm, zero_grad, sh_skip_lo, sh_skip_hi);
  else
  hipLaunchKernelGGL((adamw_kernel<T>), dim3(grid), dim3(256), 0, s, p, g, m, v, shadow, n_decay, n_total, lr, b1, b2, eps,
                     wd, bc1, bc2s, sumsq, grad_div, max_norm, zero_grad, sh_skip_lo, sh_skip_hi);
  HIP_CHECK(hipGetLastError());
  return RSYS_OK;
}
template int launch_adamw<bf16>(float*, float*, float*, float*, bf16*, long long, long long, float, float, float, float, float, int, const float*, float, float, int, hipStream_t, long long, long long);
template int launch_adamw<float>(float*, float*, float*, float*, float*, long long, long long, float, float, float, float, float, int, const float*, float, float, int, hipStream_t, long long, long long);

template <typename T>
__global__ void cast_kernel(const float* __restrict__ src, T* dst, long long n) {
  for (long long i = (long long)blockIdx.x * blockDim.x + threadIdx.x; i < n; i += (long long)gridDim.x * blockDim.x)
    dst[i] = from_f32<T>(src[i]);
}
template <typename T>
int launch_cast(const float* src, T* dst, long long n, hipStream_t s) {
  int grid = (int)std::min<long long>((n + 255) / 256, 8192);
  hipLaunchKernelGGL((cast_kernel<T>), dim3(grid), dim3(256), 0, s, src, dst, n);
  HIP_CHECK(hipGetLastError());
  return RSYS_OK;
}
template int launch_cast<bf16>(const float*, bf16*, long long, hipStream_t);
template int launch_cast<float>(const float*, float*, long long, hipStream_t);

__global__ void add_bias_rows_kernel(const float* __restrict__ a, const float* __restrict__ bias, float* __restrict__ dst, long long n, int D) {
  for (long long i = ((long long)blockIdx.x * blockDim.x + threadIdx.x) * 4; i < n; i += (long long)gridDim.x * blockDim.x * 4) {
    const float4 x = *(const float4*)(a + i), b = *(const float4*)(bias + (int)(i % D));
    *(float4*)(dst + i) = make_float4(x.x + b.x, x.y + b.y, x.z + b.z, x.w + b.w);
  }
}
int launch_add_bias_rows(const float* a, const float* bias, float* dst, long long rows, int D, hipStream_t s) {
  ARG_CHECK(D % 4 == 0, "add_bias_rows: D % 4");
  const long long n = rows * D;
  int grid = (int)std::min<long long>((n / 4 + 255) / 256, 4096);
  hipLaunchKernelGGL(add_bias_rows_kernel, dim3(std::max(grid, 1)), dim3(256), 0, s, a, bias, dst, n, D);
  HIP_CHECK(hipGetLastError());
  return RSYS_OK;
}

__global__ void scale_kernel(float* g, long long n, const float* sumsq, float grad_div, float max_norm) {
  const float coef = grad_coef(sumsq, grad_div, max_norm);
  for (long long i = (long long)blockIdx.x * blockDim.x + threadIdx.x; i < n; i += (long long)gridDim.x * blockDim.x) g[i] *= coef;
}
int launch_scale(float* g, long long n, const float* sumsq, float grad_div, float max_norm, hipStream_t s) {
  int grid = (int)std::min<long long>((n + 255) / 256, 8192);
  hipLaunchKernelGGL(scale_kernel, dim3(grid), dim3(256), 0, s, g, n, sumsq, grad_div, max_norm);
  HIP_CHECK(hipGetLastError());
  return RSYS_OK;
}

__device__ __forceinline__ void normal4(const Philox& ph, unsigned long long ctr, unsigned int stream, float out[4]) {
  uint32_t r[4];
  ph.gen(ctr, stream, r);
  float u0 = fmaxf(u01(r[0]), 5.9604645e-8f), u1 = u01(r[1]);
  float u2 = fmaxf(u01(r[2]), 5.9604645e-8f), u3 = u01(r[3]);
  float ra = sqrtf(-2.f * logf(u0)), rb = sqrtf(-2.f * logf(u2));
  out[0] = ra * cosf(6.2831853f * u1); out[1] = ra * sinf(6.2831853f * u1);
  out[2] = rb * cosf(6.2831853f * u3); out[3] = rb * sinf(6.2831853f * u3);
}

__global__ void fill_normal_kernel(float* dst, long long n, float std, unsigned long long seed, unsigned int stream, long long first4) {
  Philox ph(seed);
  const long long n4 = (n + 3) >> 2;
  for (long long i = (long long)blockIdx.x * blockDim.x + threadIdx.x; i < n4; i += (long long)gridDim.x * blockDim.x) {
    float z[4];
    normal4(ph, (unsigned long long)(i + first4), stream, z);
#pragma unroll
    for (int k = 0; k < 4; ++k)
      if (i * 4 + k < n) dst[i * 4 + k] = z[k] * std;
  }
}
int launch_fill_normal(float* dst, long long n, float std, unsigned long long seed, unsigned int stream, hipStream_t s, long long first) {
  ARG_CHECK(first % 4 == 0, "fill_normal: the start offset must be a multiple of 4");
  int grid = (int)std::min<long long>((((n + 3) >> 2) + 255) / 256, 8192);
  hipLaunchKernelGGL(fill_normal_kernel, dim3(grid), dim3(256), 0, s, dst, n, std, seed, stream, first >> 2);
  HIP_CHECK(hipGetLastError());
  return RSYS_OK;
}

template <typename T>
__global__ void fill_normal_t_kernel(T* dst, long long rows, int cols, long long ld, float std, unsigned long long seed, long long row0) {
  Philox ph(seed);
  const int c4 = (cols + 3) >> 2;
  const long long total = rows * c4;
  for (long long i = (long long)blockIdx.x * blockDim.x + threadIdx.x; i < total; i += (long long)gridDim.x * blockDim.x) {
    long long r = i / c4; int c = (int)(i % c4) * 4;
    float z[4];
    normal4(ph, (unsigned long long)(i + row0 * c4), 7u, z);
// ... 67 lines not shown
```

### recommendersystem_amd/csrc/switches.hip

```cpp
#include "switches.hpp"

#include <cstdio>
#include <cstdlib>
#include <cstring>
#include <mutex>

namespace rsys {
namespace {

struct Entry { const char* name; int Switches::*field; int dflt; };
const Entry kEntries[] = {
    {"RSYS_ATTN_DMA", &Switches::attn_dma, 1},
    {"RSYS_GEMM_KERNEL", &Switches::gemm_kernel, -1},
    {"RSYS_GEMM_KERNEL_TN", &Switches::gemm_kernel_tn, -1},
    {"RSYS_GEMM_KERNEL_NT_SPLITK", &Switches::gemm_kernel_nt_splitk, -1},
    {"RSYS_GEMM_KERNEL_MIX", &Switches::gemm_kernel_mix, 1},
    {"RSYS_GEMM8C_HALF", &Switches::gemm8c_half, 1},
    {"RSYS_GEMM4P", &Switches::gemm4p, 1},
    {"RSYS_GEMM4K", &Switches::gemm4k, 1},
    {"RSYS_GEMM8C", &Switches::gemm8c, 1},
    {"RSYS_GEMM_REVERSE", &Switches::gemm_reverse, 1},
    {"RSYS_GEMM_PATCH", &Switches::gemm_patch, 1},
    {"RSYS_TABLE_TAIL", &Switches::table_tail, 1},
    {"RSYS_DW_GROUP", &Switches::dw_group, 1},
    {"RSYS_DET_DW_GROUP", &Switches::det_dw_group, 1},
    {"RSYS_SPARSE_TOP", &Switches::sparse_top, 1},
    {"RSYS_TOP_ORDER", &Switches::top_order, 1},
    {"RSYS_SELECT_CHUNKED", &Switches::select_chunked, 1},
    {"RSYS_SCATTER_ATOMIC", &Switches::scatter_atomic, 0},
    {"RSYS_F8_DW", &Switches::f8_dw, 1},
    {"RSYS_F8_DW_ROUND_BF16", &Switches::f8_dw_round_bf16, 0},
    {"RSYS_F8_DEBUG_KEEP", &Switches::f8_debug_keep, 0},
    {"RSYS_FORCE_RCCL", &Switches::force_rccl, 0},
    {"RSYS_DEBUG_8P", &Switches::debug_8p, 0},
    {"RSYS_DEBUG_8G_SPLITK", &Switches::debug_8g_splitk, 0},
    {"RSYS_DEBUG_8T_SPLITK", &Switches::debug_8t_splitk, 0},
    {"RSYS_DEBUG_EPI", &Switches::debug_epi, -1},
    {"RSYS_DEBUG_F8_CAST_WAVES", &Switches::debug_f8_cast_waves, 4},
    {"RSYS_DEBUG_NORM_BWD_GRID", &Switches::debug_norm_bwd_grid, 1024},
    {"RSYS_DEBUG_NORM_BWD_WAVES", &Switches::debug_norm_bwd_waves, 0},
    {"RSYS_DEBUG_ADAMW", &Switches::debug_adamw, 0},
};

Switches g_sw;
bool g_parsed = false;
std::mutex g_mu;

void parse_locked() {
  for (const Entry& e : kEntries) {
    const char* v = getenv(e.name);
    g_sw.*(e.field) = (v && *v) ? atoi(v) : e.dflt;
  }
  g_parsed = true;
}

}

void switches_parse() { std::lock_guard<std::mutex> lk(g_mu); parse_locked(); }

const Switches& sw() {
  if (!g_parsed) { std::lock_guard<std::mutex> lk(g_mu); if (!g_parsed) parse_locked(); }
  return g_sw;
}

int switches_describe(char* buf, int cap) {
  const Switches& s = sw();
  int need = 0;
  if (buf && cap > 0) buf[0] = 0;
  for (const Entry& e : kEntries) {
    if (s.*(e.field) == e.dflt) continue;
    char one[96];
    const int n = snprintf(one, sizeof one, "%s%s=%d", need ? " " : "", e.name, s.*(e.field));
    if (buf && need + n < cap) memcpy(buf + need, one, (size_t)n + 1);
    need += n;
  }
  return need;
// ... 4 lines not shown
```

### recommendersystem_amd/csrc/switches.hpp

```cpp
#pragma once

namespace rsys {

struct Switches {
  int attn_dma;
  int gemm_kernel;
  int gemm_kernel_tn;
  int gemm_kernel_nt_splitk;
  int gemm_kernel_mix;
  int gemm8c_half;
  int gemm4p;
  int gemm4k;
  int gemm8c;
  int gemm_reverse;
  int gemm_patch;
  int table_tail;
  int dw_group;
  int det_dw_group;
  int sparse_top;
  int top_order;
  int select_chunked;
  int scatter_atomic;
  int f8_dw;
  int f8_dw_round_bf16;
  int f8_debug_keep;
  int force_rccl;
  int debug_8p;
  int debug_8g_splitk;
  int debug_8t_splitk;
  int debug_epi;
  int debug_f8_cast_waves;
  int debug_norm_bwd_grid;
  int debug_adamw;
  int debug_norm_bwd_waves;
};

const Switches& sw();
void switches_parse();
int switches_describe(char* buf, int cap);

}
```

Before: 1.632 million.

## Fold embedding-grad sumsq into cast-transpose pass and defer gE zeroing

```diff
diff --git a/include/rsys_debug.h b/include/rsys_debug.h
--- a/include/rsys_debug.h
+++ b/include/rsys_debug.h
@@ -84,6 +84,7 @@
                             float task_w, int32_t evaluate, float* loss, float* dw2, float* db2, float* db0, const int32_t* npos,
                             int32_t deterministic);
 int32_t rsys_op_sumsq(const float* g, int64_t n, float* out);
+int32_t rsys_op_sumsq_folded(const float* g, int64_t n, int64_t e_lo, int64_t rows, int32_t D, float* out);
 int32_t rsys_op_clip_adamw(int32_t dtype, float* p, float* g, float* m, float* v, void* shadow, int64_t n_decay, int64_t n_total,
                            float lr, float b1, float b2, float eps, float wd, int32_t step, float max_norm, float grad_div,
                            int32_t zero_grad, int64_t sh_skip_lo, int64_t sh_skip_hi, int32_t fused, float* sumsq);
diff --git a/recommendersystem_amd/_lib.py b/recommendersystem_amd/_lib.py
--- a/recommendersystem_amd/_lib.py
+++ b/recommendersystem_amd/_lib.py
@@ -225,6 +225,7 @@
     ("rsys_op_rating_tail", C.c_int32, [C.c_int32, _P, _P, C.c_int32, C.c_int32] + [_P] * 6 + [C.c_float, C.c_float, C.c_int32]
                                         + [_P] * 5 + [C.c_int32]),
     ("rsys_op_sumsq", C.c_int32, [_P, C.c_int64, _P]),
+    ("rsys_op_sumsq_folded", C.c_int32, [_P, C.c_int64, C.c_int64, C.c_int64, C.c_int32, _P]),
     ("rsys_op_clip_adamw", C.c_int32, [C.c_int32] + [_P] * 5 + [C.c_int64, C.c_int64] + [C.c_float] * 5
                                        + [C.c_int32, C.c_float, C.c_float, C.c_int32, C.c_int64, C.c_int64, C.c_int32, _P]),
     ("rsys_op_adapter_bank", C.c_int32, [C.c_int32] * 11 + [C.c_float, C.c_uint64, C.c_int64] + [_P] * 16 + [C.c_int32]),
diff --git a/recommendersystem_amd/csrc/capi.hip b/recommendersystem_amd/csrc/capi.hip
--- a/recommendersystem_amd/csrc/capi.hip
+++ b/recommendersystem_amd/csrc/capi.hip
@@ -74,6 +74,8 @@
   HIP_CHECK(hipMemsetAsync(h->m->G, 0, h->m->n_total * 4, h->m->stream));
   h->m->table_grads_pending = false;
   h->m->gE_clean[0] = h->m->gE_clean[1] = true;
+  h->m->gE_stale[0] = h->m->gE_stale[1] = false;
+  h->m->sumsq_Epart_n = 0;
   return RSYS_OK;
 }
 
@@ -741,6 +743,7 @@
   }
   HIP_CHECK(hipEventRecord(c->ev_done, c->stream));
   HIP_CHECK(hipStreamWaitEvent(m->stream, c->ev_done, 0));
+  m->sumsq_Epart_n = 0;
   return RSYS_OK;
 }
 int32_t rsys_grad_sync_early(rsys_model* h, int64_t* n) { CHECK_HANDLE(h); ARG_CHECK(n, "null"); *n = h->m->early_reduced; return RSYS_OK; }
@@ -783,6 +786,7 @@
   CHECK_HANDLE(h);
   int rc = model_finalize_grads(h->m);
   if (rc) return rc;
+  h->m->sumsq_Epart_n = 0;
   *p = h->m->G; *n = h->m->n_opt;
   return RSYS_OK;
 }
@@ -1224,6 +1228,26 @@
   return RSYS_OK;
 }
 
+int32_t rsys_op_sumsq_folded(const float* g, int64_t n, int64_t e_lo, int64_t rows, int32_t D, float* out) {
+  ARG_CHECK(g && out && rows > 0 && D > 0 && D % 64 == 0 && e_lo >= 0 && e_lo % 4 == 0 && e_lo + rows * D <= n, "rsys_op_sumsq_folded: arguments");
+  const int64_t ldt = (rows + 63) / 64 * 64;
+  const int nparts = cast_transpose_colsum_parts(rows);
+  float *part = nullptr, *epart = nullptr, *colsum = nullptr; bf16* dT = nullptr;
+  HIP_CHECK(hipMalloc((void**)&part, (size_t)sumsq_parts() * 4));
+  HIP_CHECK(hipMalloc((void**)&epart, (size_t)nparts * 4));
+  HIP_CHECK(hipMalloc((void**)&colsum, (size_t)D * 4));
+  HIP_CHECK(hipMalloc((void**)&dT, (size_t)D * ldt * 2));
+  HIP_CHECK(hipMemset(colsum, 0, (size_t)D * 4));
+  int got = 0;
+  int rc = launch_cast_transpose_colsum(g + e_lo, dT, rows, D, ldt, colsum, nullptr, epart, &got);
+  if (!rc) rc = launch_sumsq_skip(g, n, e_lo, e_lo + rows * D, epart, got, out, part, nullptr);
+  hipError_t e = hipDeviceSynchronize();
+  hipFree(part); hipFree(epart); hipFree(colsum); hipFree(dT);
+  if (rc) return rc;
+  HIP_CHECK(e);
+  return RSYS_OK;
+}
+
 int32_t rsys_op_clip_adamw(int32_t dtype, float* p, float* g, float* m, float* v, void* shadow, int64_t n_decay, int64_t n_total,
                            float lr, float b1, float b2, float eps, float wd, int32_t step, float max_norm, float grad_div,
                            int32_t zero_grad, int64_t sh_skip_lo, int64_t sh_skip_hi, int32_t fused, float* sumsq) {
diff --git a/recommendersystem_amd/csrc/elementwise.hip b/recommendersystem_amd/csrc/elementwise.hip
--- a/recommendersystem_amd/csrc/elementwise.hip
+++ b/recommendersystem_amd/csrc/elementwise.hip
@@ -872,9 +872,10 @@
 }
 
 __global__ __launch_bounds__(256) void cast_transpose_colsum_kernel(const float* __restrict__ src, bf16* __restrict__ dstT, long long rows, int D,
-                                                                    long long ldt, float* colsum, int rows_per_block, float* part) {
+                                                                    long long ldt, float* colsum, int rows_per_block, float* part, float* sq_part) {
   __shared__ unsigned short tile[64][72];
   __shared__ float red[16][64];
+  float sq = 0.f;
   const int t = threadIdx.x;
   const int lr = t >> 4, c4 = (t & 15) * 4;
   const int oc = t >> 2, or8 = (t & 3) * 16;
@@ -889,6 +890,7 @@
         const long long r = rb + 4 * lr + i;
         v[i] = r < rows ? *(const float4*)(src + r * D + ct * 64 + c4) : make_float4(0, 0, 0, 0);
         acc.x += v[i].x; acc.y += v[i].y; acc.z += v[i].z; acc.w += v[i].w;
+        sq += (v[i].x * v[i].x + v[i].y * v[i].y) + (v[i].z * v[i].z + v[i].w * v[i].w);
       }
       {
         bf16x4 o;
@@ -916,14 +918,20 @@
     }
     __syncthreads();
   }
-}
-int launch_cast_transpose_colsum(const float* src, bf16* dstT, long long rows, int D, long long ldt, float* colsum, hipStream_t s) {
+  if (sq_part != nullptr) {
+    const float v = block_sum(sq, &red[0][0]);
+    if (t == 0) sq_part[blockIdx.x] = v;
+  }
+}
+static int cast_transpose_chunks_per_block(long long rows) { return (int)std::max<long long>(1, ((rows + 63) / 64 + 2047) / 2048); }
+int cast_transpose_colsum_parts(long long rows) { const long long chunks = (rows + 63) / 64; const int cpb = cast_transpose_chunks_per_block(rows); return (int)((chunks + cpb - 1) / cpb); }
+int launch_cast_transpose_colsum(const float* src, bf16* dstT, long long rows, int D, long long ldt, float* colsum, hipStream_t s, float* sq_part, int* n_sq_part) {
   ARG_CHECK(D % 64 == 0 && ldt % 8 == 0 && ldt >= ((rows + 63) & ~63LL), "cast_transpose_colsum: D % 64, ldt % 8, ldt >= rows rounded up to 64");
-  const long long chunks = (rows + 63) / 64;
-  const int cpb = (int)std::max<long long>(1, (chunks + 2047) / 2048);
-  const int grid = (int)((chunks + cpb - 1) / cpb);
+  const int cpb = cast_transpose_chunks_per_block(rows);
+  const int grid = cast_transpose_colsum_parts(rows);
+  if (n_sq_part) *n_sq_part = grid;
   float* part = det_part((long long)grid * D);
-  hipLaunchKernelGGL(cast_transpose_colsum_kernel, dim3(grid), dim3(256), 0, s, src, dstT, rows, D, ldt, colsum, cpb * 64, part);
+  hipLaunchKernelGGL(cast_transpose_colsum_kernel, dim3(grid), dim3(256), 0, s, src, dstT, rows, D, ldt, colsum, cpb * 64, part, sq_part);
   HIP_CHECK(hipGetLastError());
   if (part != nullptr) return launch_reduce_parts(part, grid, D, D, colsum, s);
   return RSYS_OK;
diff --git a/recommendersystem_amd/csrc/kernels.hpp b/recommendersystem_amd/csrc/kernels.hpp
--- a/recommendersystem_amd/csrc/kernels.hpp
+++ b/recommendersystem_amd/csrc/kernels.hpp
@@ -86,7 +86,9 @@
 
 int launch_colsum_add(const float* src, long long ld, long long rows, int cols, float* dst, hipStream_t s);
 int launch_cast_colsum(const float* src, bf16* dst, long long rows, int D, float* colsum, hipStream_t s);
-int launch_cast_transpose_colsum(const float* src, bf16* dstT, long long rows, int D, long long ldt, float* colsum, hipStream_t s);
+int launch_cast_transpose_colsum(const float* src, bf16* dstT, long long rows, int D, long long ldt, float* colsum, hipStream_t s,
+                                 float* sq_part = nullptr, int* n_sq_part = nullptr);
+int cast_transpose_colsum_parts(long long rows);
 
 int launch_embedding_scatter_add(const float* gx0, const BatchDev& b, int V, int D, float* gE, hipStream_t s);
 
@@ -190,12 +192,14 @@
 
 int launch_sumsq(const float* g, long long n, float* out , float* part, hipStream_t s, bool overwrite = false);
 int sumsq_parts();
+int launch_sumsq_skip(const float* g, long long n, long long skip_lo, long long skip_hi, const float* extra, int n_extra, float* out, float* part, hipStream_t s);
 int launch_checksum(const float* p, const long long* ranges, int n_ranges, double* part, double* out, hipStream_t s);
 int checksum_scratch_doubles();
 template <typename T>
 int launch_adamw(float* p, float* g, float* m, float* v, T* shadow, long long n_decay, long long n_total,
                  float lr, float b1, float b2, float eps, float wd, int step, const float* sumsq, float grad_div,
-                 float max_norm, int zero_grad, hipStream_t s, long long sh_skip_lo = 0, long long sh_skip_hi = 0 );
+                 float max_norm, int zero_grad, hipStream_t s, long long sh_skip_lo = 0, long long sh_skip_hi = 0 ,
+                 long long g_keep_lo = 0, long long g_keep_hi = 0 );
 template <typename T> int launch_cast(const float* src, T* dst, long long n, hipStream_t s);
 int launch_add_bias_rows(const float* a, const float* bias, float* dst, long long rows, int D, hipStream_t s);
 template <typename T> int launch_widen(const T* src, float* dst, long long n, hipStream_t s);
@@ -203,6 +207,7 @@
 struct TransposeJob { const void* src; void* dst; int rows, cols; long long ld_src, ld_dst; };
 struct TransposeBatch { TransposeJob job[64]; int n; };
 int launch_transpose_bf16(const TransposeBatch& b, hipStream_t s);
+int launch_zero_if_empty(const int* count , float* dst, long long n, hipStream_t s);
 int launch_scale(float* g, long long n, const float* sumsq, float grad_div, float max_norm, hipStream_t s);
 int launch_fill_normal(float* dst, long long n, float std, unsigned long long seed, unsigned int stream, hipStream_t s, long long first = 0);
 template <typename T>
diff --git a/recommendersystem_amd/csrc/model.hip b/recommendersystem_amd/csrc/model.hip
--- a/recommendersystem_amd/csrc/model.hip
+++ b/recommendersystem_amd/csrc/model.hip
@@ -255,6 +255,7 @@
   DALLOC(m->dO, NT * D * e); DALLOC(m->dqkv, NT * m->Nqkv * e);
   DALLOC(m->delta, (int64_t)m->rows_max * m->H * m->Ta * 4); DALLOC(m->gf, N * 32 * 4);
   DALLOC(m->sumsq, 64); DALLOC(m->sumsq_part, (size_t)sumsq_parts() * 4);
+  DALLOC(m->sumsq_Epart, (size_t)cast_transpose_colsum_parts(m->TR) * 4);
   DALLOC(m->sel_scratch, 12 * 32 * 4);
   m->dLa = nullptr; m->dxl = nullptr;
   if (cfg->finetune) { DALLOC(m->dLa, NT * 16 * e); DALLOC(m->dxl, NT * D * e); }
@@ -544,6 +545,7 @@
     return RSYS_OK;
   }
   if (which == 1) RC(model_finalize_grads(m));
+  if (which == 1 && in) m->sumsq_Epart_n = 0;
   float* base = (which == 0 ? m->P : m->G) + t.off;
   const int64_t int_rows = (t.map == MAP_DIRECT) ? t.rows : 2 * m->Ip;
   std::vector<float> host((size_t)int_rows * t.ld);
@@ -881,7 +883,7 @@
   if (!evaluate) {
     m->split_head_reduced = false;
     m->split_head_event = nullptr;
-    if (m->table_head_hook) RC(m->table_head_hook());
+    if (m->table_head_hook) { RC(model_gE_fill(m)); RC(m->table_head_hook()); }
     RC(backward_trunk<T>(m));
   }
   return RSYS_OK;
diff --git a/recommendersystem_amd/csrc/model.hpp b/recommendersystem_amd/csrc/model.hpp
--- a/recommendersystem_amd/csrc/model.hpp
+++ b/recommendersystem_amd/csrc/model.hpp
@@ -188,6 +188,8 @@
   int *attn_order_q = nullptr, *attn_order_k = nullptr, *attn_order_q_p = nullptr, *attn_order_k_p = nullptr;
   bool table_grads_pending = false;
   bool gE_clean[2] = {false, false};
+  bool gE_stale[2] = {false, false};
+  float* sumsq_Epart = nullptr; int sumsq_Epart_n = 0;
   bool drop_active = false; unsigned long long drop_seed = 0, drop_step = 0;
   bool last_evaluate = false;
   PhaseTimer timer;
@@ -290,6 +292,7 @@
 int model_item_table_device(Model* m, int medium, const float** rows, int64_t* Vm, int* D);
 int model_materialise_trunk_output(Model* m);
 int model_finalize_grads(Model* m);
+int model_gE_fill(Model* m);
 bool model_finalize_splittable(const Model* m);
 int model_batch_prefetch(Model* m, const rsys_batch* b);
 int model_batch_swap(Model* m);
diff --git a/recommendersystem_amd/csrc/model_backward.hip b/recommendersystem_amd/csrc/model_backward.hip
--- a/recommendersystem_amd/csrc/model_backward.hip
+++ b/recommendersystem_amd/csrc/model_backward.hip
@@ -324,6 +324,7 @@
   if (trunk_frozen(m)) return RSYS_OK;
   tic(m, "phase_embed_bwd");
   BatchDev b = m->bd; b.N = N; b.rows = rows; b.S = m->S;
+  RC(model_gE_fill(m));
   tic(m, "hbm_scatter", 12.0 * D * N);
   {
     const bool atomic_ab = sw().scatter_atomic != 0;
@@ -386,8 +387,12 @@
 static int finalize_grads_t(Model* m, int stage) {
   tic(m, stage == 2 ? "phase_table_bwd_gemm" : "phase_table_bwd");
   const bool direct = m->bf16_mode && m->D % 64 == 0;
+  if (stage != 2) m->sumsq_Epart_n = 0;
   if (stage != 2 && direct) {
-    RC(launch_cast_transpose_colsum(m->G + m->o_E, (bf16*)m->dFT, m->TR, m->D, m->Vp, m->G + m->o_bp, m->stream));
+    const bool fold = sw().table_lean != 0 && stage == 0 && !m->sharded && !m->deterministic;
+    int nsq = 0;
+    RC(launch_cast_transpose_colsum(m->G + m->o_E, (bf16*)m->dFT, m->TR, m->D, m->Vp, m->G + m->o_bp, m->stream, fold ? m->sumsq_Epart : nullptr, &nsq));
+    if (fold) m->sumsq_Epart_n = nsq;
   } else if (stage != 2) {
     m->table_dirty = true;
     const bool fused = m->bf16_mode && m->D <= 1024 && 1024 % (m->D >> 2) == 0;
@@ -419,7 +424,18 @@
   return RSYS_OK;
 }
 
+int model_gE_fill(Model* m) {
+  for (int md = 0; md < 2; ++md) {
+    if (!m->gE_stale[md]) continue;
+    const int64_t r0 = md == 0 ? 0 : m->V0, nr = md == 0 ? m->V0 : m->V1;
+    if (nr > 0) HIP_CHECK(hipMemsetAsync(m->G + m->o_E + r0 * m->D, 0, (size_t)nr * m->D * 4, m->stream));
+    m->gE_stale[md] = false;
+  }
+  return RSYS_OK;
+}
+
 int model_finalize_grads(Model* m) {
+  RC(model_gE_fill(m));
   if (!m->table_grads_pending || m->cfg.finetune) return RSYS_OK;
   DetScope det(m);
   m->table_grads_pending = false;
@@ -501,6 +517,7 @@
   if (wp_off) *wp_off = m->o_Wp;
   if (wp_n) *wp_n = (int64_t)m->D * m->Mp;
   if (stage == 2) m->table_grads_pending = false;
+  if (stage == 1) RC(model_gE_fill(m));
   DetScope det(m);
   return finalize_grads_t<bf16>(m, stage);
 }
diff --git a/recommendersystem_amd/csrc/model_forward.hip b/recommendersystem_amd/csrc/model_forward.hip
--- a/recommendersystem_amd/csrc/model_forward.hip
+++ b/recommendersystem_amd/csrc/model_forward.hip
@@ -463,6 +463,12 @@
           p.A = m->logits; p.lda = m->ldl; p.B = m->Ew; p.ldb = D; p.C = m->G + m->o_E + (int64_t)vs * D; p.ldc = D; p.c_f32 = 1;
           p.M = Vm; p.N = D; p.K = KB; p.epi = m->gE_clean[medium] ? EPI_STORE : EPI_ACCUM; p.k_dev = np;
           m->gE_clean[medium] = false;
+          if (m->gE_stale[medium]) {
+            GemmParams q = p; q.alpha = 1.f; q.splitk = 1; q.flags |= m->gemm_flags;
+            if (p.epi != EPI_STORE) RC(model_gE_fill(m));
+            else if (gemm_route<T>(q, false, false, true, true, cu_count()).kernel != GK_8TS) RC(launch_zero_if_empty(np, (float*)p.C, (long long)Vm * D, s));
+            m->gE_stale[medium] = false;
+          }
           RC(gemm<T>(m, "gemm_head_dw", p, false, true, true));
         }
         if (!trunk_frozen(m)) m->table_grads_pending = true;
diff --git a/recommendersystem_amd/csrc/model_optim.hip b/recommendersystem_amd/csrc/model_optim.hip
--- a/recommendersystem_amd/csrc/model_optim.hip
+++ b/recommendersystem_amd/csrc/model_optim.hip
@@ -3,8 +3,10 @@
 namespace rsys {
 
 static int grad_sumsq(Model* m) {
+  const int64_t e0 = m->o_E, e1 = m->o_E + (int64_t)m->TR * m->D;
+  if (!m->sharded && m->sumsq_Epart_n > 0 && !m->table_grads_pending && e1 <= m->n_opt && e0 % 4 == 0 && e1 % 4 == 0)
+    return launch_sumsq_skip(m->G, m->n_opt, e0, e1, m->sumsq_Epart, m->sumsq_Epart_n, m->sumsq, m->sumsq_part, m->stream);
   if (!m->sharded || !comm_active(m->shard_comm)) return launch_sumsq(m->G, m->n_opt, m->sumsq, m->sumsq_part, m->stream, true);
-  const int64_t e0 = m->o_E, e1 = m->o_E + (int64_t)m->TR * m->D;
   RC(launch_sumsq(m->G, e0, m->sumsq, m->sumsq_part, m->stream, true));
   RC(launch_sumsq(m->G + e1, m->n_opt - e1, m->sumsq, m->sumsq_part, m->stream));
   RC(launch_sumsq(m->G + e0, e1 - e0, m->sumsq_E, m->sumsq_part, m->stream, true));
@@ -18,6 +20,7 @@
   RC(model_finalize_grads(m));
   RC(grad_sumsq(m));
   RC(launch_scale(m->G, m->n_opt, m->sumsq, 1.0f, max_norm, m->stream));
+  m->sumsq_Epart_n = 0;
   if (norm_out) {
     float ss;
     HIP_CHECK(hipMemcpyAsync(&ss, m->sumsq, 4, hipMemcpyDeviceToHost, m->stream));
@@ -35,24 +38,29 @@
   if (grad_div <= 0.f) grad_div = 1.f;
   const float* ss = nullptr;
   if (clip > 0.f) {
-    tic(m, "sumsq", 4.0 * m->n_opt);
+    tic(m, "sumsq", 4.0 * (m->n_opt - ((!m->sharded && m->sumsq_Epart_n > 0) ? (int64_t)m->TR * m->D : 0)));
     RC(grad_sumsq(m));
     toc(m);
     ss = m->sumsq;
   }
   o->step += 1;
   const long long e_lo = m->cfg.finetune ? 0 : m->o_E, e_hi = m->cfg.finetune ? 0 : m->o_E + pad8((int64_t)m->TR * m->D);
-  tic(m, "adamw", 32.0 * m->n_opt + (m->bf16_mode ? 2.0 * (m->n_opt - (e_hi - e_lo)) : 0.0));
+  const bool lean = sw().table_lean != 0 && !m->cfg.finetune && !m->sharded && m->bf16_mode && !m->fp8 && ((int64_t)(m->V0 + m->V1) * m->D) % 4 == 0 &&
+                    m->o_E % 4 == 0 && m->V0 + m->V1 < m->TR;
+  const long long k_lo = lean ? m->o_E : 0, k_hi = lean ? m->o_E + (int64_t)(m->V0 + m->V1) * m->D : 0;
+  tic(m, "adamw", 32.0 * m->n_opt - 4.0 * (k_hi - k_lo) + (m->bf16_mode ? 2.0 * (m->n_opt - (e_hi - e_lo)) : 0.0));
   int rc;
   if (!m->cfg.finetune) { m->wt_dirty = true; m->table_dirty = true; m->w8_dirty = true; }
   if (m->bf16_mode)
     rc = launch_adamw<bf16>(m->P, m->G, o->mom, o->var, (bf16*)m->Sh, m->n_opt_decay, m->n_opt, o->lr * lr_factor, o->b1, o->b2,
-                            o->eps, o->wd, o->step, ss, grad_div, clip, 1, m->stream, e_lo, e_hi);
+                            o->eps, o->wd, o->step, ss, grad_div, clip, 1, m->stream, e_lo, e_hi, k_lo, k_hi);
   else
     rc = launch_adamw<float>(m->P, m->G, o->mom, o->var, nullptr, m->n_opt_decay, m->n_opt, o->lr * lr_factor, o->b1, o->b2,
                              o->eps, o->wd, o->step, ss, grad_div, clip, 1, m->stream);
   toc(m);
+  m->sumsq_Epart_n = 0;
   if (rc == RSYS_OK && !m->cfg.finetune) m->gE_clean[0] = m->gE_clean[1] = true;
+  if (rc == RSYS_OK && lean) m->gE_stale[0] = m->gE_stale[1] = true;
   return rc;
 }
 
diff --git a/recommendersystem_amd/csrc/optim.hip b/recommendersystem_amd/csrc/optim.hip
--- a/recommendersystem_amd/csrc/optim.hip
+++ b/recommendersystem_amd/csrc/optim.hip
@@ -3,32 +3,36 @@
 
 namespace rsys {
 
-__global__ __launch_bounds__(256) void sumsq_kernel(const float* __restrict__ g, long long n, float* __restrict__ part) {
+template <bool SKIP>
+__global__ __launch_bounds__(256) void sumsq_kernel(const float* __restrict__ g, long long n, float* __restrict__ part, long long skip_lo4, long long skip_n4) {
   __shared__ float red[16];
   float a0 = 0.f, a1 = 0.f, a2 = 0.f, a3 = 0.f;
-  const long long n4 = n >> 2, stride = (long long)gridDim.x * blockDim.x;
+  const long long n4 = (n >> 2) - (SKIP ? skip_n4 : 0), stride = (long long)gridDim.x * blockDim.x;
   long long i = (long long)blockIdx.x * blockDim.x + threadIdx.x;
   const float4* g4 = (const float4*)g;
+  auto at = [&](long long j) { if constexpr (SKIP) return j >= skip_lo4 ? j + skip_n4 : j; else return j; };
   for (; i + 3 * stride < n4; i += 4 * stride) {
-    const float4 v0 = g4[i], v1 = g4[i + stride], v2 = g4[i + 2 * stride], v3 = g4[i + 3 * stride];
+    const float4 v0 = g4[at(i)], v1 = g4[at(i + stride)], v2 = g4[at(i + 2 * stride)], v3 = g4[at(i + 3 * stride)];
     a0 += v0.x * v0.x + v0.y * v0.y + v0.z * v0.z + v0.w * v0.w;
     a1 += v1.x * v1.x + v1.y * v1.y + v1.z * v1.z + v1.w * v1.w;
     a2 += v2.x * v2.x + v2.y * v2.y + v2.z * v2.z + v2.w * v2.w;
     a3 += v3.x * v3.x + v3.y * v3.y + v3.z * v3.z + v3.w * v3.w;
   }
   for (; i < n4; i += stride) {
-    const float4 v = g4[i];
+    const float4 v = g4[at(i)];
     a0 += v.x * v.x + v.y * v.y + v.z * v.z + v.w * v.w;
   }
   if (blockIdx.x == 0)
-    for (long long k = (n4 << 2) + threadIdx.x; k < n; k += blockDim.x) a1 += g[k] * g[k];
+    for (long long k = ((n >> 2) << 2) + threadIdx.x; k < n; k += blockDim.x) a1 += g[k] * g[k];
   const float acc = block_sum((a0 + a1) + (a2 + a3), red);
   if (threadIdx.x == 0) part[blockIdx.x] = acc;
 }
-__global__ __launch_bounds__(256) void sumsq_final_kernel(const float* __restrict__ part, int nparts, float* out, int overwrite) {
+__global__ __launch_bounds__(256) void sumsq_final_kernel(const float* __restrict__ part, int nparts, float* out, int overwrite,
+                                                          const float* __restrict__ part2, int nparts2) {
   __shared__ float red[16];
   float a = 0.f;
   for (int i = threadIdx.x; i < nparts; i += 256) a += part[i];
+  for (int i = threadIdx.x; i < nparts2; i += 256) a += part2[i];
   a = block_sum(a, red);
   if (threadIdx.x == 0) *out = overwrite ? a : *out + a;
 }
@@ -39,9 +43,22 @@
   if (n <= 0) { if (overwrite) HIP_CHECK(hipMemsetAsync(out, 0, 4, s)); return RSYS_OK; }
   ARG_CHECK(((uintptr_t)g % 16) == 0, "sumsq: the range must start on a 16-byte boundary");
   const int grid = (int)std::min<long long>(((n >> 2) + 1023) / 1024 + 1, 2048);
-  hipLaunchKernelGGL(sumsq_kernel, dim3(grid), dim3(256), 0, s, g, n, part);
-  HIP_CHECK(hipGetLastError());
-  hipLaunchKernelGGL(sumsq_final_kernel, dim3(1), dim3(256), 0, s, part, grid, out, overwrite ? 1 : 0);
+  hipLaunchKernelGGL(sumsq_kernel<false>, dim3(grid), dim3(256), 0, s, g, n, part, 0LL, 0LL);
+  HIP_CHECK(hipGetLastError());
+  hipLaunchKernelGGL(sumsq_final_kernel, dim3(1), dim3(256), 0, s, part, grid, out, overwrite ? 1 : 0, (const float*)nullptr, 0);
+  HIP_CHECK(hipGetLastError());
+  return RSYS_OK;
+}
+int launch_sumsq_skip(const float* g, long long n, long long skip_lo, long long skip_hi, const float* extra, int n_extra, float* out, float* part,
+                      hipStream_t s) {
+  ARG_CHECK(part != nullptr && extra != nullptr && n_extra > 0, "sumsq: no partial-sum buffer");
+  ARG_CHECK(0 <= skip_lo && skip_lo <= skip_hi && skip_hi <= n && skip_lo % 4 == 0 && skip_hi % 4 == 0, "sumsq: the skipped range must lie inside [0, n) on multiples of 4");
+  ARG_CHECK(((uintptr_t)g % 16) == 0, "sumsq: the range must start on a 16-byte boundary");
+  const long long rest = n - (skip_hi - skip_lo);
+  const int grid = (int)std::min<long long>(((rest >> 2) + 1023) / 1024 + 1, 2048);
+  hipLaunchKernelGGL(sumsq_kernel<true>, dim3(grid), dim3(256), 0, s, g, n, part, skip_lo >> 2, (skip_hi - skip_lo) >> 2);
+  HIP_CHECK(hipGetLastError());
+  hipLaunchKernelGGL(sumsq_final_kernel, dim3(1), dim3(256), 0, s, part, grid, out, 1, extra, n_extra);
   HIP_CHECK(hipGetLastError());
   return RSYS_OK;
 }
@@ -100,7 +117,8 @@
 __global__ __launch_bounds__(256) void adamw_kernel(float* p, float* g, float* m, float* v, T* shadow, long long n_decay,
                                                     long long n_total, float lr, float b1, float b2, float eps, float wd,
                                                     float bc1, float bc2_sqrt, const float* sumsq, float grad_div,
-                                                    float max_norm, int zero_grad, long long sh_skip_lo, long long sh_skip_hi) {
+                                                    float max_norm, int zero_grad, long long sh_skip_lo, long long sh_skip_hi,
+                                                    long long g_keep_lo, long long g_keep_hi) {
   const float coef = grad_coef(sumsq, grad_div, max_norm);
   const long long n4 = n_total >> 2;
   for (long long i = (long long)blockIdx.x * blockDim.x + threadIdx.x; i < n4; i += (long long)gridDim.x * blockDim.x) {
@@ -125,10 +143,10 @@
       typedef __attribute__((ext_vector_type(4))) float nt_f32x4;
       auto st = [](float* q, const float4& x) { const nt_f32x4 t = {x.x, x.y, x.z, x.w}; __builtin_nontemporal_store(t, (nt_f32x4*)q); };
       st(p + 4 * i, pv); st(m + 4 * i, mv); st(v + 4 * i, vv);
-      if (zero_grad) st(g + 4 * i, make_float4(0, 0, 0, 0));
+      if (zero_grad && !(i * 4 >= g_keep_lo && i * 4 < g_keep_hi)) st(g + 4 * i, make_float4(0, 0, 0, 0));
     } else {
       ((float4*)p)[i] = pv; ((float4*)m)[i] = mv; ((float4*)v)[i] = vv;
-      if (zero_grad) ((float4*)g)[i] = make_float4(0, 0, 0, 0);
+      if (zero_grad && !(i * 4 >= g_keep_lo && i * 4 < g_keep_hi)) ((float4*)g)[i] = make_float4(0, 0, 0, 0);
     }
     if constexpr (is_bf16<T>::value) {
       if (shadow && !(i * 4 >= sh_skip_lo && i * 4 < sh_skip_hi)) {
@@ -142,23 +160,23 @@
 template <typename T>
 int launch_adamw(float* p, float* g, float* m, float* v, T* shadow, long long n_decay, long long n_total, float lr,
                  float b1, float b2, float eps, float wd, int step, const float* sumsq, float grad_div, float max_norm,
-                 int zero_grad, hipStream_t s, long long sh_skip_lo, long long sh_skip_hi) {
-  ARG_CHECK(n_decay % 4 == 0 && n_total % 4 == 0 && sh_skip_lo % 4 == 0 && sh_skip_hi % 4 == 0, "adamw: flat sizes must be multiples of 4");
+                 int zero_grad, hipStream_t s, long long sh_skip_lo, long long sh_skip_hi, long long g_keep_lo, long long g_keep_hi) {
+  ARG_CHECK(n_decay % 4 == 0 && n_total % 4 == 0 && sh_skip_lo % 4 == 0 && sh_skip_hi % 4 == 0 && g_keep_lo % 4 == 0 && g_keep_hi % 4 == 0, "adamw: flat sizes must be multiples of 4");
   const float bc1 = 1.f - powf(b1, (float)step);
   const float bc2s = sqrtf(1.f - powf(b2, (float)step));
   const int mode = sw().debug_adamw;
   int grid = (int)std::min<long long>(((n_total >> 2) + 255) / 256, (mode & 2) ? 8192 : 4096);
   if (!(mode & 1))
     hipLaunchKernelGGL((adamw_kernel<T, true>), dim3(grid), dim3(256), 0, s, p, g, m, v, shadow, n_decay, n_total, lr, b1, b2, eps,
-                       wd, bc1, bc2s, sumsq, grad_div, max_norm, zero_grad, sh_skip_lo, sh_skip_hi);
+                       wd, bc1, bc2s, sumsq, grad_div, max_norm, zero_grad, sh_skip_lo, sh_skip_hi, g_keep_lo, g_keep_hi);
   else
   hipLaunchKernelGGL((adamw_kernel<T>), dim3(grid), dim3(256), 0, s, p, g, m, v, shadow, n_decay, n_total, lr, b1, b2, eps,
-                     wd, bc1, bc2s, sumsq, grad_div, max_norm, zero_grad, sh_skip_lo, sh_skip_hi);
-  HIP_CHECK(hipGetLastError());
-  return RSYS_OK;
-}
-template int launch_adamw<bf16>(float*, float*, float*, float*, bf16*, long long, long long, float, float, float, float, float, int, const float*, float, float, int, hipStream_t, long long, long long);
-template int launch_adamw<float>(float*, float*, float*, float*, float*, long long, long long, float, float, float, float, float, int, const float*, float, float, int, hipStream_t, long long, long long);
+                     wd, bc1, bc2s, sumsq, grad_div, max_norm, zero_grad, sh_skip_lo, sh_skip_hi, g_keep_lo, g_keep_hi);
+  HIP_CHECK(hipGetLastError());
+  return RSYS_OK;
+}
+template int launch_adamw<bf16>(float*, float*, float*, float*, bf16*, long long, long long, float, float, float, float, float, int, const float*, float, float, int, hipStream_t, long long, long long, long long, long long);
+template int launch_adamw<float>(float*, float*, float*, float*, float*, long long, long long, float, float, float, float, float, int, const float*, float, float, int, hipStream_t, long long, long long, long long, long long);
 
 template <typename T>
 __global__ void cast_kernel(const float* __restrict__ src, T* dst, long long n) {
@@ -186,6 +204,22 @@
   const long long n = rows * D;
   int grid = (int)std::min<long long>((n / 4 + 255) / 256, 4096);
   hipLaunchKernelGGL(add_bias_rows_kernel, dim3(std::max(grid, 1)), dim3(256), 0, s, a, bias, dst, n, D);
+  HIP_CHECK(hipGetLastError());
+  return RSYS_OK;
+}
+
+__global__ __launch_bounds__(256) void zero_if_empty_kernel(const int* __restrict__ count, float* __restrict__ dst, long long n) {
+  if (*count > 0) return;
+  const long long n4 = n >> 2;
+  for (long long i = (long long)blockIdx.x * blockDim.x + threadIdx.x; i < n4; i += (long long)gridDim.x * blockDim.x) ((float4*)dst)[i] = make_float4(0, 0, 0, 0);
+  if (blockIdx.x == 0)
+    for (long long k = (n4 << 2) + threadIdx.x; k < n; k += blockDim.x) dst[k] = 0.f;
+}
+int launch_zero_if_empty(const int* count, float* dst, long long n, hipStream_t s) {
+  ARG_CHECK(count != nullptr && ((uintptr_t)dst % 16) == 0, "zero_if_empty: null count or unaligned range");
+  if (n <= 0) return RSYS_OK;
+  const int grid = (int)std::min<long long>(((n >> 2) + 255) / 256 + 1, 2048);
+  hipLaunchKernelGGL(zero_if_empty_kernel, dim3(grid), dim3(256), 0, s, count, dst, n);
   HIP_CHECK(hipGetLastError());
   return RSYS_OK;
 }
diff --git a/recommendersystem_amd/csrc/switches.hip b/recommendersystem_amd/csrc/switches.hip
--- a/recommendersystem_amd/csrc/switches.hip
+++ b/recommendersystem_amd/csrc/switches.hip
@@ -22,6 +22,7 @@
     {"RSYS_GEMM_REVERSE", &Switches::gemm_reverse, 1},
     {"RSYS_GEMM_PATCH", &Switches::gemm_patch, 1},
     {"RSYS_TABLE_TAIL", &Switches::table_tail, 1},
+    {"RSYS_TABLE_LEAN", &Switches::table_lean, 1},
     {"RSYS_DW_GROUP", &Switches::dw_group, 1},
     {"RSYS_DET_DW_GROUP", &Switches::det_dw_group, 1},
     {"RSYS_SPARSE_TOP", &Switches::sparse_top, 1},
diff --git a/recommendersystem_amd/csrc/switches.hpp b/recommendersystem_amd/csrc/switches.hpp
--- a/recommendersystem_amd/csrc/switches.hpp
+++ b/recommendersystem_amd/csrc/switches.hpp
@@ -15,6 +15,7 @@
   int gemm_reverse;
   int gemm_patch;
   int table_tail;
+  int table_lean;
   int dw_group;
   int det_dw_group;
   int sparse_top;
```

Result: no change. 1.643 million (median of 6 runs) (+0.7%).
